# Komputerowe-Projektowanie-Lekow/pmarlo

Measured on AMD Instinct MI355X. Metric: frames/sec featurize->TICA->k-means->T-matrix, 1Mx64 synth; ITS rel-err, higher is better.
Workload: dtype f64; 1 GPU; synthetic 1000000 frames x 64 f32 features per GPU (AR(1) latents), TICA->10, k=500 (10 Lloyd iterations), lag=10, row-normalised T; frames_per_gpu=1000000, features=64, tica_dim=10, k=500, lag=10, kmeans_iters=10, parallelism=shards1

## Files before the change

include/msmhip.h:

```cpp
#ifndef MSMHIP_H
#define MSMHIP_H

#include <stddef.h>
#include <stdint.h>

#ifdef __cplusplus
extern "C" {
#endif

typedef struct msm_ctx msm_ctx;
typedef struct msm_event msm_event;
typedef struct msm_graph msm_graph;

typedef enum {
    MSM_OK = 0,
    MSM_ERR_INVALID = 1,
    MSM_ERR_HIP = 2,
    MSM_ERR_NOMEM = 3,
    MSM_ERR_UNSUPPORTED = 4,
    MSM_ERR_NOCONV = 5
} msm_status;

typedef enum { MSM_F32 = 0, MSM_F64 = 1 } msm_dtype;

// ... 33 lines not shown
                            int64_t ld, int col_off);
msm_status msm_featurize_angles(msm_ctx* ctx, const float* d_xyz, int64_t n, int A,
                                const int32_t* d_triplets, int Tn, float* d_out, int64_t ld, int col_off);
msm_status msm_featurize_dihedrals(msm_ctx* ctx, const float* d_xyz, int64_t n, int A,
                                   const int32_t* d_quads, int Q, int mode, float* d_out, int64_t ld,
                                   int col_off);

msm_status msm_featurize_sasa(msm_ctx* ctx, const float* d_xyz, int64_t n, int A, const float* d_radii,
                              const float* d_points, int P, float* d_out);
msm_status msm_hbond_presence(msm_ctx* ctx, const float* d_xyz, int64_t n, int A, const int32_t* d_triplets,
                              int Tn, float dist_cutoff, float angle_cutoff, uint64_t* d_counts);
msm_status msm_dssp(msm_ctx* ctx, const float* d_xyz, int64_t n, int A, const int32_t* d_backbone,
                    const int32_t* d_chain, const uint8_t* d_proline, int R, uint8_t* d_codes);

#define MSM_SUPERPOSE_TILE_FRAMES 64
#define MSM_SUPERPOSE_TILE_FLOATS 12288
#define MSM_SUPERPOSE_LDS_ATOMS 4096
#define MSM_SUPERPOSE_NARROW_SEL 64
msm_status msm_superpose(msm_ctx* ctx, const float* d_xyz, int64_t n, int A, const int32_t* d_sel, int S,
                         const float* d_ref, float* d_out, float* d_rmsd);


msm_status msm_count_transitions(msm_ctx* ctx, const int32_t* d_labels, int64_t n,
                                 const int64_t* h_seg_start, const int64_t* h_seg_stop,
                                 int n_seg, int lag, int stride, int k,
                                 int64_t* d_counts, int64_t* d_pairs);

msm_status msm_count_transitions_weighted(msm_ctx* ctx, const int32_t* d_labels,
                                          const double* d_weights, int64_t n,
                                          const int64_t* h_seg_start, const int64_t* h_seg_stop,
                                          int n_seg, int lag, int stride, int k,
                                          double* d_counts, int64_t* d_pairs);

msm_status msm_count_transitions_lagscan(msm_ctx* ctx, const int32_t* d_labels, int64_t n,
                                         const int64_t* h_seg_start, const int64_t* h_seg_stop,
                                         int n_seg, const int32_t* h_lags, int n_lag, int k,
                                         int64_t* d_counts, int64_t* d_pairs);

msm_status msm_state_counts(msm_ctx* ctx, const int32_t* d_labels, int64_t n, int k,
                            int64_t* d_visits);

msm_status msm_run_lengths(msm_ctx* ctx, const int32_t* d_labels, int64_t n, int k, int64_t* d_stats,
                           int32_t* d_run_state, int64_t* d_run_len, int64_t capacity, int64_t* d_n_runs);


msm_status msm_column_moments_partial(msm_ctx* ctx, const void* d_x, msm_dtype dtype, int64_t n, int F,
                                      int64_t ld, const double* d_shift, double* d_sums,
                                      double* d_shift_out);
msm_status msm_moments_finalize(msm_ctx* ctx, const double* d_sums, const double* d_shift, int F,
                                int ddof, double* d_mean, double* d_std, double* d_count);
msm_status msm_column_minmax(msm_ctx* ctx, const void* d_x, msm_dtype dtype, int64_t n, int F, int64_t ld,
                             double* d_min, double* d_max, int64_t* d_counts);
msm_status msm_column_moments(msm_ctx* ctx, const void* d_x, msm_dtype dtype, int64_t n, int F,
                              int64_t ld, int ddof, double* d_mean, double* d_std, double* d_count);

msm_status msm_standardise_params(msm_ctx* ctx, const double* d_sums, const double* d_shift, int F,
                                  double n_rows, int with_std, double* d_mean, double* d_scale,
                                  double* d_inv_scale);

msm_status msm_lagged_moments(msm_ctx* ctx, const void* d_x, msm_dtype dtype, int64_t n, int F, int64_t ld,
                              const int64_t* h_seg_start, const int64_t* h_seg_stop, int n_seg, int lag,
                              const double* d_shift, int assume_finite, double* d_moments);

msm_status msm_lagged_moments_reversible(msm_ctx* ctx, const void* d_x, msm_dtype dtype, int64_t n, int F, int64_t ld,
                                         const int64_t* h_seg_start, const int64_t* h_seg_stop, int n_seg, int lag,
                                         const double* d_shift, int assume_finite, double* d_moments);

msm_status msm_lagged_moments_onesided(msm_ctx* ctx, const void* d_x, msm_dtype dtype, int64_t n, int F,
                                       int64_t ld, const int64_t* h_seg_start, const int64_t* h_seg_stop,
                                       int n_seg, int lag, const double* d_shift, int assume_finite,
                                       double* d_moments);

msm_status msm_onesided_tica_eigenvalues(msm_ctx* ctx, const double* d_moments, int F, double clip,
                                         double* d_eigvals);

msm_status msm_moments_from_lagged(msm_ctx* ctx, const void* d_x, msm_dtype dtype, int64_t n, int F, int64_t ld,
                                   const int64_t* h_seg_start, const int64_t* h_seg_stop, int n_seg, int lag,
                                   const double* d_shift, const double* d_moments, double* d_sums);

msm_status msm_tica_solve(msm_ctx* ctx, const double* d_moments, const double* d_scale, int F,
                          double epsilon, int kinetic_map, double* d_eigvals, double* d_coeffs,
                          double* d_mean, int* d_rank);

msm_status msm_project(msm_ctx* ctx, const void* d_x, msm_dtype dtype, int64_t n, int F, int64_t ld,
                       const double* d_mu, const double* d_inv_sigma, const double* d_mean2,
                       const double* d_w, int d, int64_t ldw, double* d_y, int64_t ldy, double* d_absmax);

msm_status msm_project_finite(msm_ctx* ctx, const void* d_x, msm_dtype dtype, int64_t n, int F, int64_t ld,
                              const double* d_mu, const double* d_inv_sigma, const double* d_mean2,
                              const double* d_w, int d, int64_t ldw, double* d_y, int64_t ldy, double* d_absmax);

msm_status msm_eigh(msm_ctx* ctx, const double* d_a, int n, double* d_w, double* d_v, int* d_sweeps);

msm_status msm_autocorr_lagscan(msm_ctx* ctx, const void* d_x, msm_dtype dtype, int64_t n, int F, int64_t ld,
                                const int64_t* h_seg_start, const int64_t* h_seg_stop, int n_seg,
                                const int32_t* h_lags, int n_lag, double var_floor, double* d_value,
                                int32_t* d_nvalid);

msm_status msm_hstack_f64(msm_ctx* ctx, const void* d_a, msm_dtype dtype_a, int pa, int64_t lda, const void* d_b,
                          msm_dtype dtype_b, int pb, int64_t ldb, int64_t n, double* d_out);


msm_status msm_kmeans_assign(msm_ctx* ctx, const void* d_x, msm_dtype dtype, int64_t n, int d,
                             int64_t ld, const double* d_centers, int k,
                             const double* d_mean, const double* d_std,
                             int32_t* d_labels, double* d_mindist);

msm_status msm_kmeans_fit(msm_ctx* ctx, const void* d_x, msm_dtype dtype, int64_t n, int d, int64_t ld,
                          const double* d_mean, const double* d_std, int k, uint64_t seed,
                          int init_centers, int max_iter, double tol2, double* d_centers,
                          double* d_state);
msm_status msm_kmeans_init_plusplus(msm_ctx* ctx, const void* d_x, msm_dtype dtype, int64_t n, int d, int64_t ld,
                                    const double* d_mean, const double* d_std, int k, uint64_t seed, double n_total,
                                    double* d_centers, const double* d_state, int64_t* d_picked);
msm_status msm_kmeans_fit_begin(msm_ctx* ctx, const void* d_x, msm_dtype dtype, int64_t n, int d,
                                int64_t ld, const double* d_mean, const double* d_std, int k,
                                uint64_t seed, int init_centers, double n_total, double tol2,
                                double* d_centers, double* d_state, int absmax_ready);
msm_status msm_kmeans_accumulate(msm_ctx* ctx, const void* d_x, msm_dtype dtype, int64_t n, int d,
                                 int64_t ld, const double* d_centers, int k, const double* d_mean,
                                 const double* d_std, const double* d_state, int64_t* d_sums,
                                 int64_t* d_counts);
msm_status msm_kmeans_update(msm_ctx* ctx, int64_t* d_sums, int64_t* d_counts, int k, int d,
                             double* d_centers, double* d_state, int clear);

msm_status msm_kmeans_image_bytes(int64_t n, int d, size_t* out_bytes);
msm_status msm_kmeans_pack(msm_ctx* ctx, const void* d_x, msm_dtype dtype, int64_t n, int d, int64_t ld,
                           const double* d_mean, const double* d_std, void* d_image);
msm_status msm_kmeans_pack_bounded(msm_ctx* ctx, const void* d_x, msm_dtype dtype, int64_t n, int d, int64_t ld,
                                   const double* d_mean, const double* d_std, const double* d_absmax, void* d_image);
msm_status msm_kmeans_assign_packed(msm_ctx* ctx, const void* d_x, msm_dtype dtype, int64_t n, int d,
                                    int64_t ld, const double* d_centers, int k, const double* d_mean,
                                    const double* d_std, const void* d_image, int32_t* d_labels,
                                    double* d_mindist);
msm_status msm_kmeans_accumulate_packed(msm_ctx* ctx, const void* d_x, msm_dtype dtype, int64_t n, int d,
                                        int64_t ld, const double* d_centers, int k, const double* d_mean,
                                        const double* d_std, const void* d_image, const double* d_state,
                                        int64_t* d_sums, int64_t* d_counts);
msm_status msm_kmeans_accumulate_delta(msm_ctx* ctx, const void* d_x, msm_dtype dtype, int64_t n, int d,
                                       int64_t ld, const double* d_centers, int k, const double* d_mean,
                                       const double* d_std, const void* d_image, const double* d_state,
                                       int32_t* d_prev_labels, int64_t* d_sums, int64_t* d_counts);
msm_status msm_kmeans_lloyd_pass(msm_ctx* ctx, const void* d_x, msm_dtype dtype, int64_t n, int d, int64_t ld,
                                 double* d_centers, int k, const double* d_mean, const double* d_std,
                                 const void* d_image, double* d_state, int32_t* d_prev_labels, int64_t* d_sums,
                                 int64_t* d_counts);
msm_status msm_kmeans_filter_scanned(msm_ctx* ctx, uint64_t* h_out, int reset);
msm_status msm_mfma_bf16_probe(msm_ctx* ctx, const uint16_t* h_a, const uint16_t* h_b, const float* h_c,
                               float* h_d, int n_tiles);
msm_status msm_mfma_f16_probe(msm_ctx* ctx, const uint16_t* h_a, const uint16_t* h_b, const float* h_c,
                              float* h_d, int n_tiles);

msm_status msm_sum_f64(msm_ctx* ctx, const double* d_v, int64_t n, double* d_out);


msm_status msm_transition_matrix(msm_ctx* ctx, const void* d_counts, int counts_are_f64, int k, int mode,
                                 double alpha, double epsilon, double* d_T, int32_t* d_active,
                                 int32_t* d_inv_map, int32_t* d_n_active, double* d_rowsum,
                                 double* d_diag_mass);

msm_status msm_embed_full(msm_ctx* ctx, const double* d_T_active, const double* d_pi_active,
                          const int32_t* d_inv_map, int k, double* d_T_full, double* d_pi_full);

size_t msm_spectrum_workspace_bytes(int n_max, int p, int batch);
msm_status msm_spectrum(msm_ctx* ctx, const double* d_T, int64_t t_stride, int ld, const int32_t* d_n,
                        int n_max, int batch, int p, int n_iter, int init, uint64_t seed, int n_watch,
                        void* d_workspace, double* d_ritz, double* d_pi, int64_t pi_stride,
                        double* d_change, int32_t* d_status, int n_its, const double* d_lags,
                        double* d_its_eig, double* d_its_ts, double freeze_tol, double* d_vecs, int n_vecs);
msm_status msm_matrix_power(msm_ctx* ctx, const double* d_T, int64_t t_stride, int ld, const int32_t* d_n, int n_max,
                            int batch, int n_squarings, double* d_scratch, double* d_out);
msm_status msm_spectrum_powered(msm_ctx* ctx, const double* d_T, const double* d_T_power, int64_t t_stride, int ld,
                                const int32_t* d_n, int n_max, int batch, int p, int n_iter, int init, uint64_t seed,
                                int n_watch, void* d_workspace, double* d_ritz, double* d_pi, int64_t pi_stride,
                                double* d_change, int32_t* d_status, int n_its, const double* d_lags,
                                double* d_its_eig, double* d_its_ts, double freeze_tol, double* d_vecs, int n_vecs);

msm_status msm_reversible_mle(msm_ctx* ctx, const double* d_counts, int n, int ld, double maxerr, int maxiter,
                              double* d_T, int ldt, double* d_pi, int* h_iterations, double* h_err);

msm_status msm_sample_transition_matrices(msm_ctx* ctx, const void* d_counts, int counts_are_f64, int k,
                                          const int32_t* d_active, const int32_t* d_n_active, double alpha,
                                          uint64_t seed, int first_sample, int n_samples, double* d_T,
                                          int64_t t_stride, int ld);

msm_status msm_sample_reversible_transition_matrices(msm_ctx* ctx, const double* d_counts, int n, int ld,
                                                     const double* d_T0, const double* d_pi0, uint64_t seed,
                                                     int first_sample, int n_samples, int n_sweeps, double* d_T,
                                                     int64_t t_stride, int ldt, double* d_pi);

msm_status msm_active_counts(msm_ctx* ctx, const void* d_counts, int counts_are_f64, int k, const int32_t* d_active,
                             const int32_t* d_n_active, double alpha, double* d_out);

msm_status msm_philox4x32(msm_ctx* ctx, uint64_t key, const uint32_t counter[4], uint32_t* d_out);

msm_status msm_gemm_f64(msm_ctx* ctx, int m, int n, int k, const double* d_A, int64_t lda,
                        const double* d_B, int64_t ldb, double* d_C, int64_t ldc);
msm_status msm_ck_test(msm_ctx* ctx, const double* d_T1, int64_t ld1, const double* d_Tk,
                       int64_t tk_stride, int64_t ldk, int n, const int32_t* h_factors, int n_factors,
                       const double* d_rowcounts, int64_t rc_stride, double* d_mse, double* d_noise);

msm_status msm_diff_norms(msm_ctx* ctx, const double* d_P, int64_t ldp, const double* d_Q, int64_t ldq, int n, int m,
                          double* d_out);

msm_status msm_order_statistics(msm_ctx* ctx, const double* d_x, int64_t stride, int64_t n, const int64_t* h_ranks,
                                int n_ranks, double* h_out);

msm_status msm_weighted_stats(msm_ctx* ctx, const double* d_x, int64_t stride, int64_t n,
                              const double* d_w, double* d_out6);
msm_status msm_hist2d(msm_ctx* ctx, const double* d_x, int64_t sx, const double* d_y, int64_t sy,
                      int64_t n, const double* d_w, double w_absmax, const double* d_xedges, int nx,
                      const double* d_yedges, int ny, double* d_hist);
msm_status msm_smooth_sparse_bins(msm_ctx* ctx, const double* d_hist, int nx, int ny,
                                  double min_count, double* d_out, int32_t* d_n_smoothed);
msm_status msm_scale_to_total(msm_ctx* ctx, double* d_v, int n, double total);
msm_status msm_fes_finalize(msm_ctx* ctx, const double* d_hist, int n_cells, double kT,
                            double* d_F, int32_t* d_status);
msm_status msm_kde2d(msm_ctx* ctx, const double* d_x, int64_t sx, const double* d_y, int64_t sy,
                     int64_t n, const double* d_w, double w_scale, const double* d_xcenters, int nx,
                     const double* d_ycenters, int ny, double bw_x, double bw_y, int periodic, double* d_density);

msm_status msm_clip_or_wrap(msm_ctx* ctx, const double* d_x, int64_t stride, int64_t n, double lo, double hi, int mode,
                            double* d_out);

msm_status msm_gather_f64(msm_ctx* ctx, const double* d_table, int m, const int32_t* d_idx, int64_t n, double* d_out);

msm_status msm_solve_f64(msm_ctx* ctx, int n, int nrhs, double* d_A, int64_t lda, double* d_B,
                         int64_t ldb, int32_t* d_info);
msm_status msm_reactive_flux(msm_ctx* ctx, const double* d_T, int64_t ldt, const double* d_pi,
// ... 62 lines not shown
```

pmarlo_amd/_lib.py:

```python

from __future__ import annotations

import ctypes as C
from pathlib import Path

__all__ = ["lib", "load", "LIB_PATH", "check", "MsmError", "DECLARED_SYMBOLS"]

LIB_PATH = Path(__file__).resolve().parent / "csrc" / "libmsmhip.so"

MSM_OK, MSM_ERR_INVALID, MSM_ERR_HIP, MSM_ERR_NOMEM, MSM_ERR_UNSUPPORTED, MSM_ERR_NOCONV = range(6)
MSM_F32, MSM_F64 = 0, 1
SUPERPOSE_TILE_FRAMES, SUPERPOSE_TILE_FLOATS, SUPERPOSE_LDS_ATOMS, SUPERPOSE_NARROW_SEL = 64, 12288, 4096, 64
REP_MAX_D, REP_GROUP_CHUNK, REP_TILE_I, REP_TILE_J = 256, 1024, 128, 64
REP_FLAG_NONFINITE, REP_FLAG_NEGATIVE, REP_FLAG_NONPOSITIVE_SUM = 1, 2, 4
REP_SCORE_CENTROID, REP_SCORE_MEDOID = 0, 1
REP_SELECT_SMALLEST, REP_SELECT_DIVERSE = 0, 1


class MsmError(RuntimeError):
    """A HIP-side failure reported through the C ABI."""


_vp = C.c_void_p
_i32 = C.c_int
_i64 = C.c_int64
_sz = C.c_size_t
_f64 = C.c_double
_pp = C.POINTER(C.c_void_p)

_PROTOTYPES: dict[str, tuple] = {
    "msm_version": (C.c_char_p, []),
    "msm_ctx_create": (_i32, [_i32, _vp, _pp]),
    "msm_ctx_destroy": (None, [_vp]),
    "msm_last_error": (C.c_char_p, [_vp]),
    "msm_device_info": (_i32, [_vp, C.c_char_p, _sz, C.POINTER(_i32), C.POINTER(_sz)]),
    "msm_malloc": (_i32, [_vp, _sz, _pp]),
    "msm_free": (_i32, [_vp, _vp]),
    "msm_memcpy_h2d": (_i32, [_vp, _vp, _vp, _sz]),
    "msm_memcpy_d2h": (_i32, [_vp, _vp, _vp, _sz]),
    "msm_memcpy_d2d": (_i32, [_vp, _vp, _vp, _sz]),
    "msm_memset": (_i32, [_vp, _vp, _i32, _sz]),
    "msm_sync": (_i32, [_vp]),
    "msm_event_create": (_i32, [_vp, _pp]),
    "msm_event_destroy": (None, [_vp]),
    "msm_event_record": (_i32, [_vp, _vp]),
    "msm_event_elapsed_ms": (_i32, [_vp, _vp, C.POINTER(C.c_float)]),
    "msm_graph_begin": (_i32, [_vp]),
    "msm_graph_end": (_i32, [_vp, _pp]),
    "msm_graph_launch": (_i32, [_vp, _vp]),
    "msm_graph_destroy": (None, [_vp]),
    "msm_featurize_distances": (_i32, [_vp, _vp, _i64, _i32, _vp, _i32, _vp, _i64, _i32]),
    "msm_featurize_contacts": (_i32, [_vp, _vp, _i64, _i32, _vp, _i32, C.c_float, _vp, _i64, _i32]),
    "msm_featurize_rg": (_i32, [_vp, _vp, _i64, _i32, _vp, _i64, _i32]),
    "msm_featurize_angles": (_i32, [_vp, _vp, _i64, _i32, _vp, _i32, _vp, _i64, _i32]),
    "msm_featurize_dihedrals": (_i32, [_vp, _vp, _i64, _i32, _vp, _i32, _i32, _vp, _i64, _i32]),
    "msm_featurize_sasa": (_i32, [_vp, _vp, _i64, _i32, _vp, _vp, _i32, _vp]),
    "msm_hbond_presence": (_i32, [_vp, _vp, _i64, _i32, _vp, _i32, C.c_float, C.c_float, _vp]),
    "msm_dssp": (_i32, [_vp, _vp, _i64, _i32, _vp, _vp, _vp, _i32, _vp]),
    "msm_superpose": (_i32, [_vp, _vp, _i64, _i32, _vp, _i32, _vp, _vp, _vp]),
    "msm_count_transitions": (_i32, [_vp, _vp, _i64, _vp, _vp, _i32, _i32, _i32, _i32, _vp, _vp]),
    "msm_count_transitions_weighted": (
        _i32, [_vp, _vp, _vp, _i64, _vp, _vp, _i32, _i32, _i32, _i32, _vp, _vp]),
    "msm_count_transitions_lagscan": (_i32, [_vp, _vp, _i64, _vp, _vp, _i32, _vp, _i32, _i32, _vp, _vp]),
    "msm_state_counts": (_i32, [_vp, _vp, _i64, _i32, _vp]),
    "msm_column_moments_partial": (_i32, [_vp, _vp, _i32, _i64, _i32, _i64, _vp, _vp, _vp]),
    "msm_moments_finalize": (_i32, [_vp, _vp, _vp, _i32, _i32, _vp, _vp, _vp]),
    "msm_column_moments": (_i32, [_vp, _vp, _i32, _i64, _i32, _i64, _i32, _vp, _vp, _vp]),
    "msm_column_minmax": (_i32, [_vp, _vp, _i32, _i64, _i32, _i64, _vp, _vp, _vp]),
    "msm_standardise_params": (_i32, [_vp, _vp, _vp, _i32, _f64, _i32, _vp, _vp, _vp]),
    "msm_lagged_moments": (_i32, [_vp, _vp, _i32, _i64, _i32, _i64, _vp, _vp, _i32, _i32, _vp, _i32, _vp]),
    "msm_tica_solve": (_i32, [_vp, _vp, _vp, _i32, _f64, _i32, _vp, _vp, _vp, _vp]),
    "msm_lagged_moments_reversible": (_i32, [_vp, _vp, _i32, _i64, _i32, _i64, _vp, _vp, _i32, _i32, _vp, _i32, _vp]),
    "msm_lagged_moments_onesided": (_i32, [_vp, _vp, _i32, _i64, _i32, _i64, _vp, _vp, _i32, _i32, _vp, _i32, _vp]),
    "msm_onesided_tica_eigenvalues": (_i32, [_vp, _vp, _i32, _f64, _vp]),
    "msm_moments_from_lagged": (_i32, [_vp, _vp, _i32, _i64, _i32, _i64, _vp, _vp, _i32, _i32, _vp, _vp, _vp]),
    "msm_project": (_i32, [_vp, _vp, _i32, _i64, _i32, _i64, _vp, _vp, _vp, _vp, _i32, _i64, _vp, _i64, _vp]),
    "msm_project_finite": (_i32, [_vp, _vp, _i32, _i64, _i32, _i64, _vp, _vp, _vp, _vp, _i32, _i64, _vp, _i64, _vp]),
    "msm_eigh": (_i32, [_vp, _vp, _i32, _vp, _vp, _vp]),
    "msm_autocorr_lagscan": (_i32, [_vp, _vp, _i32, _i64, _i32, _i64, _vp, _vp, _i32, _vp, _i32, _f64, _vp, _vp]),
    "msm_hstack_f64": (_i32, [_vp, _vp, _i32, _i32, _i64, _vp, _i32, _i32, _i64, _i64, _vp]),
    "msm_kmeans_assign": (_i32, [_vp, _vp, _i32, _i64, _i32, _i64, _vp, _i32, _vp, _vp, _vp, _vp]),
    "msm_kmeans_fit": (_i32, [_vp, _vp, _i32, _i64, _i32, _i64, _vp, _vp, _i32, C.c_uint64, _i32, _i32, _f64, _vp, _vp]),
    "msm_kmeans_fit_begin": (
        _i32, [_vp, _vp, _i32, _i64, _i32, _i64, _vp, _vp, _i32, C.c_uint64, _i32, _f64, _f64, _vp, _vp, _i32]),
    "msm_kmeans_accumulate": (_i32, [_vp, _vp, _i32, _i64, _i32, _i64, _vp, _i32, _vp, _vp, _vp, _vp, _vp]),
    "msm_kmeans_update": (_i32, [_vp, _vp, _vp, _i32, _i32, _vp, _vp, _i32]),
    "msm_comm_unique_id": (_i32, [_vp, _sz]),
    "msm_comm_init": (_i32, [_vp, _i32, _i32, _vp, _sz, _pp]),
    "msm_comm_destroy": (None, [_vp]),
    "msm_comm_info": (_i32, [_vp, C.POINTER(_i32), C.POINTER(_i32), C.POINTER(C.c_uint64)]),
    "msm_allreduce_i64": (_i32, [_vp, _vp, _sz]),
    "msm_allreduce_i64_from": (_i32, [_vp, _vp, _vp, _sz]),
    "msm_allreduce_f64": (_i32, [_vp, _vp, _sz]),
    "msm_allreduce_min_f64": (_i32, [_vp, _vp, _sz]),
    "msm_allreduce_max_f64": (_i32, [_vp, _vp, _sz]),
    "msm_broadcast": (_i32, [_vp, _vp, _sz, _i32]),
    "msm_rcp_f64": (_i32, [_vp, _vp, _sz, _vp]),
    "msm_kmeans_image_bytes": (_i32, [_i64, _i32, C.POINTER(_sz)]),
    "msm_kmeans_pack": (_i32, [_vp, _vp, _i32, _i64, _i32, _i64, _vp, _vp, _vp]),
    "msm_kmeans_pack_bounded": (_i32, [_vp, _vp, _i32, _i64, _i32, _i64, _vp, _vp, _vp, _vp]),
    "msm_kmeans_assign_packed": (_i32, [_vp, _vp, _i32, _i64, _i32, _i64, _vp, _i32, _vp, _vp, _vp, _vp, _vp]),
    "msm_kmeans_accumulate_packed": (_i32, [_vp, _vp, _i32, _i64, _i32, _i64, _vp, _i32, _vp, _vp, _vp, _vp, _vp, _vp]),
    "msm_kmeans_lloyd_pass": (_i32, [_vp, _vp, _i32, _i64, _i32, _i64, _vp, _i32, _vp, _vp, _vp, _vp, _vp, _vp, _vp]),
    "msm_kmeans_accumulate_delta": (_i32, [_vp, _vp, _i32, _i64, _i32, _i64, _vp, _i32, _vp, _vp, _vp, _vp, _vp, _vp,
                                           _vp]),
    "msm_kmeans_filter_scanned": (_i32, [_vp, C.POINTER(C.c_uint64), _i32]),
    "msm_kmeans_init_plusplus": (_i32, [_vp, _vp, _i32, _i64, _i32, _i64, _vp, _vp, _i32, C.c_uint64, _f64, _vp, _vp, _vp]),
    "msm_mfma_bf16_probe": (_i32, [_vp, _vp, _vp, _vp, _vp, _i32]),
    "msm_mfma_f16_probe": (_i32, [_vp, _vp, _vp, _vp, _vp, _i32]),
    "msm_run_lengths": (_i32, [_vp, _vp, _i64, _i32, _vp, _vp, _vp, _i64, _vp]),
    "msm_sum_f64": (_i32, [_vp, _vp, _i64, _vp]),
    "msm_transition_matrix": (_i32, [_vp, _vp, _i32, _i32, _i32, _f64, _f64, _vp, _vp, _vp, _vp, _vp, _vp]),
    "msm_embed_full": (_i32, [_vp, _vp, _vp, _vp, _i32, _vp, _vp]),
    "msm_spectrum_workspace_bytes": (_sz, [_i32, _i32, _i32]),
    "msm_spectrum": (_i32, [_vp, _vp, _i64, _i32, _vp, _i32, _i32, _i32, _i32, _i32, C.c_uint64, _i32, _vp, _vp, _vp,
                            _i64, _vp, _vp, _i32, _vp, _vp, _vp, _f64, _vp, _i32]),
    "msm_matrix_power": (_i32, [_vp, _vp, _i64, _i32, _vp, _i32, _i32, _i32, _vp, _vp]),
    "msm_spectrum_powered": (_i32, [_vp, _vp, _vp, _i64, _i32, _vp, _i32, _i32, _i32, _i32, _i32, C.c_uint64, _i32, _vp, _vp,
                                    _vp, _i64, _vp, _vp, _i32, _vp, _vp, _vp, _f64, _vp, _i32]),
    "msm_sample_transition_matrices": (_i32, [_vp, _vp, _i32, _i32, _vp, _vp, _f64, C.c_uint64, _i32, _i32, _vp, _i64,
                                              _i32]),
    "msm_sample_reversible_transition_matrices": (_i32, [_vp, _vp, _i32, _i32, _vp, _vp, C.c_uint64, _i32, _i32, _i32,
                                                         _vp, _i64, _i32, _vp]),
    "msm_active_counts": (_i32, [_vp, _vp, _i32, _i32, _vp, _vp, _f64, _vp]),
    "msm_reversible_mle": (_i32, [_vp, _vp, _i32, _i32, _f64, _i32, _vp, _i32, _vp, _vp, _vp]),
    "msm_philox4x32": (_i32, [_vp, C.c_uint64, _vp, _vp]),
    "msm_gemm_f64": (_i32, [_vp, _i32, _i32, _i32, _vp, _i64, _vp, _i64, _vp, _i64]),
    "msm_diff_norms": (_i32, [_vp, _vp, _i64, _vp, _i64, _i32, _i32, _vp]),
    "msm_gather_f64": (_i32, [_vp, _vp, _i32, _vp, _i64, _vp]),
    "msm_clip_or_wrap": (_i32, [_vp, _vp, _i64, _i64, _f64, _f64, _i32, _vp]),
    "msm_order_statistics": (_i32, [_vp, _vp, _i64, _i64, _vp, _i32, _vp]),
    "msm_weighted_stats": (_i32, [_vp, _vp, _i64, _i64, _vp, _vp]),
    "msm_hist2d": (_i32, [_vp, _vp, _i64, _vp, _i64, _i64, _vp, _f64, _vp, _i32, _vp, _i32, _vp]),
    "msm_smooth_sparse_bins": (_i32, [_vp, _vp, _i32, _i32, _f64, _vp, _vp]),
    "msm_scale_to_total": (_i32, [_vp, _vp, _i32, _f64]),
    "msm_fes_finalize": (_i32, [_vp, _vp, _i32, _f64, _vp, _vp]),
    "msm_kde2d": (_i32, [_vp, _vp, _i64, _vp, _i64, _i64, _vp, _f64, _vp, _i32, _vp, _i32, _f64, _f64, _i32, _vp]),
    "msm_solve_f64": (_i32, [_vp, _i32, _i32, _vp, _i64, _vp, _i64, _vp]),
    "msm_reactive_flux": (_i32, [_vp, _vp, _i64, _vp, _vp, _i32, _vp, _vp, _vp, _vp, _vp, _vp]),
    "msm_lump_macro": (_i32, [_vp, _vp, _i64, _vp, _vp, _i32, _i32, _vp, _vp]),
    "msm_macro_mfpt": (_i32, [_vp, _vp, _i64, _i32, _vp, _vp]),
    "msm_silhouette": (_i32, [_vp, _vp, _i64, _i32, _i64, _vp, _i32, _vp, _vp]),
    "msm_grid_cells": (_i32, [_vp, _vp, _i32, _i64, _i32, _i64, _vp, _i32, _vp]),
    "msm_first_occurrence": (_i32, [_vp, _vp, _i64, _i32, _vp]),
    "msm_relabel": (_i32, [_vp, _vp, _i64, _vp, _i32, _vp]),
    "msm_ck_test": (_i32, [_vp, _vp, _i64, _vp, _i64, _i64, _i32, _vp, _i32, _vp, _i64, _vp, _vp]),
    "msm_group_by_label": (_i32, [_vp, _vp, _i64, _i32, _vp, _vp]),
    "msm_state_centroids": (_i32, [_vp, _vp, _i64, _i32, _i64, _vp, _vp, _vp, _i32, _vp, _vp, _vp]),
    "msm_state_scores": (_i32, [_vp, _vp, _i64, _i32, _i64, _vp, _vp, _vp, _vp, _i32, _vp, _vp, _i32, _vp, _vp, _i32, _vp]),
    "msm_state_select": (_i32, [_vp, _vp, _i64, _i32, _i64, _vp, _vp, _i32, _vp, _vp, _i32, _vp, _i32, _i32, _vp]),
}

DECLARED_SYMBOLS = tuple(_PROTOTYPES)

_lib = None


def load() -> C.CDLL:
    global _lib
    if _lib is not None:
        return _lib
    if not LIB_PATH.exists():
        raise ImportError(
            f"{LIB_PATH} is missing: build it with `python -m pmarlo_amd.csrc.build` "
            "(hipcc, gfx950).  pmarlo_amd has no CPU fallback."
        )
    handle = C.CDLL(str(LIB_PATH))
    for name, (res, args) in _PROTOTYPES.items():
        fn = getattr(handle, name)
        fn.restype = res
        fn.argtypes = args
    _lib = handle
    return handle


class _LazyLib:
    def __getattr__(self, name):
        return getattr(load(), name)


lib = _LazyLib()

_EXC = {
    MSM_ERR_INVALID: ValueError,
    MSM_ERR_HIP: MsmError,
    MSM_ERR_NOMEM: MemoryError,
# ... 15 lines not shown
```

pmarlo_amd/csrc/cov.hip:

```cpp
#include "common.h"

#include <cstring>

namespace {

typedef double v4f64 __attribute__((ext_vector_type(4)));

constexpr int kThreads = 256;
constexpr int kWaves = kThreads / 64;
constexpr int kUnroll = 1;

struct FrameTab {
    int n;
    int lag;
    int64_t start[MSM_SEG_INLINE];
    int64_t stop[MSM_SEG_INLINE];
    int64_t prefix[MSM_SEG_INLINE + 1];
    int64_t total;
    int64_t pairs;
    double wy_w;
};
constexpr int kGroup = 4 * kUnroll;

template <typename T>
__device__ __forceinline__ double to_f64(T v) { return (double)v; }

template <int NT>
struct CovShape {
    static constexpr int kSym = NT * (NT + 1) / 2;
    static constexpr int kTiles = NT * NT + kSym;
    static constexpr int kSlab = kTiles * 256 + 2 * NT * 16;
};

template <int NT>
__host__ __device__ constexpr int sym_index(int ti, int tj) { return ti * NT - ti * (ti - 1) / 2 + (tj - ti); }

template <int NT>
struct TileSplit {
    static constexpr int kSym = NT * (NT + 1) / 2;
    static constexpr int kTotal = NT * NT + kSym;
    static constexpr int kRows0 = (NT + 1) / 2;
    static constexpr int kSym0 = (kTotal + 1) / 2 - kRows0 * NT;
    template <int HALF> static constexpr bool own_0t(int a) { return HALF < 0 || (HALF == 0) == (a < kRows0); }
    template <int HALF> static constexpr bool own_00(int sidx) { return HALF < 0 || (HALF == 0) == (sidx < kSym0); }
};

template <int NT>
struct TileSplitSym {
    template <int HALF> static constexpr bool own_0t(int) { return HALF <= 0; }
    template <int HALF> static constexpr bool own_00(int) { return HALF != 0; }
};

template <typename T, int NT, bool VEC, int HALF, bool FINITE, bool SYM = false>
__device__ __forceinline__ void cov_wave_body(const T* __restrict__ x, int F, int64_t ld, const FrameTab& ft,
                                              const double* __restrict__ mu, int64_t frames_per_wave,
                                              int frame_wave, int n_frame_waves, double* red, int red_wave,
                                              volatile int* prog = nullptr) {
    using S = CovShape<NT>;
    using TS = std::conditional_t<SYM, TileSplitSym<NT>, TileSplit<NT>>;
    const int lane = threadIdx.x & 63;
    const int fi_ = lane & 15;
    const int kk = lane >> 4;
    const int lag = ft.lag;

    v4f64 acc0t[NT][NT];
    v4f64 acc00[S::kSym];
    double ssum[NT], shift[NT];
    double ssum2[NT];
    double sint[NT];
    bool fok[NT];
#pragma unroll
    for (int a = 0; a < NT; ++a) {
#pragma unroll
        for (int b = 0; b < NT; ++b) acc0t[a][b] = (v4f64){0.0, 0.0, 0.0, 0.0};
        ssum[a] = ssum2[a] = sint[a] = 0.0;
        const int f = NT * fi_ + a;
        fok[a] = f < F;
        shift[a] = fok[a] ? mu[f] : 0.0;
    }
#pragma unroll
    for (int a = 0; a < S::kSym; ++a) acc00[a] = (v4f64){0.0, 0.0, 0.0, 0.0};

    const int64_t gw = (int64_t)blockIdx.x * n_frame_waves + frame_wave;
// ... 566 lines not shown
    }
    ft.total = ft.prefix[ft.n];
    *out = ft;
    return MSM_OK;
}

__global__ __launch_bounds__(256) void symmetrise_m0t_kernel(double* __restrict__ m0t, int F) {
    const int64_t e = (int64_t)blockIdx.x * blockDim.x + threadIdx.x;
    if (e >= (int64_t)F * F) return;
    const int i = (int)(e / F), j = (int)(e % F);
    if (i >= j) return;
    const double h = 0.5 * (m0t[(size_t)i * F + j] + m0t[(size_t)j * F + i]);
    m0t[(size_t)i * F + j] = h;
    m0t[(size_t)j * F + i] = h;
}

template <typename T, int NT>
msm_status launch_cov(msm_ctx* ctx, const T* x, int F, int64_t ld, const FrameTab& ft, const double* mu,
                      bool finite, bool sym, double* d_out) {
    using S = CovShape<NT>;
    int blocks = ctx->n_cu;
    const int64_t groups = ft.total / kGroup;
    const int64_t min_groups_per_wave = 4;
    if ((int64_t)blocks * kWaves * min_groups_per_wave > groups)
        blocks = (int)std::max<int64_t>(1, groups / (kWaves * min_groups_per_wave));
    int64_t fpw = (ft.total + (int64_t)blocks * kWaves - 1) / ((int64_t)blocks * kWaves);
    fpw = (fpw + kGroup - 1) / kGroup * kGroup;
    blocks = (int)((ft.total + fpw * kWaves - 1) / (fpw * kWaves));
    msm_status rs = msm_reserve_scratch(ctx, (size_t)blocks * S::kSlab * sizeof(double));
    if (rs != MSM_OK) return rs;
    const size_t lds = ((size_t)S::kTiles * 256 + (size_t)kWaves * 2 * NT * 64) * sizeof(double);
    const bool vec = (NT != 3) && (F == 16 * NT) && (ld % NT == 0) && (((uintptr_t)x) % (NT * sizeof(T)) == 0) &&
                     (ld * 4 * (int64_t)sizeof(T) < (int64_t(1) << 31));
    constexpr bool kSplit = NT >= 3;
    constexpr bool kHasSym = kSplit;
    auto kern = vec ? (finite ? cov_fused_kernel<T, NT, true, kSplit, true> : cov_fused_kernel<T, NT, true, kSplit, false>)
                    : (finite ? cov_fused_kernel<T, NT, false, kSplit, true> : cov_fused_kernel<T, NT, false, kSplit, false>);
    if constexpr (kHasSym) {
        if (sym)
            kern = vec ? (finite ? cov_fused_kernel<T, NT, true, kSplit, true, true> : cov_fused_kernel<T, NT, true, kSplit, false, true>)
                       : (finite ? cov_fused_kernel<T, NT, false, kSplit, true, true> : cov_fused_kernel<T, NT, false, kSplit, false, true>);
    }
    if (lds > 48 * 1024)
        MSM_HIP(ctx, hipFuncSetAttribute((const void*)kern, hipFuncAttributeMaxDynamicSharedMemorySize, (int)lds));
    hipLaunchKernelGGL(kern, dim3(blocks), dim3(kSplit ? 512 : 256), lds, ctx->stream, x, F, ld, ft, mu, fpw,
                       (double*)ctx->scratch);
    MSM_CHECK_LAUNCH(ctx);
    if (sym && kHasSym) {
        hipLaunchKernelGGL((cov_reduce_kernel<NT, kHasSym>), dim3(msm_ceil_div(S::kSlab, 64)), dim3(1024), 0, ctx->stream,
                           (const double*)ctx->scratch, blocks, F, (double)ft.pairs, d_out);
    } else {
        hipLaunchKernelGGL(cov_reduce_kernel<NT>, dim3(msm_ceil_div(S::kSlab, 64)), dim3(1024), 0, ctx->stream,
                           (const double*)ctx->scratch, blocks, F, (double)ft.pairs, d_out);
        if (sym) {
            MSM_CHECK_LAUNCH(ctx);
            hipLaunchKernelGGL(symmetrise_m0t_kernel, dim3(msm_ceil_div(F * F, 256)), dim3(256), 0, ctx->stream,
                               d_out + (size_t)F * F, F);
        }
    }
    MSM_CHECK_LAUNCH(ctx);
    return MSM_OK;
}

template <typename T>
msm_status dispatch_cov(msm_ctx* ctx, const T* x, int F, int64_t ld, const FrameTab& ft, const double* mu,
                        bool finite, bool sym, double* d_out) {
    if (F <= 16) return launch_cov<T, 1>(ctx, x, F, ld, ft, mu, finite, sym, d_out);
    if (F <= 32) return launch_cov<T, 2>(ctx, x, F, ld, ft, mu, finite, sym, d_out);
    if (F <= 48) return launch_cov<T, 3>(ctx, x, F, ld, ft, mu, finite, sym, d_out);
    if (F <= 64) return launch_cov<T, 4>(ctx, x, F, ld, ft, mu, finite, sym, d_out);
    msm_status rs = launch_cov_blocked<T>(ctx, x, F, ld, ft, mu, finite, d_out);
    if (rs == MSM_OK && sym) {
        hipLaunchKernelGGL(symmetrise_m0t_kernel, dim3(msm_ceil_div((int64_t)F * F, 256)), dim3(256), 0, ctx->stream,
                           d_out + (size_t)F * F, F);
        MSM_CHECK_LAUNCH(ctx);
    }
    return rs;
}

}

namespace {

struct EdgeSegs {
    int n;
    int lag;
    int64_t start[MSM_SEG_INLINE];
    int64_t stop[MSM_SEG_INLINE];
};

template <typename T>
__global__ __launch_bounds__(256) void moments_from_lagged_kernel(const T* __restrict__ x, int F, int64_t ld,
                                                                  EdgeSegs sg, const double* __restrict__ shift,
                                                                  const double* __restrict__ mom,
                                                                  double* __restrict__ sums) {
    double frames = 0.0;
    for (int q = 0; q < sg.n; ++q) frames += (double)(sg.stop[q] - sg.start[q]);
    for (int f = threadIdx.x; f < F; f += blockDim.x) {
        const double sh = shift[f];
        double e1 = 0.0, e2 = 0.0;
        for (int q = 0; q < sg.n; ++q) {
            const int64_t s = sg.start[q], e = sg.stop[q];
            const int64_t head = min<int64_t>(s + sg.lag, e), tail = max<int64_t>(e - sg.lag, s);
            const int n_head = (int)(head - s), n_edge = n_head + (int)(e - tail);
#pragma unroll 8
            for (int q2 = 0; q2 < n_edge; ++q2) {
                const int64_t t = q2 < n_head ? s + q2 : tail + (q2 - n_head);
                const double z = (double)x[t * ld + f] - sh;
                e1 += z;
                e2 = fma(z, z, e2);
            }
        }
        const double sx = mom[(size_t)2 * F * F + f], sy = mom[(size_t)2 * F * F + F + f];
        sums[f] = frames;
        sums[F + f] = 0.5 * (sx + sy + e1);
        sums[2 * F + f] = 0.5 * (mom[(size_t)f * F + f] + e2);
    }
}

}

extern "C" {

static msm_status lagged_moments_impl(msm_ctx* ctx, const void* d_x, msm_dtype dtype, int64_t n, int F, int64_t ld,
                                      const int64_t* h_seg_start, const int64_t* h_seg_stop, int n_seg, int lag,
                                      const double* d_shift, int assume_finite, bool one_sided, bool sym,
                                      double* d_moments) {
    if (!ctx) return MSM_ERR_INVALID;
    MSM_REQUIRE(ctx, n >= 0 && F >= 1 && ld >= F, "msm_lagged_moments: need n >= 0, F >= 1, ld >= F");
    MSM_REQUIRE(ctx, dtype == MSM_F32 || dtype == MSM_F64, "msm_lagged_moments: bad dtype");
    MSM_REQUIRE(ctx, d_shift && d_moments && (d_x || n == 0), "msm_lagged_moments: NULL pointer");
    FrameTab ft;
    msm_status rs = build_frametab(ctx, n, h_seg_start, h_seg_stop, n_seg, lag, one_sided, &ft);
    if (rs != MSM_OK) return rs;
    if (ft.total == 0) {
        MSM_HIP(ctx, hipMemsetAsync(d_moments, 0, ((size_t)2 * F * F + 2 * F + 1) * sizeof(double), ctx->stream));
        return MSM_OK;
    }
    if (dtype == MSM_F32)
        return dispatch_cov<float>(ctx, (const float*)d_x, F, ld, ft, d_shift, assume_finite != 0, sym, d_moments);
    return dispatch_cov<double>(ctx, (const double*)d_x, F, ld, ft, d_shift, assume_finite != 0, sym, d_moments);
}

msm_status msm_lagged_moments(msm_ctx* ctx, const void* d_x, msm_dtype dtype, int64_t n, int F, int64_t ld,
                              const int64_t* h_seg_start, const int64_t* h_seg_stop, int n_seg, int lag,
                              const double* d_shift, int assume_finite, double* d_moments) {
    return lagged_moments_impl(ctx, d_x, dtype, n, F, ld, h_seg_start, h_seg_stop, n_seg, lag, d_shift, assume_finite,
                               false, false, d_moments);
}

msm_status msm_lagged_moments_reversible(msm_ctx* ctx, const void* d_x, msm_dtype dtype, int64_t n, int F, int64_t ld,
                                         const int64_t* h_seg_start, const int64_t* h_seg_stop, int n_seg, int lag,
                                         const double* d_shift, int assume_finite, double* d_moments) {
    return lagged_moments_impl(ctx, d_x, dtype, n, F, ld, h_seg_start, h_seg_stop, n_seg, lag, d_shift, assume_finite,
                               false, true, d_moments);
}

msm_status msm_lagged_moments_onesided(msm_ctx* ctx, const void* d_x, msm_dtype dtype, int64_t n, int F, int64_t ld,
                                       const int64_t* h_seg_start, const int64_t* h_seg_stop, int n_seg, int lag,
                                       const double* d_shift, int assume_finite, double* d_moments) {
    return lagged_moments_impl(ctx, d_x, dtype, n, F, ld, h_seg_start, h_seg_stop, n_seg, lag, d_shift, assume_finite,
                               true, false, d_moments);
}

msm_status msm_moments_from_lagged(msm_ctx* ctx, const void* d_x, msm_dtype dtype, int64_t n, int F, int64_t ld,
                                   const int64_t* h_seg_start, const int64_t* h_seg_stop, int n_seg, int lag,
                                   const double* d_shift, const double* d_moments, double* d_sums) {
    if (!ctx) return MSM_ERR_INVALID;
    MSM_REQUIRE(ctx, n >= 0 && F >= 1 && ld >= F && lag >= 1, "msm_moments_from_lagged: bad shape / lag");
    MSM_REQUIRE(ctx, dtype == MSM_F32 || dtype == MSM_F64, "msm_moments_from_lagged: bad dtype");
    MSM_REQUIRE(ctx, d_shift && d_moments && d_sums && (d_x || n == 0), "msm_moments_from_lagged: NULL pointer");
    MSM_REQUIRE(ctx, n_seg >= 0 && n_seg <= MSM_SEG_INLINE && (n_seg == 0 || (h_seg_start && h_seg_stop)),
                "msm_moments_from_lagged: at most %d segments per call", MSM_SEG_INLINE);
    EdgeSegs sg;
    sg.n = 0;
    sg.lag = lag;
    if (n_seg == 0) {
        if (n > 0) { sg.start[0] = 0; sg.stop[0] = n; sg.n = 1; }
    } else {
        for (int q = 0; q < n_seg; ++q) {
            const int64_t a = std::max<int64_t>(0, h_seg_start[q]), b = std::min<int64_t>(n, h_seg_stop[q]);
            if (b > a) { sg.start[sg.n] = a; sg.stop[sg.n] = b; ++sg.n; }
        }
    }
    if (dtype == MSM_F32)
        hipLaunchKernelGGL(moments_from_lagged_kernel<float>, dim3(1), dim3(256), 0, ctx->stream, (const float*)d_x, F, ld,
                           sg, d_shift, d_moments, d_sums);
    else
        hipLaunchKernelGGL(moments_from_lagged_kernel<double>, dim3(1), dim3(256), 0, ctx->stream, (const double*)d_x, F,
                           ld, sg, d_shift, d_moments, d_sums);
    MSM_CHECK_LAUNCH(ctx);
    return MSM_OK;
}

}
```

pmarlo_amd/csrc/eig.hip:

```cpp
#include "common.h"
#include "wave.h"

#ifdef MSM_JACOBI_STAMPS
__device__ unsigned long long g_jacobi_stamps[8];
#define JSTAMP(i)                                                                          \
    do {                                                                                   \
        unsigned long long t__;                                                            \
        asm volatile("s_memtime %0\n\ts_waitcnt lgkmcnt(0)" : "=s"(t__)::"memory");       \
        acc__[i] += t__ - last__;                                                          \
        last__ = t__;                                                                      \
    } while (0)
#define JSTAMP_INIT unsigned long long acc__[8] = {0, 0, 0, 0, 0, 0, 0, 0}; unsigned long long last__; asm volatile("s_memtime %0\n\ts_waitcnt lgkmcnt(0)" : "=s"(last__)::"memory");
#define JSTAMP_FLUSH if (threadIdx.x == 0) { for (int i__ = 0; i__ < 8; ++i__) g_jacobi_stamps[i__] += acc__[i__]; }
#else
#define JSTAMP(i)
#define JSTAMP_INIT
#define JSTAMP_FLUSH
#endif

namespace {

constexpr int kEigThreads = 1024;
constexpr int kMaxPairs = 128;

struct JacobiShared {
    double2 cs[kMaxPairs];
    int p[kMaxPairs], q[kMaxPairs];
    int colw[kMaxPairs];
    int roww[kMaxPairs];
    double2 cs2[2][32];
    int colw2[2][32], roww2[2][32];
    double red[kEigThreads / 64];
    double bc[4];
    int ibc[4];
};

__device__ __forceinline__ double nr_rcp(double x) {
    double r = __builtin_amdgcn_rcp(x);
    r = fma(r, fma(-x, r, 1.0), r);
    r = fma(r, fma(-x, r, 1.0), r);
    return r;
}
__device__ __forceinline__ double nr_rsqrt(double x) {
    double r = __builtin_amdgcn_rsq(x);
    const double h = 0.5 * x;
    r = r * fma(-h * r, r, 1.5);
    r = r * fma(-h * r, r, 1.5);
    return r;
}

__device__ __forceinline__ void jacobi_rotation(double app, double aqq, double apq, double& c, double& s) {
    c = 1.0; s = 0.0;
    if (apq == 0.0) return;
    const double a = 0.5 * (aqq - app);
    const double h2 = fma(a, a, apq * apq);
    if (!(h2 > 1e-300) || !(h2 < 1e300)) return;
    double rh = __builtin_amdgcn_rsq(h2);
    rh = rh * fma(-0.5 * h2 * rh, rh, 1.5);
    const double h = h2 * rh;
    const double den = fabs(a) + h;
    double rd = __builtin_amdgcn_rcp(den);
    rd = fma(rd, fma(-den, rd, 1.0), rd);
    const double t = (a >= 0.0 ? apq : -apq) * rd;
    c = nr_rsqrt(fma(t, t, 1.0));
    s = t * c;
}

__device__ __forceinline__ void pivot_pair(int round, int i, int npad, int& p, int& q) {
    if (i == 0) { p = round; q = npad - 1; return; }
    p = round + i; if (p >= npad - 1) p -= npad - 1;
    q = round - i; if (q < 0) q += npad - 1;
}

__device__ __forceinline__ int jacobi_eigh_pipelined(double* A, double* V, int n, int ld, JacobiShared* sh,
                                                     int max_sweeps);

__device__ __forceinline__ int jacobi_eigh(double* A, double* V, int n, int ld, JacobiShared* sh, int max_sweeps) {
    const int tid = threadIdx.x, nt = blockDim.x;
    {
        const int mh = n / 2;
        if ((n & 1) == 0 && mh >= 4 && mh <= 32 && mh * mh <= nt && mh * n <= 2 * nt && n * ld < 65536 && nt >= 64)
            return jacobi_eigh_pipelined(A, V, n, ld, sh, max_sweeps);
    }
    for (int i = tid; i < n * n; i += nt) V[(i / n) * ld + (i % n)] = (i / n == i % n) ? 1.0 : 0.0;
// ... 798 lines not shown
            }
#pragma unroll
            for (int u = 0; u < 8; ++u) {
                if (j0 + u + 1 < n && j0 + u >= kk) {
                    z = f[u] * z;
                    Xc[(j0 + u + 1) * ld] = z;
                    nrm2 = fma(z, z, nrm2);
                }
            }
        }
        ts->uq[lane] = nrm2;
    }
    __syncthreads();
    if (tid < n) {
        const double nrm2 = ts->praw[tid] + ts->uq[tid];
        const bool ok = nrm2 > 0.0 && nrm2 < 1e300;
        ts->inv[tid] = nr_rsqrt(ok ? nrm2 : 1.0);
        if (!ok) ts->bad = 1;
    }
    __syncthreads();
    TSTAMP(5);
    {
        double worst = 0.0;
        bool bad = false;
        for (int e0 = tid; e0 < n * n; e0 += nt) {
            const int j = e0 / n, i = e0 - j * n;
            const double x0 = X[j * ld + i];
            const double xm = j > 0 ? ts->e[j - 1] * X[(j - 1) * ld + i] : 0.0;
            const double xp = j + 1 < n ? ts->e[j] * X[(j + 1) * ld + i] : 0.0;
            const double tx = fma(ts->d[j] - ts->lam[i], x0, xm + xp) * ts->inv[i];
            bad = bad || !(fabs(tx) <= 1e-10);
        }
        const int jj = lane & 15, g = lane >> 4;
        const int tiles = (n + 15) >> 4;
        for (int t = wave; t < tiles * tiles; t += nt >> 6) {
            const int a0 = (t / tiles) * 16, b0 = (t - (t / tiles) * tiles) * 16;
            if (b0 > a0) continue;
            const bool aok = a0 + jj < n, bok = b0 + jj < n;
            const int ai = aok ? a0 + jj : 0, bi = bok ? b0 + jj : 0;
            const double sa = ts->inv[ai], sb = ts->inv[bi];
            tri_v4f64 acc = {0.0, 0.0, 0.0, 0.0};
            for (int k0 = 0; k0 < n; k0 += 16) {
                double a[4], b[4];
#pragma unroll
                for (int u = 0; u < 4; ++u) {
                    const bool kok = k0 + 4 * u + g < n;
                    const int k = kok ? k0 + 4 * u + g : 0;
                    a[u] = X[k * ld + ai] * sa;
                    b[u] = X[k * ld + bi] * sb;
                    if (!(aok && kok)) a[u] = 0.0;
                    if (!(bok && kok)) b[u] = 0.0;
                }
#pragma unroll
                for (int u = 0; u < 4; ++u) acc = __builtin_amdgcn_mfma_f64_16x16x4f64(a[u], b[u], acc, 0, 0, 0);
            }
#pragma unroll
            for (int r = 0; r < 4; ++r) {
                const int row = a0 + g + 4 * r, col = b0 + jj;
                if (row < n && col < n) worst = fmax(worst, fabs(acc[r] - (row == col ? 1.0 : 0.0)));
            }
        }
        if (bad) worst = 1e300;
#pragma unroll
        for (int off = 32; off > 0; off >>= 1) worst = fmax(worst, __shfl_xor(worst, off, 64));
        if (lane == 0) ts->red[wave] = worst;
        __syncthreads();
        worst = 0.0;
        for (int w = 0; w < nt / 64; ++w) worst = fmax(worst, ts->red[w]);
        TSTAMP(6);
        if (ts->bad || !(worst <= orth_tol)) return false;
    }
    mfma_mm<true, false>(A, Q, X, n, n, n, ld, ts->inv);
    if (tid < n) ts->lam[tid] /= ts->scale;
    __syncthreads();
    TSTAMP(7);
    return true;
}

struct TicaWork {
    double *A, *V, *B1, *B2, *ev, *mean, *isc;
    int* order;
};

template <int lds_mats>
__global__ __launch_bounds__(kEigThreads) void tica_solve_kernel(
    const double* __restrict__ mom, const double* __restrict__ scale, int n, int ld, double epsilon, int kinetic_map,
    TicaWork wk, double* __restrict__ out_eig, double* __restrict__ out_W, double* __restrict__ out_mean,
    int* __restrict__ out_rank) {
    extern __shared__ __attribute__((aligned(16))) unsigned char smem_raw[];
    __shared__ JacobiShared sh;
    __shared__ TriShared ts;
    const int tid = threadIdx.x, nt = blockDim.x;
    double* lds = reinterpret_cast<double*>(smem_raw);
    const size_t mat = (size_t)n * ld;
    double *A, *V, *B1, *B2;
    if constexpr (lds_mats >= 2) { A = lds; V = lds + mat; } else { A = wk.A; V = wk.V; }
    if constexpr (lds_mats >= 4) { B1 = lds + 2 * mat; B2 = lds + 3 * mat; } else { B1 = wk.B1; B2 = wk.B2; }

    const double* M00 = mom;
    const double* M0t = mom + (size_t)n * n;
    const double* sx = M0t + (size_t)n * n;
    const double* sy = sx + n;
    const double T = sy[n];
    const double w = 2.0 * T;
    KSTAMP_INIT
    if (!(T > 0.0)) {
        if (tid == 0) *out_rank = 0;
        for (int i = tid; i < n; i += nt) { out_eig[i] = 0.0; out_mean[i] = 0.0; }
        for (int i = tid; i < n * n; i += nt) out_W[i] = 0.0;
        return;
    }
    double* iscp = (lds_mats == 4 && n <= kTriMax) ? ts.lam : wk.isc;
    double* meanp = (lds_mats == 4 && n <= kTriMax) ? ts.inv : wk.mean;
    for (int i = tid; i < n; i += nt) {
        const double is = scale ? 1.0 / scale[i] : 1.0;
        iscp[i] = is;
        const double m = (sx[i] + sy[i]) / w * is;
        meanp[i] = m;
        out_mean[i] = m;
    }
    __syncthreads();
    auto build_cov = [&]() {
        for (int e = tid; e < n * n; e += nt) {
            const int i = e / n, j = e - i * n;
            const double ss = iscp[i] * iscp[j];
            const double mm = meanp[i] * meanp[j];
            A[i * ld + j] = 0.5 * (M00[e] + M00[j * n + i]) / w * ss - mm;
            B1[i * ld + j] = (M0t[e] + M0t[j * n + i]) / w * ss - mm;
        }
        __syncthreads();
    };
    build_cov();
    KSTAMP(8);

    constexpr bool kFused = lds_mats == 4;
    bool full_rank;
    if (kFused && n <= kTriMax) {
        full_rank = ldl_whiten_registers(A, B2, n, epsilon, &ts, 1);
        if (full_rank) {
            double s = 0.0;
            for (int e = tid; e < n * n; e += nt) {
                const double wv = B2[(e / n) * ld + (e % n)];
                s = fma(wv, wv, s);
            }
            s = block_sum_bcast(s, sh.red, sh.bc);
            if (!(s * epsilon * (1.0 + 1e-9) <= 1.0)) full_rank = ldl_whiten_registers(A, nullptr, n, epsilon, &ts, 2);
        }
    } else {
        for (int e = tid; e < n * n; e += nt) {
            const int i = e / n, j = e - i * n;
            B2[i * ld + j] = A[i * ld + j] - (i == j ? epsilon : 0.0);
            V[i * ld + j] = A[i * ld + j];
        }
        __syncthreads();
        full_rank = cholesky_lower_pair(B2, V, n, ld, &sh);
        if (full_rank) {
            lower_inverse(V, A, n, ld);
            for (int e = tid; e < n * n; e += nt) {
                const int i = e / n, j = e - i * n;
                B2[i * ld + j] = j >= i ? A[j * ld + i] : 0.0;
            }
            __syncthreads();
        } else {
            __syncthreads();
            build_cov();
        }
    }
    KSTAMP(9);
    int rank;
    if (full_rank) {
        rank = n;
        if (tid == 0) *out_rank = n;
    } else {
        jacobi_eigh(A, V, n, ld, &sh, 40);
        for (int i = tid; i < n; i += nt) wk.ev[i] = A[i * ld + i];
        __syncthreads();
        sort_desc_abs(wk.ev, n, wk.order);
        if (tid == 0) {
            double evmin = wk.ev[0];
            for (int i = 1; i < n; ++i) evmin = fmin(evmin, wk.ev[i]);
            double eps = epsilon;
            if (evmin < 0.0) eps = fmax(eps, -evmin + 1e-16);
            int rank = 0;
            for (int i = 0; i < n; ++i) rank += fabs(wk.ev[i]) >= eps;
            sh.ibc[0] = rank;
            *out_rank = rank;
        }
        __syncthreads();
        rank = sh.ibc[0];
        if (rank == 0) {
            for (int i = tid; i < n; i += nt) out_eig[i] = 0.0;
            for (int i = tid; i < n * n; i += nt) out_W[i] = 0.0;
            return;
        }
        for (int e = tid; e < n * rank; e += nt) {
            const int i = e / rank, j = e - i * rank;
            B2[i * ld + j] = V[i * ld + wk.order[j]];
        }
        __syncthreads();
// ... 174 lines not shown
    __syncthreads();
    auto eigh = [&](const double*& vec) {
        bool fast = false;
        if (use_lds && n <= kTriMax) {
            for (int e = tid; e < n * n; e += nt) gbak[e] = P0[(e / n) * ld + (e % n)];
            __syncthreads();
            fast = tridiag_eigh(P0, P2, P3, n, ld, &ts, 1e-12);
            if (fast) {
                for (int i = tid; i < n; i += nt) gw[i] = ts.lam[i];
                vec = P0;
            } else {
                __syncthreads();
                for (int e = tid; e < n * n; e += nt) P0[(e / n) * ld + (e % n)] = gbak[e];
            }
            __syncthreads();
        }
        if (!fast) {
            jacobi_eigh(P0, P2, n, ld, &sh, 40);
            for (int i = tid; i < n; i += nt) gw[i] = P0[i * ld + i];
            vec = P2;
            __syncthreads();
        }
    };
    const double* vec = nullptr;
    eigh(vec);
    for (int e = tid; e < n * n; e += nt) {
        const int i = e / n, j = e - i * n;
        const double wj = gw[j] > clip ? gw[j] : clip;
        P3[i * ld + j] = vec[i * ld + j] / sqrt(sqrt(wj));
    }
    __syncthreads();
    mfma_mm<false, true>(P0, P3, P3, n, n, n, ld);
    mfma_mm<false, false>(P2, P0, P1, n, n, n, ld);
    mfma_mm<false, false>(P3, P2, P0, n, n, n, ld);
    for (int e = tid; e < n * n; e += nt) {
        const int i = e / n, j = e - i * n;
        P0[i * ld + j] = 0.5 * (P3[i * ld + j] + P3[j * ld + i]);
    }
    __syncthreads();
    eigh(vec);
    for (int i = tid; i < n; i += nt) {
        const double a = gw[i];
        int rank = 0;
        for (int j = 0; j < n; ++j) {
            const double b = gw[j];
            rank += (b > a) || (b == a && j < i);
        }
        order[rank] = i;
    }
    __syncthreads();
    for (int j = tid; j < n; j += nt) out_eig[j] = gw[order[j]];
}

size_t jacobi_lds_bytes(int n, int ld) { return (size_t)(n <= kTriMax ? 3 : 2) * n * ld * sizeof(double); }

}

extern "C" {

msm_status msm_tica_solve(msm_ctx* ctx, const double* d_moments, const double* d_scale, int F, double epsilon,
                          int kinetic_map, double* d_eigvals, double* d_coeffs, double* d_mean, int* d_rank) {
    if (!ctx) return MSM_ERR_INVALID;
    MSM_REQUIRE(ctx, F >= 1 && F <= 2 * kMaxPairs, "msm_tica_solve: need 1 <= F <= %d (got %d)", 2 * kMaxPairs, F);
    MSM_REQUIRE(ctx, epsilon >= 0.0, "msm_tica_solve: epsilon must be >= 0");
    MSM_REQUIRE(ctx, d_moments && d_eigvals && d_coeffs && d_mean && d_rank, "msm_tica_solve: NULL pointer");
    const int ld = F <= kTriMax ? kTriLd : (F | 1);
    const size_t mat = (size_t)F * ld;
    const size_t need = (4 * mat + 3 * F) * sizeof(double) + (size_t)F * sizeof(int) + 64;
    msm_status rs = msm_reserve_scratch(ctx, need);
    if (rs != MSM_OK) return rs;
    double* base = (double*)ctx->scratch;
    TicaWork wk;
    wk.A = base; wk.V = base + mat; wk.B1 = base + 2 * mat; wk.B2 = base + 3 * mat;
    wk.ev = base + 4 * mat; wk.mean = wk.ev + F; wk.isc = wk.mean + F; wk.order = (int*)(wk.isc + F);
    const size_t lds_budget = 150 * 1024;
    int lds_mats = 0;
    if (4 * mat * sizeof(double) <= lds_budget) lds_mats = 4;
    else if (2 * mat * sizeof(double) <= lds_budget) lds_mats = 2;
    const size_t lds = (size_t)lds_mats * mat * sizeof(double);
    auto kern = lds_mats == 4 ? tica_solve_kernel<4> : (lds_mats == 2 ? tica_solve_kernel<2> : tica_solve_kernel<0>);
    if (lds > 48 * 1024)
        MSM_HIP(ctx, hipFuncSetAttribute((const void*)kern, hipFuncAttributeMaxDynamicSharedMemorySize, (int)lds));
    hipLaunchKernelGGL(kern, dim3(1), dim3(kEigThreads), lds, ctx->stream, d_moments, d_scale, F, ld, epsilon,
                       kinetic_map, wk, d_eigvals, d_coeffs, d_mean, d_rank);
    MSM_CHECK_LAUNCH(ctx);
    return MSM_OK;
}

msm_status msm_onesided_tica_eigenvalues(msm_ctx* ctx, const double* d_moments, int F, double clip, double* d_eigvals) {
    if (!ctx) return MSM_ERR_INVALID;
    MSM_REQUIRE(ctx, F >= 1 && F <= 2 * kMaxPairs, "msm_onesided_tica_eigenvalues: need 1 <= F <= %d (got %d)",
                2 * kMaxPairs, F);
    MSM_REQUIRE(ctx, d_moments && d_eigvals && clip > 0.0, "msm_onesided_tica_eigenvalues: bad arguments");
    const int ld = F <= kTriMax ? kTriLd : (F | 1);
    const size_t mat = (size_t)F * ld;
    const size_t lds = 4 * mat * sizeof(double);
    const bool use_lds = lds <= 140 * 1024;
    msm_status rs = msm_reserve_scratch(ctx, ((use_lds ? 0 : 4 * mat) + (size_t)F * F + F) * sizeof(double) +
                                                 (size_t)F * sizeof(int) + 64);
    if (rs != MSM_OK) return rs;
    double* gP = (double*)ctx->scratch;
    double* gbak = gP + (use_lds ? 0 : 4 * mat);
    double* gw = gbak + (size_t)F * F;
    int* order = (int*)(gw + F);
    auto kern = use_lds ? onesided_eig_kernel<true> : onesided_eig_kernel<false>;
    if (use_lds && lds > 48 * 1024)
        MSM_HIP(ctx, hipFuncSetAttribute((const void*)kern, hipFuncAttributeMaxDynamicSharedMemorySize, (int)lds));
    hipLaunchKernelGGL(kern, dim3(1), dim3(kEigThreads), use_lds ? lds : 0, ctx->stream, d_moments, F, ld, clip, gP, gbak,
                       gw, order, d_eigvals);
    MSM_CHECK_LAUNCH(ctx);
    return MSM_OK;
}

msm_status msm_eigh(msm_ctx* ctx, const double* d_a, int n, double* d_w, double* d_v, int* d_sweeps) {
    if (!ctx) return MSM_ERR_INVALID;
    MSM_REQUIRE(ctx, n >= 1 && n <= 2 * kMaxPairs, "msm_eigh: need 1 <= n <= %d (got %d)", 2 * kMaxPairs, n);
    MSM_REQUIRE(ctx, d_a && d_w, "msm_eigh: NULL pointer");
    const int ld = n <= kTriMax ? kTriLd : (n | 1);
    const size_t mat = (size_t)n * ld;
    msm_status rs = msm_reserve_scratch(ctx, 2 * mat * sizeof(double) + (size_t)n * sizeof(int) + 64);
    if (rs != MSM_OK) return rs;
    double* gA = (double*)ctx->scratch;
    double* gV = gA + mat;
    int* order = (int*)(gV + mat);
    const size_t lds = jacobi_lds_bytes(n, ld);
    const int use_lds = lds <= 140 * 1024;
    auto kern = use_lds ? eigh_kernel<true> : eigh_kernel<false>;
    if (use_lds && lds > 48 * 1024)
        MSM_HIP(ctx, hipFuncSetAttribute((const void*)kern, hipFuncAttributeMaxDynamicSharedMemorySize, (int)lds));
    hipLaunchKernelGGL(kern, dim3(1), dim3(kEigThreads), use_lds ? lds : 0, ctx->stream, d_a, n, ld, gA, gV, order,
                       d_w, d_v, d_sweeps);
    MSM_CHECK_LAUNCH(ctx);
    return MSM_OK;
}

}
```

pmarlo_amd/csrc/kmeans.hip:

```cpp
#include "common.h"
#include "wave.h"

#include <algorithm>
#include <cstdlib>

namespace {

constexpr int kThreads = 256;

template <typename T>
__device__ __forceinline__ double load_as_f64(const T* p) { return (double)(*p); }

struct FitState {
    double scale;
    double inv_scale;
    double absmax;
    double shift2;
    double tol2;
    double done;
    double n_iter;
    double inertia;
};

__device__ __forceinline__ long long to_fixed(double v, double scale) { return __double2ll_rn(v * scale); }

template <typename T>
__global__ __launch_bounds__(kThreads) void absmax_kernel(const T* __restrict__ x, int64_t n, int d, int64_t ld,
                                                         const double* __restrict__ mean,
                                                         const double* __restrict__ stdv,
                                                         unsigned long long* __restrict__ out_bits) {
    double m = 0.0;
    const int64_t total = n * d;
    const int64_t step = (int64_t)gridDim.x * kThreads;
    if (ld == d && !mean) {
        constexpr int V = 16 / (int)sizeof(T);
        struct alignas(16) Pack { T v[V]; };
        const bool aligned = (reinterpret_cast<uintptr_t>(x) & 15) == 0;
        const int64_t npack = aligned ? total / V : 0;
        const Pack* xp = reinterpret_cast<const Pack*>(x);
        int64_t i = (int64_t)blockIdx.x * kThreads + threadIdx.x;
        for (; i + 3 * step < npack; i += 4 * step) {
            Pack q[4];
#pragma unroll
            for (int u = 0; u < 4; ++u) q[u] = xp[i + u * step];
#pragma unroll
            for (int u = 0; u < 4; ++u)
#pragma unroll
                for (int j = 0; j < V; ++j) m = fmax(m, fabs((double)q[u].v[j]));
        }
        for (; i < npack; i += step) {
            const Pack q = xp[i];
#pragma unroll
            for (int j = 0; j < V; ++j) m = fmax(m, fabs((double)q.v[j]));
        }
        for (int64_t e = npack * V + (int64_t)blockIdx.x * kThreads + threadIdx.x; e < total; e += step)
            m = fmax(m, fabs((double)x[e]));
    } else {
        for (int64_t i = (int64_t)blockIdx.x * kThreads + threadIdx.x; i < total; i += step) {
            const int64_t r = i / d;
            const int f = (int)(i - r * d);
            double v = (double)x[r * ld + f];
            if (mean) v = (v - mean[f]) / stdv[f];
            m = fmax(m, fabs(v));
        }
    }
    m = wave_max_down(m);
    __shared__ double wave_max[kThreads / 64];
    if ((threadIdx.x & 63) == 0) wave_max[threadIdx.x >> 6] = m;
    __syncthreads();
    if (threadIdx.x == 0) {
        for (int w = 1; w < kThreads / 64; ++w) m = fmax(m, wave_max[w]);
        const unsigned long long bits = (unsigned long long)__double_as_longlong(m);
        if (bits > __atomic_load_n(out_bits, __ATOMIC_RELAXED)) atomicMax(out_bits, bits);
    }
}

__device__ __forceinline__ void fit_scale_body(const unsigned long long* __restrict__ absmax_bits, double n_total,
                                               double tol2, FitState* __restrict__ st) {
    double amax = __longlong_as_double((long long)*absmax_bits);
    if (!(amax > 0.0)) amax = 1.0;
    int e = 61 - (int)ceil(log2(n_total * amax));
    if (e > 60) e = 60;
    if (e < -900) e = -900;
    st->scale = ldexp(1.0, e);
    st->inv_scale = ldexp(1.0, -e);
    st->absmax = amax;
    st->shift2 = 0.0;
    st->tol2 = tol2;
    st->done = 0.0;
    st->n_iter = 0.0;
    st->inertia = 0.0;
}

__global__ void fit_scale_kernel(const unsigned long long* __restrict__ absmax_bits, double n_total, double tol2,
                                 FitState* __restrict__ st) {
    if (threadIdx.x != 0 || blockIdx.x != 0) return;
    fit_scale_body(absmax_bits, n_total, tol2, st);
}

template <typename T>
__global__ void init_centers_kernel(const T* __restrict__ x, int64_t n, int d, int64_t ld,
                                    const double* __restrict__ mean, const double* __restrict__ stdv, int k,
                                    unsigned long long seed, double* __restrict__ centers,
                                    const unsigned long long* __restrict__ absmax_bits, double n_total, double tol2,
                                    FitState* __restrict__ st) {
    const int i = blockIdx.x * blockDim.x + threadIdx.x;
    if (i == 0 && st) fit_scale_body(absmax_bits, n_total, tol2, st);
    if (i >= k * d) return;
    const int j = i / d, f = i - j * d;
    unsigned long long h = seed + 0x9E3779B97F4A7C15ull * (unsigned long long)(j + 1);
    h = (h ^ (h >> 30)) * 0xBF58476D1CE4E5B9ull;
    h = (h ^ (h >> 27)) * 0x94D049BB133111EBull;
    h ^= h >> 31;
    const double u = (double)(h >> 11) * (1.0 / 9007199254740992.0);
    int64_t t = (int64_t)(((double)j + u) * ((double)n / (double)k));
    if (t >= n) t = n - 1;
    double v = (double)x[t * ld + f];
    if (mean) v = (v - mean[f]) / stdv[f];
    centers[i] = v;
}

__global__ __launch_bounds__(1024) void kmeans_update_kernel(unsigned long long* __restrict__ sums,
                                                            unsigned long long* __restrict__ counts, int k, int d,
                                                            double* __restrict__ centers, FitState* __restrict__ st,
                                                            int clear) {
    __shared__ double red[16];
    if (st->done != 0.0) return;
    const double inv_scale = st->inv_scale;
    double acc = 0.0;
    constexpr int CH = 4;
    for (int i0 = threadIdx.x; i0 < k * d; i0 += 1024 * CH) {
        long long cnt[CH], sm[CH];
        double old[CH];
#pragma unroll
        for (int c = 0; c < CH; ++c) {
            const int i = i0 + c * 1024;
            cnt[c] = 0;
            if (i < k * d) {
                cnt[c] = (long long)counts[i / d];
                sm[c] = (long long)sums[i];
                old[c] = centers[i];
            }
        }
#pragma unroll
        for (int c = 0; c < CH; ++c)
            if (cnt[c] > 0) {
                const double c_new = (double)sm[c] * inv_scale / (double)cnt[c];
                const double dlt = c_new - old[c];
                acc = fma(dlt, dlt, acc);
                centers[i0 + c * 1024] = c_new;
            }
    }
    acc = wave_sum_down(acc);
    if ((threadIdx.x & 63) == 0) red[threadIdx.x >> 6] = acc;
    __syncthreads();
    if (clear) {
        for (int i = threadIdx.x; i < k * d; i += blockDim.x) sums[i] = 0ull;
        for (int i = threadIdx.x; i < k; i += blockDim.x) counts[i] = 0ull;
    }
    if (threadIdx.x == 0) {
        double t = 0.0;
        for (int i = 0; i < (int)(blockDim.x >> 6); ++i) t += red[i];
        st->shift2 = t;
        st->n_iter += 1.0;
        if (t <= st->tol2) st->done = 1.0;
    }
}

constexpr int kUpdateWide = 16384;
__global__ __launch_bounds__(1024) void kmeans_update_wide_kernel(unsigned long long* __restrict__ sums,
                                                                 unsigned long long* __restrict__ counts, int k, int d,
                                                                 int centres_per_block, double* __restrict__ centers,
                                                                 const FitState* __restrict__ st, int clear,
                                                                 double* __restrict__ partial) {
    __shared__ double red[16];
    if (st->done != 0.0) return;
    const double inv_scale = st->inv_scale;
    const int j0 = blockIdx.x * centres_per_block, j1 = min(k, j0 + centres_per_block);
    const int64_t e0 = (int64_t)j0 * d, e1 = (int64_t)j1 * d;
    double acc = 0.0;
    for (int64_t i = e0 + threadIdx.x; i < e1; i += blockDim.x) {
        const int j = (int)(i / d);
        const long long cnt = (long long)counts[j];
        if (cnt > 0) {
            const double c_new = (double)(long long)sums[i] * inv_scale / (double)cnt;
            const double dlt = c_new - centers[i];
            acc = fma(dlt, dlt, acc);
            centers[i] = c_new;
        }
    }
// ... 572 lines not shown
    D += (size_t)blockIdx.x * 256;
    v8bf a, b;
    for (int j = 0; j < 8; ++j) {
        a[j] = __builtin_bit_cast(__bf16, A[i * 32 + 8 * q + j]);
        b[j] = __builtin_bit_cast(__bf16, B[(8 * q + j) * 16 + i]);
    }
    v4f32 c;
    for (int r = 0; r < 4; ++r) c[r] = C[(4 * q + r) * 16 + i];
    c = __builtin_amdgcn_mfma_f32_16x16x32_bf16(a, b, c, 0, 0, 0);
    for (int r = 0; r < 4; ++r) D[(4 * q + r) * 16 + i] = c[r];
}

__global__ void mfma_f16_probe_kernel(const uint16_t* __restrict__ A, const uint16_t* __restrict__ B,
                                      const float* __restrict__ C, float* __restrict__ D) {
    const int l = threadIdx.x, i = l & 15, q = l >> 4;
    A += (size_t)blockIdx.x * 512;
    B += (size_t)blockIdx.x * 512;
    C += (size_t)blockIdx.x * 256;
    D += (size_t)blockIdx.x * 256;
    v8h a, b;
    for (int j = 0; j < 8; ++j) {
        a[j] = __builtin_bit_cast(_Float16, A[i * 32 + 8 * q + j]);
        b[j] = __builtin_bit_cast(_Float16, B[(8 * q + j) * 16 + i]);
    }
    v4f32 c;
    for (int r = 0; r < 4; ++r) c[r] = C[(4 * q + r) * 16 + i];
    c = __builtin_amdgcn_mfma_f32_16x16x32_f16(a, b, c, 0, 0, 0);
    for (int r = 0; r < 4; ++r) D[(4 * q + r) * 16 + i] = c[r];
}

bool filter_enabled() {
    static const bool on = [] {
        const char* e = getenv("MSM_KMEANS_FILTER");
        return !(e && e[0] == '0');
    }();
    return on;
}

size_t filter_image_bytes(int64_t n, int) { return (size_t)((n + 63) & ~(int64_t)63) * 16 * kFilterRowQ + 16; }

template <typename T>
msm_status launch_pack(msm_ctx* ctx, const T* x, int64_t n, int d, int64_t ld, const double* mean, const double* stdv,
                       const double* absmax, uint4* image) {
    const unsigned grid = (unsigned)((n + 255) / 256);
    if (!absmax) {
        uint4* tail = image + (size_t)((n + 63) & ~(int64_t)63) * kFilterRowQ;
        MSM_HIP(ctx, hipMemsetAsync(tail, 0, 8, ctx->stream));
        const int g = (int)std::min<int64_t>((n * d + 256 * 8 - 1) / (256 * 8), (int64_t)ctx->n_cu * 8);
        hipLaunchKernelGGL(filter_absmax_kernel<T>, dim3(g), dim3(256), 0, ctx->stream, x, n, d, ld, mean, stdv,
                           (unsigned long long*)tail);
        MSM_CHECK_LAUNCH(ctx);
        absmax = (const double*)tail;
    }
    const int dense = ld == d && ((uintptr_t)x & 15) == 0;
#define MSM_PACK_CASE(D)                                                                                              \
    case D:                                                                                                           \
        hipLaunchKernelGGL((kmeans_pack_kernel<T, D>), dim3(grid), dim3(256), 0, ctx->stream, x, n, ld, mean, stdv, absmax, \
                           image, dense);                                                                             \
        break
    switch (d) {
        MSM_PACK_CASE(1); MSM_PACK_CASE(2); MSM_PACK_CASE(3); MSM_PACK_CASE(4); MSM_PACK_CASE(5);
        MSM_PACK_CASE(6); MSM_PACK_CASE(7); MSM_PACK_CASE(8); MSM_PACK_CASE(9); MSM_PACK_CASE(10);
        default: return msm_fail(ctx, MSM_ERR_UNSUPPORTED, "k-means frame images need d <= %d (got %d)", kFilterMaxD, d);
    }
#undef MSM_PACK_CASE
    MSM_CHECK_LAUNCH(ctx);
    return MSM_OK;
}

msm_status filter_stats_buffer(msm_ctx* ctx, unsigned long long** out) {
    static_assert(sizeof(unsigned long long) == 8, "");
    if (!ctx->km_stats) {
        if (ctx->capturing) { *out = nullptr; return MSM_OK; }
        MSM_HIP(ctx, hipMalloc(&ctx->km_stats, 16));
        MSM_HIP(ctx, hipMemsetAsync(ctx->km_stats, 0, 16, ctx->stream));
    }
    *out = (unsigned long long*)ctx->km_stats;
    return MSM_OK;
}

template <typename T, int DP, bool ACCUM>
msm_status launch_filter_dp(msm_ctx* ctx, const T* x, int64_t n, int d, int64_t ld, const double* centers, int k,
                            const double* mean, const double* stdv, const uint4* image, int32_t* labels, double* mindist,
                            const FitState* st, unsigned long long* sums, unsigned long long* counts, double* upd_centers) {
    constexpr int NF = 4;
    const size_t lds = filter_lds_bytes(k, d, ACCUM);
    msm_status rs;
    const int64_t n_units = (n + 16 * NF - 1) / (16 * NF);
    const int kWaves = filter_waves(DP, ACCUM);
    const int grid = (int)std::min<int64_t>((n_units + kWaves - 1) / kWaves, (int64_t)ctx->n_cu);
    unsigned long long* stats = nullptr;
    rs = filter_stats_buffer(ctx, &stats);
    if (rs != MSM_OK) return rs;
    auto kern = mean ? kmeans_filter_kernel<T, DP, NF, ACCUM, true> : kmeans_filter_kernel<T, DP, NF, ACCUM, false>;
    if (lds > 48 * 1024)
        MSM_HIP(ctx, hipFuncSetAttribute((const void*)kern, hipFuncAttributeMaxDynamicSharedMemorySize, (int)lds));
    hipLaunchKernelGGL(kern, dim3(grid), dim3(64 * kWaves), lds, ctx->stream, x, n, d, ld, k, mean, stdv, image, centers,
                       labels, mindist, st, sums, counts, stats, stats ? upd_centers : nullptr,
                       stats ? (unsigned int*)(stats + 1) : nullptr);
    MSM_CHECK_LAUNCH(ctx);
    return MSM_OK;
}

template <typename T, bool ACCUM>
msm_status launch_filter(msm_ctx* ctx, const T* x, int64_t n, int d, int64_t ld, const double* centers, int k,
                         const double* mean, const double* stdv, const uint4* image, int32_t* labels, double* mindist,
                         const FitState* st, unsigned long long* sums, unsigned long long* counts, double* upd_centers) {
    if (filter_dp(d) == 4)
        return launch_filter_dp<T, 4, ACCUM>(ctx, x, n, d, ld, centers, k, mean, stdv, image, labels, mindist, st, sums,
                                             counts, upd_centers);
    return launch_filter_dp<T, 10, ACCUM>(ctx, x, n, d, ld, centers, k, mean, stdv, image, labels, mindist, st, sums, counts,
                                          upd_centers);
}

bool filter_fits(int k, int d, bool accum) { return filter_enabled() && d <= kFilterMaxD && filter_lds_bytes(k, d, accum) != 0; }

template <typename T, bool ACCUM>
msm_status dispatch_mfma(msm_ctx* ctx, const T* x, int64_t n, int d, int64_t ld, const double* centers, int k,
                         const double* mean, const double* stdv, int32_t* labels, double* mindist, const FitState* st,
                         unsigned long long* sums, unsigned long long* counts, const void* image = nullptr,
                         double* upd_centers = nullptr, bool* folded = nullptr) {
    if (folded) *folded = false;
    if (filter_fits(k, d, ACCUM)) {
        if (getenv("MSM_KMEANS_DEBUG"))
            fprintf(stderr, "msm_kmeans: filter T=%s n=%lld d=%d k=%d ACCUM=%d\n", sizeof(T) == 4 ? "f32" : "f64", (long long)n,
                    d, k, (int)ACCUM);
        if (!image) {
            msm_status rs = msm_reserve_km_image(ctx, filter_image_bytes(n, d));
            if (rs != MSM_OK) return rs;
            rs = launch_pack<T>(ctx, x, n, d, ld, mean, stdv, nullptr, (uint4*)ctx->km_image);
            if (rs != MSM_OK) return rs;
            image = ctx->km_image;
        }
        if (upd_centers && !(ACCUM && (int64_t)k * d <= kUpdateWide && (ctx->km_stats || !ctx->capturing))) upd_centers = nullptr;
        if (folded) *folded = upd_centers != nullptr;
        return launch_filter<T, ACCUM>(ctx, x, n, d, ld, centers, k, mean, stdv, (const uint4*)image, labels, mindist, st,
                                       sums, counts, upd_centers);
    }
#define MSM_MFMA_CASE(KSV) \
    if (d <= 4 * KSV)      \
        return launch_mfma<T, KSV, ACCUM>(ctx, x, n, d, ld, centers, k, mean, stdv, labels, mindist, st, sums, counts)
    MSM_MFMA_CASE(1);
    MSM_MFMA_CASE(2);
    MSM_MFMA_CASE(3);
    MSM_MFMA_CASE(4);
    MSM_MFMA_CASE(6);
    MSM_MFMA_CASE(8);
    MSM_MFMA_CASE(12);
    MSM_MFMA_CASE(16);
    MSM_MFMA_CASE(24);
    MSM_MFMA_CASE(32);
    MSM_MFMA_CASE(48);
    MSM_MFMA_CASE(64);
#undef MSM_MFMA_CASE
    return msm_fail(ctx, MSM_ERR_UNSUPPORTED, "k-means: d=%d > 256 not supported", d);
}

msm_status mfma_probe(msm_ctx* ctx, bool f16, const uint16_t* h_a, const uint16_t* h_b, const float* h_c, float* h_d,
                      int n_tiles) {
    if (!ctx) return MSM_ERR_INVALID;
    MSM_REQUIRE(ctx, n_tiles >= 1 && h_a && h_b && h_c && h_d, "msm_mfma_probe: bad arguments");
    const size_t na = (size_t)n_tiles * 512 * sizeof(uint16_t), nc = (size_t)n_tiles * 256 * sizeof(float);
    msm_status rs = msm_reserve_scratch(ctx, 2 * na + 2 * nc);
    if (rs != MSM_OK) return rs;
    unsigned char* base = (unsigned char*)ctx->scratch;
    uint16_t* d_a = (uint16_t*)base;
    uint16_t* d_b = (uint16_t*)(base + na);
    float* d_c = (float*)(base + 2 * na);
    float* d_d = (float*)(base + 2 * na + nc);
    MSM_HIP(ctx, hipMemcpyAsync(d_a, h_a, na, hipMemcpyHostToDevice, ctx->stream));
    MSM_HIP(ctx, hipMemcpyAsync(d_b, h_b, na, hipMemcpyHostToDevice, ctx->stream));
    MSM_HIP(ctx, hipMemcpyAsync(d_c, h_c, nc, hipMemcpyHostToDevice, ctx->stream));
    if (f16)
        hipLaunchKernelGGL(mfma_f16_probe_kernel, dim3((unsigned)n_tiles), dim3(64), 0, ctx->stream, d_a, d_b, d_c, d_d);
    else
        hipLaunchKernelGGL(mfma_bf16_probe_kernel, dim3((unsigned)n_tiles), dim3(64), 0, ctx->stream, d_a, d_b, d_c, d_d);
    MSM_CHECK_LAUNCH(ctx);
    MSM_HIP(ctx, hipMemcpyAsync(h_d, d_d, nc, hipMemcpyDeviceToHost, ctx->stream));
    MSM_HIP(ctx, hipStreamSynchronize(ctx->stream));
    return MSM_OK;
}

}

extern "C" {

static msm_status kmeans_assign_impl(msm_ctx* ctx, const void* d_x, msm_dtype dtype, int64_t n, int d, int64_t ld,
                                     const double* d_centers, int k, const double* d_mean, const double* d_std,
                                     const void* d_image, int32_t* d_labels, double* d_mindist) {
    if (!ctx) return MSM_ERR_INVALID;
    MSM_REQUIRE(ctx, n >= 0 && d >= 1 && k >= 1, "msm_kmeans_assign: need n >= 0, d >= 1, k >= 1");
    MSM_REQUIRE(ctx, ld >= d, "msm_kmeans_assign: ld (%lld) < d (%d)", (long long)ld, d);
    MSM_REQUIRE(ctx, (d_mean == nullptr) == (d_std == nullptr),
                "msm_kmeans_assign: mean and std must both be given or both be NULL");
    MSM_REQUIRE(ctx, dtype == MSM_F32 || dtype == MSM_F64, "msm_kmeans_assign: bad dtype");
    if (n == 0) return MSM_OK;
    MSM_REQUIRE(ctx, d_x && d_centers && d_labels, "msm_kmeans_assign: NULL pointer");
    if (dtype == MSM_F32)
        return dispatch_mfma<float, false>(ctx, (const float*)d_x, n, d, ld, d_centers, k, d_mean, d_std, d_labels,
                                           d_mindist, nullptr, nullptr, nullptr, d_image);
    return dispatch_mfma<double, false>(ctx, (const double*)d_x, n, d, ld, d_centers, k, d_mean, d_std, d_labels,
                                        d_mindist, nullptr, nullptr, nullptr, d_image);
}

msm_status msm_kmeans_assign(msm_ctx* ctx, const void* d_x, msm_dtype dtype, int64_t n, int d, int64_t ld,
                             const double* d_centers, int k, const double* d_mean, const double* d_std,
                             int32_t* d_labels, double* d_mindist) {
    return kmeans_assign_impl(ctx, d_x, dtype, n, d, ld, d_centers, k, d_mean, d_std, nullptr, d_labels, d_mindist);
}

msm_status msm_kmeans_assign_packed(msm_ctx* ctx, const void* d_x, msm_dtype dtype, int64_t n, int d, int64_t ld,
                                    const double* d_centers, int k, const double* d_mean, const double* d_std,
                                    const void* d_image, int32_t* d_labels, double* d_mindist) {
    return kmeans_assign_impl(ctx, d_x, dtype, n, d, ld, d_centers, k, d_mean, d_std, d_image, d_labels, d_mindist);
}

msm_status msm_kmeans_image_bytes(int64_t n, int d, size_t* out_bytes) {
    if (!out_bytes || n < 0 || d < 1) return MSM_ERR_INVALID;
    *out_bytes = d <= kFilterMaxD ? filter_image_bytes(n, d) : 0;
    return MSM_OK;
}

msm_status msm_kmeans_pack(msm_ctx* ctx, const void* d_x, msm_dtype dtype, int64_t n, int d, int64_t ld,
                           const double* d_mean, const double* d_std, void* d_image) {
    return msm_kmeans_pack_bounded(ctx, d_x, dtype, n, d, ld, d_mean, d_std, nullptr, d_image);
}

msm_status msm_kmeans_pack_bounded(msm_ctx* ctx, const void* d_x, msm_dtype dtype, int64_t n, int d, int64_t ld,
                                   const double* d_mean, const double* d_std, const double* d_absmax, void* d_image) {
    if (!ctx) return MSM_ERR_INVALID;
    MSM_REQUIRE(ctx, n >= 0 && d >= 1 && d <= kFilterMaxD && ld >= d, "msm_kmeans_pack: need 1 <= d <= %d, ld >= d",
                kFilterMaxD);
    MSM_REQUIRE(ctx, (d_mean == nullptr) == (d_std == nullptr), "msm_kmeans_pack: mean/std must come together");
    MSM_REQUIRE(ctx, dtype == MSM_F32 || dtype == MSM_F64, "msm_kmeans_pack: bad dtype");
    if (n == 0) return MSM_OK;
    MSM_REQUIRE(ctx, d_x && d_image, "msm_kmeans_pack: NULL pointer");
    MSM_REQUIRE(ctx, ((uintptr_t)d_image & 15) == 0, "msm_kmeans_pack: the image must be 16-byte aligned");
    if (dtype == MSM_F32)
        return launch_pack<float>(ctx, (const float*)d_x, n, d, ld, d_mean, d_std, d_absmax, (uint4*)d_image);
    return launch_pack<double>(ctx, (const double*)d_x, n, d, ld, d_mean, d_std, d_absmax, (uint4*)d_image);
}

msm_status msm_kmeans_filter_scanned(msm_ctx* ctx, uint64_t* h_out, int reset) {
    if (!ctx || !h_out) return MSM_ERR_INVALID;
    *h_out = 0;
    if (!ctx->km_stats) return MSM_OK;
    MSM_HIP(ctx, hipStreamSynchronize(ctx->stream));
    MSM_HIP(ctx, hipMemcpy(h_out, ctx->km_stats, 8, hipMemcpyDeviceToHost));
    if (reset) MSM_HIP(ctx, hipMemset(ctx->km_stats, 0, 8));
    return MSM_OK;
}

msm_status msm_mfma_bf16_probe(msm_ctx* ctx, const uint16_t* h_a, const uint16_t* h_b, const float* h_c, float* h_d,
                               int n_tiles) {
    return mfma_probe(ctx, false, h_a, h_b, h_c, h_d, n_tiles);
}

msm_status msm_mfma_f16_probe(msm_ctx* ctx, const uint16_t* h_a, const uint16_t* h_b, const float* h_c, float* h_d,
                              int n_tiles) {
    return mfma_probe(ctx, true, h_a, h_b, h_c, h_d, n_tiles);
}

msm_status msm_kmeans_fit_begin(msm_ctx* ctx, const void* d_x, msm_dtype dtype, int64_t n, int d, int64_t ld,
                                const double* d_mean, const double* d_std, int k, uint64_t seed, int init_centers,
                                double n_total, double tol2, double* d_centers, double* d_state, int absmax_ready) {
    if (!ctx) return MSM_ERR_INVALID;
    MSM_REQUIRE(ctx, n >= 1 && d >= 1 && d <= 256 && k >= 1 && ld >= d, "msm_kmeans_fit_begin: bad shape");
    MSM_REQUIRE(ctx, !absmax_ready || !d_mean, "msm_kmeans_fit_begin: a precomputed max |x| excludes whitening");
    MSM_REQUIRE(ctx, !init_centers || n >= k, "msm_kmeans_fit_begin: fewer frames (%lld) than centres (%d)",
                (long long)n, k);
    MSM_REQUIRE(ctx, (d_mean == nullptr) == (d_std == nullptr), "msm_kmeans_fit_begin: mean/std must come together");
    MSM_REQUIRE(ctx, d_x && d_centers && d_state, "msm_kmeans_fit_begin: NULL pointer");
    MSM_REQUIRE(ctx, dtype == MSM_F32 || dtype == MSM_F64, "msm_kmeans_fit_begin: bad dtype");
    MSM_REQUIRE(ctx, n_total >= (double)n && tol2 >= 0.0, "msm_kmeans_fit_begin: bad n_total / tol2");
    unsigned long long* bits = (unsigned long long*)(d_state + 2);
    if (!absmax_ready) {
        MSM_HIP(ctx, hipMemsetAsync(bits, 0, sizeof(unsigned long long), ctx->stream));
        const int grid = (int)std::min<int64_t>((n * d + kThreads * 8 - 1) / (kThreads * 8), (int64_t)ctx->n_cu * 8);
        if (dtype == MSM_F32)
            hipLaunchKernelGGL(absmax_kernel<float>, dim3(grid), dim3(kThreads), 0, ctx->stream, (const float*)d_x, n, d,
                               ld, d_mean, d_std, bits);
        else
            hipLaunchKernelGGL(absmax_kernel<double>, dim3(grid), dim3(kThreads), 0, ctx->stream, (const double*)d_x, n,
                               d, ld, d_mean, d_std, bits);
        MSM_CHECK_LAUNCH(ctx);
    }
    if (!init_centers) {
        hipLaunchKernelGGL(fit_scale_kernel, dim3(1), dim3(64), 0, ctx->stream, bits, n_total, tol2, (FitState*)d_state);
        MSM_CHECK_LAUNCH(ctx);
    }
    if (init_centers) {
        const int g2 = msm_ceil_div((int64_t)k * d, 256);
        if (dtype == MSM_F32)
            hipLaunchKernelGGL(init_centers_kernel<float>, dim3(g2), dim3(256), 0, ctx->stream, (const float*)d_x, n, d,
                               ld, d_mean, d_std, k, (unsigned long long)seed, d_centers, bits, n_total, tol2,
                               (FitState*)d_state);
        else
            hipLaunchKernelGGL(init_centers_kernel<double>, dim3(g2), dim3(256), 0, ctx->stream, (const double*)d_x, n,
                               d, ld, d_mean, d_std, k, (unsigned long long)seed, d_centers, bits, n_total, tol2,
                               (FitState*)d_state);
        MSM_CHECK_LAUNCH(ctx);
    }
    return MSM_OK;
}

static msm_status kmeans_accumulate_impl(msm_ctx* ctx, const void* d_x, msm_dtype dtype, int64_t n, int d, int64_t ld,
                                         const double* d_centers, int k, const double* d_mean, const double* d_std,
                                         const void* d_image, const double* d_state, int64_t* d_sums, int64_t* d_counts,
                                         int32_t* d_prev_labels = nullptr, double* d_update_centers = nullptr,
                                         bool* folded = nullptr) {
    if (folded) *folded = false;
    if (!ctx) return MSM_ERR_INVALID;
    MSM_REQUIRE(ctx, n >= 0 && d >= 1 && k >= 1 && ld >= d, "msm_kmeans_accumulate: bad shape");
    MSM_REQUIRE(ctx, (d_mean == nullptr) == (d_std == nullptr), "msm_kmeans_accumulate: mean/std must come together");
    MSM_REQUIRE(ctx, dtype == MSM_F32 || dtype == MSM_F64, "msm_kmeans_accumulate: bad dtype");
    if (n == 0) return MSM_OK;
    MSM_REQUIRE(ctx, d_x && d_centers && d_state && d_sums && d_counts, "msm_kmeans_accumulate: NULL pointer");
    if (dtype == MSM_F32)
        return dispatch_mfma<float, true>(ctx, (const float*)d_x, n, d, ld, d_centers, k, d_mean, d_std, d_prev_labels,
                                          nullptr, (const FitState*)d_state, (unsigned long long*)d_sums,
                                          (unsigned long long*)d_counts, d_image, d_update_centers, folded);
    return dispatch_mfma<double, true>(ctx, (const double*)d_x, n, d, ld, d_centers, k, d_mean, d_std, d_prev_labels,
                                       nullptr, (const FitState*)d_state, (unsigned long long*)d_sums,
                                       (unsigned long long*)d_counts, d_image, d_update_centers, folded);
}

msm_status msm_kmeans_lloyd_pass(msm_ctx* ctx, const void* d_x, msm_dtype dtype, int64_t n, int d, int64_t ld,
                                 double* d_centers, int k, const double* d_mean, const double* d_std, const void* d_image,
                                 double* d_state, int32_t* d_prev_labels, int64_t* d_sums, int64_t* d_counts) {
    bool folded = false;
    msm_status rs = kmeans_accumulate_impl(ctx, d_x, dtype, n, d, ld, d_centers, k, d_mean, d_std, d_image, d_state, d_sums,
                                           d_counts, d_prev_labels, d_centers, &folded);
    if (rs != MSM_OK || folded) return rs;
    return msm_kmeans_update(ctx, d_sums, d_counts, k, d, d_centers, d_state, 0);
}

msm_status msm_kmeans_accumulate_delta(msm_ctx* ctx, const void* d_x, msm_dtype dtype, int64_t n, int d, int64_t ld,
                                       const double* d_centers, int k, const double* d_mean, const double* d_std,
                                       const void* d_image, const double* d_state, int32_t* d_prev_labels,
                                       int64_t* d_sums, int64_t* d_counts) {
    if (!ctx) return MSM_ERR_INVALID;
    MSM_REQUIRE(ctx, d_prev_labels || n == 0, "msm_kmeans_accumulate_delta: NULL label buffer");
    return kmeans_accumulate_impl(ctx, d_x, dtype, n, d, ld, d_centers, k, d_mean, d_std, d_image, d_state, d_sums,
                                  d_counts, d_prev_labels);
}

msm_status msm_kmeans_accumulate(msm_ctx* ctx, const void* d_x, msm_dtype dtype, int64_t n, int d, int64_t ld,
                                 const double* d_centers, int k, const double* d_mean, const double* d_std,
                                 const double* d_state, int64_t* d_sums, int64_t* d_counts) {
    return kmeans_accumulate_impl(ctx, d_x, dtype, n, d, ld, d_centers, k, d_mean, d_std, nullptr, d_state, d_sums,
                                  d_counts);
}

msm_status msm_kmeans_accumulate_packed(msm_ctx* ctx, const void* d_x, msm_dtype dtype, int64_t n, int d, int64_t ld,
                                        const double* d_centers, int k, const double* d_mean, const double* d_std,
                                        const void* d_image, const double* d_state, int64_t* d_sums,
                                        int64_t* d_counts) {
    return kmeans_accumulate_impl(ctx, d_x, dtype, n, d, ld, d_centers, k, d_mean, d_std, d_image, d_state, d_sums,
                                  d_counts);
}

msm_status msm_kmeans_update(msm_ctx* ctx, int64_t* d_sums, int64_t* d_counts, int k, int d, double* d_centers,
                             double* d_state, int clear) {
    if (!ctx) return MSM_ERR_INVALID;
    MSM_REQUIRE(ctx, k >= 1 && d >= 1, "msm_kmeans_update: bad shape");
    MSM_REQUIRE(ctx, d_sums && d_counts && d_centers && d_state, "msm_kmeans_update: NULL pointer");
    if ((int64_t)k * d > kUpdateWide) {
        const int nb = std::min(k, ctx->n_cu);
        const int cpb = (k + nb - 1) / nb;
        const int nblocks = (k + cpb - 1) / cpb;
        msm_status rs = msm_reserve_aux(ctx, (size_t)nblocks * sizeof(double));
        if (rs != MSM_OK) return rs;
        hipLaunchKernelGGL(kmeans_update_wide_kernel, dim3(nblocks), dim3(1024), 0, ctx->stream, (unsigned long long*)d_sums,
                           (unsigned long long*)d_counts, k, d, cpb, d_centers, (const FitState*)d_state, clear,
                           (double*)ctx->aux);
        MSM_CHECK_LAUNCH(ctx);
        hipLaunchKernelGGL(kmeans_update_finish_kernel, dim3(1), dim3(64), 0, ctx->stream, (const double*)ctx->aux, nblocks,
                           (FitState*)d_state);
        MSM_CHECK_LAUNCH(ctx);
        return MSM_OK;
    }
    hipLaunchKernelGGL(kmeans_update_kernel, dim3(1), dim3(1024), 0, ctx->stream, (unsigned long long*)d_sums,
                       (unsigned long long*)d_counts, k, d, d_centers, (FitState*)d_state, clear);
    MSM_CHECK_LAUNCH(ctx);
    return MSM_OK;
}

msm_status msm_kmeans_fit(msm_ctx* ctx, const void* d_x, msm_dtype dtype, int64_t n, int d, int64_t ld,
                          const double* d_mean, const double* d_std, int k, uint64_t seed, int init_centers,
                          int max_iter, double tol2, double* d_centers, double* d_state) {
    if (!ctx) return MSM_ERR_INVALID;
    MSM_REQUIRE(ctx, max_iter >= 0, "msm_kmeans_fit: max_iter must be >= 0");
    msm_status rs = msm_kmeans_fit_begin(ctx, d_x, dtype, n, d, ld, d_mean, d_std, k, seed, init_centers, (double)n,
                                         tol2, d_centers, d_state, 0);
    if (rs != MSM_OK) return rs;
    const size_t acc_bytes = ((size_t)k * (d + 1) * sizeof(unsigned long long) + 15) & ~(size_t)15;
    rs = msm_reserve_scratch(ctx, acc_bytes + (size_t)n * sizeof(int32_t));
    if (rs != MSM_OK) return rs;
    int64_t* sums = (int64_t*)ctx->scratch;
    int64_t* counts = sums + (size_t)k * d;
    int32_t* prev = (int32_t*)((char*)ctx->scratch + acc_bytes);
    MSM_HIP(ctx, hipMemsetAsync(sums, 0, acc_bytes, ctx->stream));
    MSM_HIP(ctx, hipMemsetAsync(prev, 0xFF, (size_t)n * sizeof(int32_t), ctx->stream));
    const void* image = nullptr;
    if (max_iter > 0 && filter_fits(k, d, true)) {
        rs = msm_reserve_km_image(ctx, filter_image_bytes(n, d));
        if (rs != MSM_OK) return rs;
        rs = msm_kmeans_pack(ctx, d_x, dtype, n, d, ld, d_mean, d_std, ctx->km_image);
        if (rs != MSM_OK) return rs;
        image = ctx->km_image;
    }
    for (int it = 0; it < max_iter; ++it) {
        rs = msm_kmeans_lloyd_pass(ctx, d_x, dtype, n, d, ld, d_centers, k, d_mean, d_std, image, d_state, prev, sums, counts);
        if (rs != MSM_OK) return rs;
    }
    return MSM_OK;
}
// ... 16 lines not shown
```

pmarlo_amd/csrc/kmeans_filter.h:

```cpp
#pragma once

typedef __bf16 v8bf __attribute__((ext_vector_type(8)));
typedef _Float16 v8h __attribute__((ext_vector_type(8)));
typedef float v4f32 __attribute__((ext_vector_type(4)));

#ifdef MSM_KMF_WAVES
__host__ __device__ constexpr int filter_waves(int, bool) { return MSM_KMF_WAVES; }
#else
__host__ __device__ constexpr int filter_waves(int dp, bool heavy) { return dp == 10 && heavy ? 12 : 16; }
#endif
constexpr int kFilterMaxD = 10;
constexpr int kFilterRowQ = 3;
constexpr double kFilterHi = 1e18;
constexpr double kFilterScaledHi = 16384.0;
constexpr double kF16MinNormal = 6.103515625e-05;
constexpr int kFilterScaleTop = 13;
constexpr double kFilterKappa = 52.0 * 5.9604644775390625e-08;
constexpr float kPickEps = 20.0f * 5.9604644775390625e-08f;
constexpr float kPickFloor = 1e-30f;
constexpr float kUp20 = 1.0f + 9.5367431640625e-07f;
constexpr double kUp20d = 1.0 + 9.5367431640625e-07;

__host__ __device__ inline int filter_scale_exp(double amax) {
    if (!(amax > 0.0) || !(amax <= 1.7976931348623157e308)) return 0;
// ... 241 lines not shown
__device__ __forceinline__ void filter_load_frame(const T* __restrict__ x, int64_t ld, int d, bool vec_rows,
                                                  const double* __restrict__ mean, const double* __restrict__ stdv,
                                                  int64_t t, double (&z)[DP]) {
    const T* row = x + t * ld;
    if (vec_rows) {
        const double2* r2 = reinterpret_cast<const double2*>(row);
#pragma unroll
        for (int f2 = 0; f2 < DP / 2; ++f2) {
            const double2 v = r2[f2];
            z[2 * f2] = v.x;
            z[2 * f2 + 1] = v.y;
        }
    } else {
#pragma unroll
        for (int f = 0; f < DP; ++f) {
            const double v = load_as_f64(row + (f < d ? f : d - 1));
            z[f] = f < d ? v : 0.0;
        }
    }
    if constexpr (WHITEN) {
#pragma unroll
        for (int f = 0; f < DP; ++f) {
            const int fc = f < d ? f : d - 1;
            const double w = (z[f] - mean[fc]) / stdv[fc];
            z[f] = f < d ? w : 0.0;
        }
    }
}

template <int MT>
__device__ __forceinline__ void filter_close_iteration(const unsigned long long* sums, const unsigned long long* counts, int k,
                                                       int d, double* centers, FitState* st) {
    __shared__ double red[16];
    const int tid = threadIdx.x;
    const double inv_scale = st->inv_scale;
    for (int v0 = 0; v0 < 1024; v0 += MT) {
        const int v = v0 + tid;
        if (v < 1024) {
            double acc = 0.0;
            constexpr int CH = 4;
            for (int i0 = v; i0 < k * d; i0 += 1024 * CH) {
                long long cnt[CH], sm[CH];
                double old[CH];
#pragma unroll
                for (int c = 0; c < CH; ++c) {
                    const int i = i0 + c * 1024;
                    cnt[c] = 0;
                    if (i < k * d) {
                        cnt[c] = (long long)__hip_atomic_load(&counts[i / d], __ATOMIC_RELAXED, __HIP_MEMORY_SCOPE_AGENT);
                        sm[c] = (long long)__hip_atomic_load(&sums[i], __ATOMIC_RELAXED, __HIP_MEMORY_SCOPE_AGENT);
                        old[c] = centers[i];
                    }
                }
#pragma unroll
                for (int c = 0; c < CH; ++c)
                    if (cnt[c] > 0) {
                        const double c_new = (double)sm[c] * inv_scale / (double)cnt[c];
                        const double dlt = c_new - old[c];
                        acc = fma(dlt, dlt, acc);
                        centers[i0 + c * 1024] = c_new;
                    }
            }
            for (int off = 32; off > 0; off >>= 1) acc += __shfl_down(acc, off, 64);
            if ((v & 63) == 0) red[v >> 6] = acc;
        }
    }
    __syncthreads();
    if (tid == 0) {
        double t = 0.0;
        for (int i = 0; i < 16; ++i) t += red[i];
        st->shift2 = t;
        st->n_iter += 1.0;
        if (t <= st->tol2) st->done = 1.0;
    }
}

template <typename T, int DP, int NF, bool ACCUM, bool WHITEN>
__global__ __launch_bounds__(64 * filter_waves(DP, ACCUM)) void kmeans_filter_kernel(
    const T* __restrict__ x, int64_t n, int d, int64_t ld, int k, const double* __restrict__ mean,
    const double* __restrict__ stdv, const uint4* __restrict__ image, const double* __restrict__ centers,
    int32_t* __restrict__ labels,
    double* __restrict__ mindist, const FitState* __restrict__ st, unsigned long long* __restrict__ sums,
    unsigned long long* __restrict__ counts, unsigned long long* __restrict__ n_scanned, double* upd_centers,
    unsigned int* __restrict__ ticket) {
    using S = FilterShape<DP>;
    constexpr int kFilterWaves = filter_waves(DP, ACCUM);
    constexpr int kMT = 64 * kFilterWaves, RF = S::RF, RQ = kFilterRowQ;
    static_assert(NF == 4, "one frame group per lane quarter: a unit is 64 frames, one per lane in the candidate pick");
    extern __shared__ __attribute__((aligned(16))) unsigned char smem_raw[];
    if constexpr (ACCUM) {
        if (st->done != 0.0) return;
    }
    const int k16 = (k + 15) & ~15;
    const int n_tiles = ((k16 / 16) + 1) & ~1;
    uint4* img = reinterpret_cast<uint4*>(smem_raw);
    float* tab = reinterpret_cast<float*>(img + (size_t)n_tiles * 64);
    float* cz = tab + (size_t)n_tiles * 16 * RF;
    double* hs = reinterpret_cast<double*>(cz + (size_t)n_tiles * 16);
    unsigned long long* lsum = reinterpret_cast<unsigned long long*>(hs + (size_t)n_tiles * 16);
    unsigned long long* lcnt = lsum + (ACCUM ? (size_t)k * d : 0);
    __shared__ int unit_ctr;
    __shared__ int any_bad;
    __shared__ unsigned long long cmax_bits;
    const int tid = threadIdx.x, lane = tid & 63, wave = __builtin_amdgcn_readfirstlane(tid >> 6);
    const int j16 = lane & 15, q = lane >> 4;
    const double scale = ACCUM ? st->scale : 0.0;
    if (tid == 0) {
        unit_ctr = kFilterWaves;
        any_bad = 0;
        cmax_bits = 0ull;
    }
    KSTAMP_INIT
    if constexpr (ACCUM) {
        for (int i = tid; i < k * (d + 1); i += kMT) lsum[i] = 0ull;
    }
    __syncthreads();
    constexpr int kUnit = 16 * NF;
    const int64_t n_units = (n + kUnit - 1) / kUnit;
    const int64_t units_per_block = (n_units + gridDim.x - 1) / gridDim.x;
    const int64_t u_begin = (int64_t)blockIdx.x * units_per_block;
    const int64_t u_end = min(n_units, u_begin + units_per_block);
    const int voff = j16 * RQ + filter_piece(q);
    const int ex = reinterpret_cast<const int*>(image + (size_t)((n + 63) & ~(int64_t)63) * RQ)[2];

    int64_t unit = u_begin + wave;
    v8h b[NF];
    auto load_images = [&](int64_t un) {
        const uint4* ub = image + un * (kUnit * RQ);
#pragma unroll
        for (int u = 0; u < NF; ++u) b[u] = __builtin_bit_cast(v8h, ub[voff + u * 16 * RQ]);
    };
    if (unit < u_end) load_images(unit);

    {
        double cm = 0.0;
        for (int i = tid; i < k * d; i += kMT) cm = fmax(cm, fabs(centers[i]));
        cm = wave_max_f64(cm);
        if (lane == 0 && cm > 0.0) atomicMax(&cmax_bits, (unsigned long long)__double_as_longlong(cm));
    }
    __syncthreads();
    const int ec = __builtin_amdgcn_readfirstlane(filter_scale_exp(__longlong_as_double((long long)cmax_bits)));
    const int exc = ex + ec;
    for (int t = wave; t < n_tiles; t += 2 * kFilterWaves) {
        const int t2 = t + kFilterWaves;
        double c0[kStageRegs], c1[kStageRegs], r0[DP], r1[DP];
        filter_stage_fetch<DP>(t, lane, centers, k, d, c0, r0);
        if (t2 < n_tiles) filter_stage_fetch<DP>(t2, lane, centers, k, d, c1, r1);
        filter_stage_build<DP>(t, lane, reinterpret_cast<unsigned short*>(img + (size_t)t * 64), c0, r0, k, d, ec, exc, tab, cz,
                               hs, &any_bad);
        if (t2 < n_tiles)
            filter_stage_build<DP>(t2, lane, reinterpret_cast<unsigned short*>(img + (size_t)t2 * 64), c1, r1, k, d, ec, exc, tab,
                                   cz, hs, &any_bad);
    }
    __syncthreads();
    const float inv_scale_u = __int_as_float((127 - exc) << 23);
    const bool all_scan = __builtin_amdgcn_readfirstlane(any_bad) != 0;
    KSTAMP(0);

    unsigned long long my_scans = 0;
    const bool vec_rows = sizeof(T) == 8 && d == DP && ((ld * sizeof(T)) & 15) == 0 && (((uintptr_t)x) & 15) == 0;
    const int iters = n_tiles / 2;
    constexpr int kNone = 0x7fffffff;

    auto load_frame = [&](int64_t t, double (&z)[DP]) { filter_load_frame<T, DP, WHITEN>(x, ld, d, vec_rows, mean, stdv, t, z); };
    auto score64 = [&](const double* crow, int c, const double (&z)[DP]) {
        double a = 0.0;
#pragma unroll
        for (int f = 0; f < DP; ++f)
            if (f < d) a = fma(crow[f], z[f], a);
        return a - hs[c];
    };
    auto write_label = [&](int64_t t, int bidx, double bm, const double (&z)[DP]) {
        labels[t] = bidx;
        if (mindist) {
            double zsq = 0.0;
#pragma unroll
            for (int f = 0; f < DP; ++f) zsq = fma(z[f], z[f], zsq);
            const double md = -2.0 * bm + zsq;
            mindist[t] = md > 0.0 ? md : 0.0;
        }
    };
    auto commit_scan = [&](int64_t t, int sbi, double sbest, const double (&zz)[DP], int old_s) {
        if constexpr (ACCUM) {
            if (!labels || old_s != sbi) {
#pragma unroll
                for (int f = 0; f < DP; ++f) {
                    if (f < d && lane == f) {
                        const unsigned long long fx = (unsigned long long)to_fixed(zz[f], scale);
                        atomicAdd(&lsum[(size_t)sbi * d + f], fx);
                        if (old_s >= 0) atomicAdd(&lsum[(size_t)old_s * d + f], 0ull - fx);
                    }
                }
                if (lane == 0) {
                    atomicAdd(&lcnt[sbi], 1ull);
                    if (old_s >= 0) atomicAdd(&lcnt[old_s], ~0ull);
                    if (labels) labels[t] = sbi;
                }
            }
        } else {
            if (lane == 0) write_label(t, sbi, sbest, zz);
        }
    };
    auto scan_frame = [&](int64_t t) {
        double zz[DP];
        load_frame(t, zz);
        double sbest = -__builtin_inf();
        int sbi = kNone;
        for (int c = lane; c < k; c += 64) {
            const double sc = score64(centers + (size_t)c * d, c, zz);
            if (sc > sbest) { sbest = sc; sbi = c; }
        }
#pragma unroll
        for (int off = 1; off < 64; off <<= 1) {
            const double ob = __shfl_xor(sbest, off, 64);
            const int oi = __shfl_xor(sbi, off, 64);
            if (ob > sbest || (ob == sbest && oi < sbi)) { sbest = ob; sbi = oi; }
        }
        if (sbi >= k) { sbi = 0; sbest = -__builtin_inf(); }
        int old_s = -1;
        if constexpr (ACCUM) {
            if (labels) old_s = labels[t];
        }
        commit_scan(t, sbi, sbest, zz, old_s);
#ifdef MSM_KMF_DIAG_COUNT
        if (MSM_KMF_DIAG_COUNT == 1) ++my_scans;
#else
        ++my_scans;
#endif
    };

    while (unit < u_end) {
        int nt = 0;
        if (lane == 0) nt = atomicAdd(&unit_ctr, 1);
        const int64_t nxt = u_begin + __builtin_amdgcn_readfirstlane(nt);
        KSTAMP_VM(1);
        float b1[NF], b2[NF];
        int bp[NF];
#pragma unroll
        for (int u = 0; u < NF; ++u) { b1[u] = -__builtin_inff(); b2[u] = -__builtin_inff(); bp[u] = 0; }
#ifdef MSM_KMF_DIAG_NOTILE
        for (int it = 0; it < (iters < 9 ? iters : 9); ++it) {
#else
        for (int it = 0; it < iters; ++it) {
#endif
            const int jt = 2 * it;
            const v8h aa = __builtin_bit_cast(v8h, img[(jt + 0) * 64 + lane]);
            const v8h ab = __builtin_bit_cast(v8h, img[(jt + 1) * 64 + lane]);
            const v4f32 ca = *reinterpret_cast<const v4f32*>(cz + (jt + 0) * 16 + 4 * q);
            const v4f32 cb = *reinterpret_cast<const v4f32*>(cz + (jt + 1) * 16 + 4 * q);
            v4f32 acca[NF], accb[NF];
#pragma unroll
            for (int u = 0; u < NF; ++u) {
                acca[u] = __builtin_amdgcn_mfma_f32_16x16x32_f16(aa, b[u], ca, 0, 0, 0);
                accb[u] = __builtin_amdgcn_mfma_f32_16x16x32_f16(ab, b[u], cb, 0, 0, 0);
            }
#pragma unroll
            for (int u = 0; u < NF; ++u) {
                float m = max3_f32(b2[u], acca[u][0], acca[u][1]);
                m = max3_f32(m, acca[u][2], acca[u][3]);
                m = max3_f32(m, accb[u][0], accb[u][1]);
                m = max3_f32(m, accb[u][2], accb[u][3]);
                const bool better = m > b1[u];
                b2[u] = med3_f32(b1[u], b2[u], m);
                b1[u] = hw_max_f32(b1[u], m);
                bp[u] = better ? jt : bp[u];
            }
        }
        KSTAMP(2);
        bool guard[NF];
#pragma unroll
        for (int u = 0; u < NF; ++u) guard[u] = q == 3 && __builtin_bit_cast(unsigned short, b[u][7]) == 0x7C00;
        if (nxt < u_end) load_images(nxt);
        const int64_t f0 = unit * kUnit + lane;
        const bool fok = f0 < n;
        const int64_t fr = fok ? f0 : n - 1;
        int old = -1;
        if constexpr (ACCUM) {
            if (labels) old = labels[fr];
        }
        double z[DP];
        load_frame(fr, z);
        int cd = kNone;
        float Ru = __builtin_inff();
#ifdef MSM_KMF_DIAG_NOCROSS
        cd = bp[0] | (q << 16);
        Ru = b2[0] + b1[1] + b1[2] + b1[3] + b2[1] + b2[2] + b2[3] + (guard[0] | guard[1] | guard[2] | guard[3] ? 1.f : 0.f) + (float)(bp[1] + bp[2] + bp[3]);
#else
#pragma unroll
        for (int u = 0; u < NF; ++u) {
            const float M1 = xrow_max_f32(b1[u]);
            const int code_u = xrow_min_i32(b1[u] == M1 ? ((q << 16) | bp[u]) : kNone);
            const int gs = code_u >> 16;
            float r = q == gs ? b2[u] : b1[u];
            if (guard[u]) r = __builtin_inff();
            const float R_u = xrow_max_f32(r);
            cd = q == u ? code_u : cd;
            Ru = q == u ? R_u : Ru;
        }
#endif
        Ru = __builtin_fmaf(Ru, inv_scale_u, 1.40129846e-45f);
        KSTAMP(3);
        const int gs = cd >> 16, pstar = cd & 0xffff;
        const int base = min(pstar * 16 + 4 * gs, n_tiles * 16 - 20);
        float pz[DP];
        float qz = 0.f;
#pragma unroll
        for (int f = 0; f < DP; ++f) {
            pz[f] = (float)z[f];
            qz = __builtin_fmaf(pz[f], pz[f], qz);
        }
        const bool z_bad = !(qz < __builtin_inff());
        const float zn = hw_max_f32(__builtin_amdgcn_sqrtf(qz) * kUp20, 1.0f);
        float s1 = -__builtin_inff(), s2 = -__builtin_inff(), sbmax = 0.f;
        int i1 = 0;
#ifndef MSM_KMF_DIAG_NOPICK
        const float* p_row = tab + (size_t)base * RF;
#pragma unroll
        for (int c = 0; c < 8; ++c) {
            const float4* r4 = reinterpret_cast<const float4*>(p_row + ((c & 3) + 16 * (c >> 2)) * RF);
            float a = 0.f, h, cn;
            if constexpr (DP == 4) {
                const float4 r0 = r4[0], r1 = r4[1];
                a = __builtin_fmaf(r0.x, pz[0], a);
                a = __builtin_fmaf(r0.y, pz[1], a);
                a = __builtin_fmaf(r0.z, pz[2], a);
                a = __builtin_fmaf(r0.w, pz[3], a);
                h = r1.x;
                cn = r1.y;
            } else {
                const float4 r0 = r4[0], r1 = r4[1], r2 = r4[2];
                a = __builtin_fmaf(r0.x, pz[0], a);
                a = __builtin_fmaf(r0.y, pz[1], a);
                a = __builtin_fmaf(r0.z, pz[2], a);
                a = __builtin_fmaf(r0.w, pz[3], a);
                a = __builtin_fmaf(r1.x, pz[4], a);
                a = __builtin_fmaf(r1.y, pz[5], a);
                a = __builtin_fmaf(r1.z, pz[6], a);
                a = __builtin_fmaf(r1.w, pz[7], a);
                a = __builtin_fmaf(r2.x, pz[8], a);
                a = __builtin_fmaf(r2.y, pz[9], a);
                h = r2.z;
                cn = r2.w;
            }
            const float s = a - h;
            sbmax = hw_max_f32(sbmax, __builtin_fmaf(zn, cn, h));
            const bool better = s > s1;
            s2 = med3_f32(s1, s2, s);
            s1 = hw_max_f32(s1, s);
            i1 = better ? c : i1;
        }
#endif
        const float e = __builtin_fmaf(kPickEps, sbmax, kPickFloor);
        const int jw = base + (i1 & 3) + 16 * (i1 >> 2);
        const bool certified = !all_scan && !z_bad && cd != kNone && jw < k && s1 - s2 > 2.0f * e && s1 - e > Ru;
        const int lab = jw;
#if defined(MSM_KMF_DIAG_NOSCAN) || defined(MSM_KMF_DIAG_NOQUEUE)
        unsigned long long todo = 0;
#else
        unsigned long long todo = __ballot(fok && !certified);
#endif
        KSTAMP(4);
// ... 168 lines not shown
```

pmarlo_amd/csrc/moments.hip:

```cpp
#include "common.h"
#include "wave.h"

namespace {

constexpr int kThreads = 256;

template <typename T>
__device__ __forceinline__ double ld_f64(const T* p) { return (double)(*p); }

template <typename T>
__global__ __launch_bounds__(kThreads) void moments_partial_kernel(
    const T* __restrict__ x, int64_t n, int F, int64_t ld, const double* __restrict__ shift_in,
    int tf, int64_t rows_per_block, double* __restrict__ partial) {
    extern __shared__ __attribute__((aligned(16))) unsigned char smem_raw[];
    double* red = reinterpret_cast<double*>(smem_raw);
    const int tid = threadIdx.x;
    const int fx = tid % tf;
    const int ry = tid / tf;
    const int rp = kThreads / tf;
    const int64_t r0 = (int64_t)blockIdx.x * rows_per_block;
    const int64_t r1 = min(r0 + rows_per_block, n);
    double* out = partial + (size_t)blockIdx.x * 3 * F;
    for (int f0 = 0; f0 < F; f0 += tf) {
        const int f = f0 + fx;
        double cnt = 0.0, s1 = 0.0, s2 = 0.0;
        if (f < F) {
            double sh;
            if (shift_in) sh = shift_in[f];
            else { sh = ld_f64(x + f); if (sh != sh) sh = 0.0; }
            int64_t r = r0 + ry;
            for (; r + 3 * rp < r1; r += 4 * rp) {
                double v[4];
#pragma unroll
                for (int u = 0; u < 4; ++u) v[u] = ld_f64(x + (r + (int64_t)u * rp) * ld + f);
#pragma unroll
                for (int u = 0; u < 4; ++u) {
                    if (v[u] == v[u]) { const double dlt = v[u] - sh; cnt += 1.0; s1 += dlt; s2 = fma(dlt, dlt, s2); }
                }
            }
            for (; r < r1; r += rp) {
                const double v = ld_f64(x + r * ld + f);
                if (v == v) { const double dlt = v - sh; cnt += 1.0; s1 += dlt; s2 = fma(dlt, dlt, s2); }
            }
        }
        red[tid] = cnt; red[kThreads + tid] = s1; red[2 * kThreads + tid] = s2;
        __syncthreads();
        if (ry == 0 && f < F) {
            for (int y = 1; y < rp; ++y) {
                cnt += red[y * tf + fx]; s1 += red[kThreads + y * tf + fx]; s2 += red[2 * kThreads + y * tf + fx];
            }
            out[f] = cnt; out[F + f] = s1; out[2 * F + f] = s2;
        }
        __syncthreads();
    }
}

template <typename T>
__global__ __launch_bounds__(1024) void moments_reduce_kernel(const double* __restrict__ partial, int n_blocks, int F,
                                                             const T* __restrict__ x,
                                                             const double* __restrict__ shift_in,
                                                             double* __restrict__ sums, double* __restrict__ shift_out) {
    __shared__ double red[16][64];
    const int io = threadIdx.x & 63, g = threadIdx.x >> 6;
    const int i = blockIdx.x * 64 + io;
    double acc = 0.0;
    if (i < 3 * F)
        for (int b = g; b < n_blocks; b += 16) acc += partial[(size_t)b * 3 * F + i];
    red[g][io] = acc;
    __syncthreads();
    if (g == 0 && i < 3 * F) {
        double t = 0.0;
        for (int k = 0; k < 16; ++k) t += red[k][io];
        sums[i] = t;
    }
    if (g == 1 && i < F && shift_out) {
        double sh;
        if (shift_in) sh = shift_in[i];
        else { sh = ld_f64(x + i); if (sh != sh) sh = 0.0; }
        shift_out[i] = sh;
    }
}

__global__ void moments_finalize_kernel(const double* __restrict__ sums, const double* __restrict__ shift, int F,
                                        int ddof, double* __restrict__ mean, double* __restrict__ stdv,
                                        double* __restrict__ count) {
    const int f = blockIdx.x * blockDim.x + threadIdx.x;
    if (f >= F) return;
    const double cnt = sums[f], s1 = sums[F + f], s2 = sums[2 * F + f];
    double m = 0.0, sd = 0.0;
    if (cnt > 0.0) {
        m = shift[f] + s1 / cnt;
        const double denom = cnt - (double)ddof;
        if (denom > 0.0) {
            double var = (s2 - s1 * s1 / cnt) / denom;
            sd = var > 0.0 ? sqrt(var) : 0.0;
        } else {
            sd = __builtin_nan("");
        }
    }
    mean[f] = m;
    stdv[f] = sd;
    if (count) count[f] = cnt;
}

__global__ void standardise_params_kernel(const double* __restrict__ sums, const double* __restrict__ shift, int F,
                                          double n_rows, int with_std, double* __restrict__ mean,
                                          double* __restrict__ scale, double* __restrict__ inv_scale) {
    const int f = blockIdx.x * blockDim.x + threadIdx.x;
    if (f >= F) return;
    const double cnt = sums[f], s1 = sums[F + f], s2 = sums[2 * F + f];
    double m = 0.0, sd = 1.0;
    if (cnt > 0.0) {
        m = shift[f] + s1 / cnt;
        if (with_std) {
            const double var = (s2 - s1 * s1 / cnt) / n_rows;
            sd = var > 0.0 ? sqrt(var) : 0.0;
            if (sd < 10.0 * 2.220446049250313e-16) sd = 1.0;
        }
    }
    mean[f] = m;
    scale[f] = sd;
    inv_scale[f] = 1.0 / sd;
}

constexpr int kProjFrames = 64;
constexpr int kProjFT = 64;

__device__ __forceinline__ void publish_absmax(double m, unsigned long long* __restrict__ bits, double* red) {
    if (!bits) return;
    m = wave_max_down(m);
    __syncthreads();
    if ((threadIdx.x & 63) == 0) red[threadIdx.x >> 6] = m;
    __syncthreads();
    if (threadIdx.x == 0) {
        for (int w = 1; w < kThreads / 64; ++w) m = fmax(m, red[w]);
        const unsigned long long b = (unsigned long long)__double_as_longlong(m);
        if (b > *bits) atomicMax(bits, b);
    }
}

template <typename T>
__global__ __launch_bounds__(kThreads) void project_kernel(
    const T* __restrict__ x, int64_t n, int F, int64_t ld, const double* __restrict__ mu,
    const double* __restrict__ inv_sigma, const double* __restrict__ m2, const double* __restrict__ W, int d,
    int64_t ldw, double* __restrict__ y, int64_t ldy, unsigned long long* __restrict__ absmax_bits) {
    extern __shared__ __attribute__((aligned(16))) unsigned char smem_raw[];
    double amax = 0.0;
    double* zs = reinterpret_cast<double*>(smem_raw);
    double* ws = zs + kProjFrames * (kProjFT + 1);
    const int tid = threadIdx.x;
    const int r = tid & 63;
    const int cg = tid >> 6;
    const int64_t n_tiles = (n + kProjFrames - 1) / kProjFrames;
    constexpr int kMaxCols = 16;
    for (int64_t tile = blockIdx.x; tile < n_tiles; tile += gridDim.x) {
        const int64_t t0 = tile * kProjFrames;
        const int rows = (int)min<int64_t>(kProjFrames, n - t0);
        double acc[kMaxCols];
#pragma unroll
        for (int c = 0; c < kMaxCols; ++c) acc[c] = 0.0;
        for (int f0 = 0; f0 < F; f0 += kProjFT) {
            const int fc = min(kProjFT, F - f0);
            __syncthreads();
            for (int i = tid; i < rows * fc; i += kThreads) {
                const int rr = i / fc, ff = i - rr * fc;
                double v = ld_f64(x + (t0 + rr) * ld + f0 + ff);
                double z = (v - mu[f0 + ff]) * inv_sigma[f0 + ff];
                if (v != v) z = 0.0;
                if (m2) z -= m2[f0 + ff];
                zs[rr * (kProjFT + 1) + ff] = z;
            }
            for (int i = tid; i < fc * d; i += kThreads) {
                const int ff = i / d, c = i - ff * d;
                ws[i] = W[(size_t)(f0 + ff) * ldw + c];
            }
            __syncthreads();
            if (r < rows) {
                const double* zr = zs + r * (kProjFT + 1);
#pragma unroll
                for (int ci = 0; ci < kMaxCols; ++ci) {
                    const int c = cg + 4 * ci;
                    if (c < d) {
                        double a = acc[ci];
                        for (int ff = 0; ff < fc; ++ff) a = fma(zr[ff], ws[ff * d + c], a);
                        acc[ci] = a;
                    }
                }
            }
        }
        if (r < rows) {
#pragma unroll
            for (int ci = 0; ci < kMaxCols; ++ci) {
                const int c = cg + 4 * ci;
                if (c < d) {
                    y[(t0 + r) * ldy + c] = acc[ci];
                    amax = fmax(amax, fabs(acc[ci]));
                }
            }
        }
    }
    publish_absmax(amax, absmax_bits, zs);
}
// ... 225 lines not shown

extern "C" {

msm_status msm_column_moments_partial(msm_ctx* ctx, const void* d_x, msm_dtype dtype, int64_t n, int F,
                                      int64_t ld, const double* d_shift, double* d_sums, double* d_shift_out) {
    if (!ctx) return MSM_ERR_INVALID;
    MSM_REQUIRE(ctx, n >= 1 && F >= 1 && ld >= F, "msm_column_moments_partial: need n >= 1, F >= 1, ld >= F");
    MSM_REQUIRE(ctx, d_x && d_sums, "msm_column_moments_partial: NULL pointer");
    MSM_REQUIRE(ctx, dtype == MSM_F32 || dtype == MSM_F64, "msm_column_moments_partial: bad dtype");
    if (dtype == MSM_F32)
        return moments_partial_impl<float>(ctx, (const float*)d_x, n, F, ld, d_shift, d_sums, d_shift_out);
    return moments_partial_impl<double>(ctx, (const double*)d_x, n, F, ld, d_shift, d_sums, d_shift_out);
}

msm_status msm_moments_finalize(msm_ctx* ctx, const double* d_sums, const double* d_shift, int F, int ddof,
                                double* d_mean, double* d_std, double* d_count) {
    if (!ctx) return MSM_ERR_INVALID;
    MSM_REQUIRE(ctx, F >= 1 && ddof >= 0, "msm_moments_finalize: need F >= 1, ddof >= 0");
    MSM_REQUIRE(ctx, d_sums && d_shift && d_mean && d_std, "msm_moments_finalize: NULL pointer");
    hipLaunchKernelGGL(moments_finalize_kernel, dim3(msm_ceil_div(F, 256)), dim3(256), 0, ctx->stream, d_sums, d_shift,
                       F, ddof, d_mean, d_std, d_count);
    MSM_CHECK_LAUNCH(ctx);
    return MSM_OK;
}

msm_status msm_standardise_params(msm_ctx* ctx, const double* d_sums, const double* d_shift, int F, double n_rows,
                                  int with_std, double* d_mean, double* d_scale, double* d_inv_scale) {
    if (!ctx) return MSM_ERR_INVALID;
    MSM_REQUIRE(ctx, F >= 1 && n_rows >= 1.0, "msm_standardise_params: need F >= 1, n_rows >= 1");
    MSM_REQUIRE(ctx, d_sums && d_shift && d_mean && d_scale && d_inv_scale, "msm_standardise_params: NULL pointer");
    hipLaunchKernelGGL(standardise_params_kernel, dim3(msm_ceil_div(F, 256)), dim3(256), 0, ctx->stream, d_sums, d_shift,
                       F, n_rows, with_std, d_mean, d_scale, d_inv_scale);
    MSM_CHECK_LAUNCH(ctx);
    return MSM_OK;
}

msm_status msm_column_minmax(msm_ctx* ctx, const void* d_x, msm_dtype dtype, int64_t n, int F, int64_t ld, double* d_min,
                             double* d_max, int64_t* d_counts) {
    if (!ctx) return MSM_ERR_INVALID;
    MSM_REQUIRE(ctx, n >= 0 && F >= 1 && ld >= F, "msm_column_minmax: bad shape");
    MSM_REQUIRE(ctx, F <= 4096, "msm_column_minmax: at most 4096 columns per call (F = %d)", F);
    MSM_REQUIRE(ctx, dtype == MSM_F32 || dtype == MSM_F64, "msm_column_minmax: bad dtype");
    MSM_REQUIRE(ctx, d_min && d_max && d_counts && (d_x || n == 0), "msm_column_minmax: NULL pointer");
    msm_status rs = msm_reserve_scratch(ctx, (size_t)2 * F * sizeof(unsigned long long));
    if (rs != MSM_OK) return rs;
    unsigned long long* gmin = (unsigned long long*)ctx->scratch;
    unsigned long long* gmax = gmin + F;
    MSM_HIP(ctx, hipMemsetAsync(gmin, 0xFF, (size_t)F * sizeof(unsigned long long), ctx->stream));
    MSM_HIP(ctx, hipMemsetAsync(gmax, 0, (size_t)F * sizeof(unsigned long long), ctx->stream));
    MSM_HIP(ctx, hipMemsetAsync(d_counts, 0, 2 * sizeof(int64_t), ctx->stream));
    if (n > 0) {
        const int grid = (int)std::min<int64_t>((n + 255) / 256, (int64_t)ctx->n_cu * 8);
        const size_t lds = (size_t)2 * F * sizeof(unsigned long long);
        if (dtype == MSM_F32)
            hipLaunchKernelGGL(column_minmax_kernel<float>, dim3(grid), dim3(256), lds, ctx->stream, (const float*)d_x, n, F, ld,
                               gmin, gmax, (unsigned long long*)d_counts);
        else
            hipLaunchKernelGGL(column_minmax_kernel<double>, dim3(grid), dim3(256), lds, ctx->stream, (const double*)d_x, n, F, ld,
                               gmin, gmax, (unsigned long long*)d_counts);
        MSM_CHECK_LAUNCH(ctx);
    }
    hipLaunchKernelGGL(column_minmax_finish_kernel, dim3((F + 63) / 64), dim3(64), 0, ctx->stream, gmin, gmax, F, d_min, d_max);
    MSM_CHECK_LAUNCH(ctx);
    return MSM_OK;
}

msm_status msm_column_moments(msm_ctx* ctx, const void* d_x, msm_dtype dtype, int64_t n, int F, int64_t ld, int ddof,
                              double* d_mean, double* d_std, double* d_count) {
    if (!ctx) return MSM_ERR_INVALID;
    MSM_REQUIRE(ctx, F >= 1, "msm_column_moments: F must be >= 1");
    const size_t tail = (size_t)4 * F * sizeof(double);
    const size_t head = (size_t)ctx->n_cu * 8 * 3 * F * sizeof(double);
    msm_status rs = msm_reserve_scratch(ctx, head + tail);
    if (rs != MSM_OK) return rs;
    double* sums = (double*)((char*)ctx->scratch + head);
    double* shift = sums + 3 * F;
    rs = msm_column_moments_partial(ctx, d_x, dtype, n, F, ld, nullptr, sums, shift);
    if (rs != MSM_OK) return rs;
    return msm_moments_finalize(ctx, sums, shift, F, ddof, d_mean, d_std, d_count);
}

static msm_status project_impl(msm_ctx* ctx, const void* d_x, msm_dtype dtype, int64_t n, int F, int64_t ld,
                               const double* d_mu, const double* d_inv_sigma, const double* d_mean2, const double* d_w, int d,
                               int64_t ldw, double* d_y, int64_t ldy, double* d_absmax, bool finite) {
    if (!ctx) return MSM_ERR_INVALID;
    MSM_REQUIRE(ctx, n >= 0 && F >= 1 && d >= 1 && d <= 64, "msm_project: need n >= 0, F >= 1, 1 <= d <= 64");
    unsigned long long* bits = reinterpret_cast<unsigned long long*>(d_absmax);
    if (bits) MSM_HIP(ctx, hipMemsetAsync(bits, 0, sizeof(unsigned long long), ctx->stream));
    MSM_REQUIRE(ctx, ld >= F && ldw >= d && ldy >= d, "msm_project: bad leading dimension");
    MSM_REQUIRE(ctx, dtype == MSM_F32 || dtype == MSM_F64, "msm_project: bad dtype");
    if (n == 0) return MSM_OK;
    MSM_REQUIRE(ctx, d_x && d_mu && d_inv_sigma && d_w && d_y, "msm_project: NULL pointer");
    if (d <= 16 && ((size_t)((F + 15) & ~15) * 17 + 16) * sizeof(double) <= 48 * 1024) {
        const int64_t n_groups = (n + 15) / 16;
        const size_t esz = dtype == MSM_F32 ? 4 : 8;
        const int F16 = (F + 15) & ~15;
        const size_t plds = ((size_t)F16 * 17 + 16) * sizeof(double);
        const bool vec = (F % 16 == 0) && (ld % 4 == 0) && (((uintptr_t)d_x) % (4 * esz) == 0);
#define MSM_PROJ(T, V, FIN)                                                                                    \
        do {                                                                                                   \
            int per_cu = 0;                                                                                    \
            MSM_HIP(ctx, hipOccupancyMaxActiveBlocksPerMultiprocessor(&per_cu, project_mfma_kernel<T, V, FIN>, kThreads, plds)); \
            const int grid = (int)std::min<int64_t>((n_groups + 3) / 4, (int64_t)ctx->n_cu * std::max(per_cu, 1)); \
            hipLaunchKernelGGL((project_mfma_kernel<T, V, FIN>), dim3(grid), dim3(kThreads), plds, ctx->stream, (const T*)d_x, n, \
                               F, ld, d_mu, d_inv_sigma, d_mean2, d_w, d, ldw, d_y, ldy, bits);                \
        } while (0)
        if (dtype == MSM_F32) { if (vec && finite) MSM_PROJ(float, true, true); else if (vec) MSM_PROJ(float, true, false); else MSM_PROJ(float, false, false); }
        else { if (vec && finite) MSM_PROJ(double, true, true); else if (vec) MSM_PROJ(double, true, false); else MSM_PROJ(double, false, false); }
#undef MSM_PROJ
        MSM_CHECK_LAUNCH(ctx);
        return MSM_OK;
    }
    const size_t lds = ((size_t)kProjFrames * (kProjFT + 1) + (size_t)kProjFT * d) * sizeof(double);
    const int64_t n_tiles = (n + kProjFrames - 1) / kProjFrames;
    const int grid = (int)std::min<int64_t>(n_tiles, (int64_t)ctx->n_cu * 8);
    if (lds > 48 * 1024) {
        MSM_HIP(ctx, hipFuncSetAttribute((const void*)project_kernel<float>,
                                         hipFuncAttributeMaxDynamicSharedMemorySize, (int)lds));
        MSM_HIP(ctx, hipFuncSetAttribute((const void*)project_kernel<double>,
                                         hipFuncAttributeMaxDynamicSharedMemorySize, (int)lds));
    }
    if (dtype == MSM_F32)
        hipLaunchKernelGGL(project_kernel<float>, dim3(grid), dim3(kThreads), lds, ctx->stream, (const float*)d_x, n, F,
                           ld, d_mu, d_inv_sigma, d_mean2, d_w, d, ldw, d_y, ldy, bits);
    else
        hipLaunchKernelGGL(project_kernel<double>, dim3(grid), dim3(kThreads), lds, ctx->stream, (const double*)d_x, n,
                           F, ld, d_mu, d_inv_sigma, d_mean2, d_w, d, ldw, d_y, ldy, bits);
    MSM_CHECK_LAUNCH(ctx);
    return MSM_OK;
}

msm_status msm_project(msm_ctx* ctx, const void* d_x, msm_dtype dtype, int64_t n, int F, int64_t ld,
                       const double* d_mu, const double* d_inv_sigma, const double* d_mean2, const double* d_w, int d,
                       int64_t ldw, double* d_y, int64_t ldy, double* d_absmax) {
    return project_impl(ctx, d_x, dtype, n, F, ld, d_mu, d_inv_sigma, d_mean2, d_w, d, ldw, d_y, ldy, d_absmax, false);
}

msm_status msm_project_finite(msm_ctx* ctx, const void* d_x, msm_dtype dtype, int64_t n, int F, int64_t ld,
                              const double* d_mu, const double* d_inv_sigma, const double* d_mean2, const double* d_w,
                              int d, int64_t ldw, double* d_y, int64_t ldy, double* d_absmax) {
    return project_impl(ctx, d_x, dtype, n, F, ld, d_mu, d_inv_sigma, d_mean2, d_w, d, ldw, d_y, ldy, d_absmax, true);
}

}
```

pmarlo_amd/device.py:

```python

from __future__ import annotations

import ctypes as C
import os
import sys
from typing import Iterable, Sequence

import numpy as np

from . import _lib
from ._lib import check, lib

__all__ = ["Engine", "DeviceArray", "get_engine", "segments_to_bounds"]


def _dtype_code(dtype: np.dtype) -> int:
    dtype = np.dtype(dtype)
    if dtype == np.float32:
        return _lib.MSM_F32
    if dtype == np.float64:
        return _lib.MSM_F64
    raise TypeError(f"feature matrices must be float32 or float64, got {dtype}")


# ... 432 lines not shown
                                       cnt.ptr), self.handle)
        return mean, std, cnt

    def standardise_params(self, sums: DeviceArray, shift: DeviceArray, F: int, n_rows: float, with_std: bool = True,
                           out=None):
        mean, scale, inv = out if out is not None else tuple(self.empty((F,), np.float64) for _ in range(3))
        check(lib.msm_standardise_params(self.handle, sums.ptr, shift.ptr, F, float(n_rows), int(bool(with_std)),
                                         mean.ptr, scale.ptr, inv.ptr), self.handle)
        return mean, scale, inv

    def lagged_moments(self, x: DeviceArray, lag: int, shift: DeviceArray, *, starts=None, stops=None,
                       assume_finite: bool = False, out: DeviceArray | None = None,
                       one_sided: bool = False, symmetric: bool = False, ld: int | None = None) -> DeviceArray:
        if one_sided and symmetric:
            raise ValueError("one_sided and symmetric moments exclude each other")
        n, F = x.shape
        if starts is None:
            starts, stops = segments_to_bounds(None, n)
        starts, stops = self._seg_ptrs(starts, stops)
        out = out if out is not None else self.empty((2 * F * F + 2 * F + 1,), np.float64)
        fn = (lib.msm_lagged_moments_onesided if one_sided
              else lib.msm_lagged_moments_reversible if symmetric else lib.msm_lagged_moments)
        check(fn(self.handle, x.ptr, _dtype_code(x.dtype), n, F, int(F if ld is None else ld), starts.ctypes.data,
                 stops.ctypes.data, len(starts), int(lag), shift.ptr, int(bool(assume_finite)), out.ptr), self.handle)
        return out

    def autocorr_lagscan(self, x: DeviceArray, lags: Sequence[int], *, starts=None, stops=None,
                         var_floor: float = 1e-8, ld: int | None = None):
        n, F = x.shape
        lags_arr = np.ascontiguousarray(lags, np.int64).reshape(-1)
        if lags_arr.size and (lags_arr.min() < 1 or lags_arr.max() > np.iinfo(np.int32).max):
            raise ValueError("lags must be integers in [1, 2^31)")
        lags_arr = lags_arr.astype(np.int32)
        if starts is None:
            starts, stops = segments_to_bounds(None, n)
        starts, stops = self._seg_ptrs(starts, stops)
        value = self.empty((len(starts), len(lags_arr)), np.float64)
        nvalid = self.empty((len(starts),), np.int32)
        check(lib.msm_autocorr_lagscan(self.handle, x.ptr, _dtype_code(x.dtype), n, F, int(F if ld is None else ld),
                                       starts.ctypes.data, stops.ctypes.data, len(starts), lags_arr.ctypes.data,
                                       len(lags_arr), float(var_floor), value.ptr, nvalid.ptr), self.handle)
        return value, nvalid

    def hstack(self, a: DeviceArray, b: DeviceArray) -> DeviceArray:
        (n, pa), (nb, pb) = a.shape, b.shape
        if n != nb:
            raise ValueError(f"hstack: row counts differ ({n} vs {nb})")
        out = self.empty((n, pa + pb), np.float64)
        check(lib.msm_hstack_f64(self.handle, a.ptr, _dtype_code(a.dtype), pa, pa, b.ptr, _dtype_code(b.dtype), pb, pb,
                                 n, out.ptr), self.handle)
        return out

    def onesided_tica_eigenvalues(self, moments: DeviceArray, F: int, clip: float = 1e-12) -> DeviceArray:
        out = self.empty((F,), np.float64)
        check(lib.msm_onesided_tica_eigenvalues(self.handle, moments.ptr, int(F), float(clip), out.ptr), self.handle)
        return out

    def moments_from_lagged(self, x: DeviceArray, lag: int, shift: DeviceArray, moments: DeviceArray, *, starts=None,
                            stops=None, out: DeviceArray | None = None, ld: int | None = None) -> DeviceArray:
        n, F = x.shape
        if starts is None:
            starts, stops = segments_to_bounds(None, n)
        starts, stops = self._seg_ptrs(starts, stops)
        out = out if out is not None else self.empty((3 * F,), np.float64)
        check(lib.msm_moments_from_lagged(self.handle, x.ptr, _dtype_code(x.dtype), n, F, int(F if ld is None else ld),
                                          starts.ctypes.data, stops.ctypes.data, len(starts), int(lag), shift.ptr,
                                          moments.ptr, out.ptr), self.handle)
        return out

    def tica_solve(self, moments: DeviceArray, F: int, *, scale: DeviceArray | None = None,
                   epsilon: float = 1e-6, kinetic_map: bool = True, out=None):
        if out is not None:
            eig, W, mean, rank = out
        else:
            eig = self.empty((F,), np.float64)
            W = self.empty((F, F), np.float64)
            mean = self.empty((F,), np.float64)
            rank = self.empty((1,), np.int32)
        check(lib.msm_tica_solve(self.handle, moments.ptr, scale.ptr if scale is not None else None, F,
                                 float(epsilon), int(bool(kinetic_map)), eig.ptr, W.ptr, mean.ptr, rank.ptr),
              self.handle)
        return eig, W, mean, rank

    def project(self, x: DeviceArray, mu: DeviceArray, inv_sigma: DeviceArray, W: DeviceArray, d: int, *,
                mean2: DeviceArray | None = None, out: DeviceArray | None = None,
                absmax: DeviceArray | None = None, assume_finite: bool = False, ld: int | None = None) -> DeviceArray:
        n, F = x.shape
        ldw = W.shape[1]
        out = out if out is not None else self.empty((n, d), np.float64)
        fn = lib.msm_project_finite if assume_finite else lib.msm_project
        check(fn(self.handle, x.ptr, _dtype_code(x.dtype), n, F, int(F if ld is None else ld), mu.ptr, inv_sigma.ptr,
                 mean2.ptr if mean2 is not None else None, W.ptr, int(d), ldw, out.ptr,
                 out.shape[1], absmax.ptr if absmax is not None else None), self.handle)
        return out

    def eigh(self, a: DeviceArray, want_vectors: bool = True):
        n = a.shape[0]
        w = self.empty((n,), np.float64)
        v = self.empty((n, n), np.float64) if want_vectors else None
        sweeps = self.empty((1,), np.int32)
        check(lib.msm_eigh(self.handle, a.ptr, n, w.ptr, v.ptr if v is not None else None, sweeps.ptr),
              self.handle)
        return w, v, sweeps

    def kmeans_assign(self, x: DeviceArray, centers: DeviceArray, *, mean: DeviceArray | None = None,
                      std: DeviceArray | None = None, labels: DeviceArray | None = None,
                      mindist: DeviceArray | None = None, image: DeviceArray | None = None) -> DeviceArray:
        n, d = x.shape
        k, dc = centers.shape
        if dc != d:
            raise ValueError(f"centres have {dc} features, data has {d}")
        if centers.dtype != np.float64:
            raise TypeError("centres must be float64")
        labels = labels if labels is not None else self.empty((n,), np.int32)
        check(lib.msm_kmeans_assign_packed(self.handle, x.ptr, _dtype_code(x.dtype), n, d, d, centers.ptr, k,
                                           mean.ptr if mean is not None else None,
                                           std.ptr if std is not None else None,
                                           image.ptr if image is not None else None, labels.ptr,
                                           mindist.ptr if mindist is not None else None), self.handle)
        return labels


    FIT_STATE_FIELDS = ("scale", "inv_scale", "absmax", "shift2", "tol2", "done", "n_iter", "inertia")

    def kmeans_fit(self, x: DeviceArray, k: int, *, seed: int = 0, max_iter: int = 50, tol2: float = 0.0,
                   mean: DeviceArray | None = None, std: DeviceArray | None = None,
                   centers: DeviceArray | None = None) -> tuple[DeviceArray, DeviceArray]:
        n, d = x.shape
        init = centers is None
        centers = centers if centers is not None else self.empty((k, d), np.float64)
        state = self.zeros((8,), np.float64)
        check(lib.msm_kmeans_fit(self.handle, x.ptr, _dtype_code(x.dtype), n, d, d,
                                 mean.ptr if mean is not None else None, std.ptr if std is not None else None,
                                 int(k), int(seed) & (2**64 - 1), int(init), int(max_iter), float(tol2), centers.ptr,
                                 state.ptr), self.handle)
        return centers, state

    def kmeans_init_plusplus(self, x: DeviceArray, k: int, *, seed: int = 0, mean: DeviceArray | None = None,
                             std: DeviceArray | None = None, n_total: int | None = None,
                             centers: DeviceArray | None = None, return_picked: bool = False):
        n, d = x.shape
        n_total = n if n_total is None else int(n_total)
        centers, state = self.kmeans_fit_begin(x, k, seed=seed, n_total=n_total, tol2=0.0, mean=mean, std=std,
                                               centers=centers, init_centers=False)
        picked = self.empty((k,), np.int64) if return_picked else None
        check(lib.msm_kmeans_init_plusplus(self.handle, x.ptr, _dtype_code(x.dtype), n, d, d,
                                           mean.ptr if mean is not None else None, std.ptr if std is not None else None,
                                           int(k), int(seed) & (2**64 - 1), float(n_total), centers.ptr, state.ptr,
                                           picked.ptr if picked is not None else None), self.handle)
        return (centers, picked) if return_picked else centers

    def kmeans_fit_minibatch(self, x: DeviceArray, k: int, *, seed: int = 0, batch_size: int = 100, max_iter: int = 5,
                             init: str = "kmeans++", centers: DeviceArray | None = None,
                             max_batches: int = 4096) -> tuple[DeviceArray, DeviceArray]:
        n, d = x.shape
        if batch_size < 1 or max_iter < 0:
            raise ValueError("batch_size must be >= 1 and max_iter >= 0")
        given = centers is not None
        n_terms = n * max(1, int(max_iter))
        centers, state = self.kmeans_fit_begin(x, k, seed=seed, n_total=n_terms, tol2=0.0, centers=centers,
                                               init_centers=not given and init != "kmeans++")
        if not given and init == "kmeans++":
            check(lib.msm_kmeans_init_plusplus(self.handle, x.ptr, _dtype_code(x.dtype), n, d, d, None, None, int(k),
                                               int(seed) & (2**64 - 1), float(n_terms), centers.ptr, state.ptr, None),
                  self.handle)
        nb = max(1, min(int(max_batches), -(-n // int(batch_size))))
        sums, counts = self.zeros((k * d,), np.int64), self.zeros((k,), np.int64)
        item = x.dtype.itemsize
        for _ in range(int(max_iter)):
            for b in range(nb):
                rows = (n - b + nb - 1) // nb
                if rows <= 0:
                    continue
                check(lib.msm_kmeans_accumulate(self.handle, x.ptr + b * d * item, _dtype_code(x.dtype), rows, d, nb * d,
                                                centers.ptr, k, None, None, state.ptr, sums.ptr, counts.ptr), self.handle)
                check(lib.msm_kmeans_update(self.handle, sums.ptr, counts.ptr, k, d, centers.ptr, state.ptr, 0), self.handle)
        return centers, state

    def kmeans_fit_begin(self, x: DeviceArray, k: int, *, seed: int, n_total: int, tol2: float,
                         mean: DeviceArray | None = None, std: DeviceArray | None = None,
                         centers: DeviceArray | None = None, init_centers: bool = True,
                         state: DeviceArray | None = None, absmax_ready: bool = False):
        n, d = x.shape
        centers = centers if centers is not None else self.empty((k, d), np.float64)
        state = state if state is not None else self.zeros((8,), np.float64)
        check(lib.msm_kmeans_fit_begin(self.handle, x.ptr, _dtype_code(x.dtype), n, d, d,
                                       mean.ptr if mean is not None else None,
                                       std.ptr if std is not None else None, int(k), int(seed) & (2**64 - 1),
                                       int(bool(init_centers)), float(n_total), float(tol2), centers.ptr, state.ptr,
                                       int(bool(absmax_ready))), self.handle)
        return centers, state

    def kmeans_accumulate(self, x: DeviceArray, centers: DeviceArray, state: DeviceArray, sums: DeviceArray,
                          counts: DeviceArray, *, mean: DeviceArray | None = None, std: DeviceArray | None = None,
                          image: DeviceArray | None = None, prev_labels: DeviceArray | None = None):
        n, d = x.shape
        k = centers.shape[0]
        if prev_labels is not None:
            check(lib.msm_kmeans_accumulate_delta(self.handle, x.ptr, _dtype_code(x.dtype), n, d, d, centers.ptr, k,
                                                  mean.ptr if mean is not None else None,
                                                  std.ptr if std is not None else None,
                                                  image.ptr if image is not None else None, state.ptr,
                                                  prev_labels.ptr, sums.ptr, counts.ptr), self.handle)
            return
        check(lib.msm_kmeans_accumulate_packed(self.handle, x.ptr, _dtype_code(x.dtype), n, d, d, centers.ptr, k,
                                               mean.ptr if mean is not None else None,
                                               std.ptr if std is not None else None,
                                               image.ptr if image is not None else None, state.ptr, sums.ptr,
                                               counts.ptr), self.handle)

    def kmeans_image_bytes(self, n: int, d: int) -> int:
        out = C.c_size_t(0)
        check(lib.msm_kmeans_image_bytes(int(n), int(d), C.byref(out)), self.handle)
        return int(out.value)

    def kmeans_pack(self, x: DeviceArray, *, mean: DeviceArray | None = None, std: DeviceArray | None = None,
                    image: DeviceArray | None = None, absmax: DeviceArray | None = None) -> DeviceArray | None:
        n, d = x.shape
        nbytes = self.kmeans_image_bytes(n, d)
        if nbytes == 0:
            return None
        image = image if image is not None else self.empty((nbytes,), np.uint8)
        if image.nbytes < nbytes:
            raise ValueError(f"image buffer holds {image.nbytes} bytes, {nbytes} needed")
        check(lib.msm_kmeans_pack_bounded(self.handle, x.ptr, _dtype_code(x.dtype), n, d, d,
                                          mean.ptr if mean is not None else None, std.ptr if std is not None else None,
                                          absmax.ptr if absmax is not None else None, image.ptr), self.handle)
        return image

    def kmeans_filter_scanned(self, reset: bool = False) -> int:
        out = C.c_uint64(0)
        check(lib.msm_kmeans_filter_scanned(self.handle, C.byref(out), int(reset)), self.handle)
        return int(out.value)

    def mfma_bf16_probe(self, a_bits: np.ndarray, b_bits: np.ndarray, c: np.ndarray) -> np.ndarray:
        return self._mfma_probe(lib.msm_mfma_bf16_probe, a_bits, b_bits, c)

    def mfma_f16_probe(self, a_bits: np.ndarray, b_bits: np.ndarray, c: np.ndarray) -> np.ndarray:
        return self._mfma_probe(lib.msm_mfma_f16_probe, a_bits, b_bits, c)

    def _mfma_probe(self, fn, a_bits: np.ndarray, b_bits: np.ndarray, c: np.ndarray) -> np.ndarray:
        a = np.ascontiguousarray(a_bits, np.uint16)
        b = np.ascontiguousarray(b_bits, np.uint16)
        cc = np.ascontiguousarray(c, np.float32)
        t = a.shape[0]
        if a.shape != (t, 16, 32) or b.shape != (t, 32, 16) or cc.shape != (t, 16, 16):
            raise ValueError("mfma probe: shapes must be [t,16,32], [t,32,16], [t,16,16]")
        out = np.empty((t, 16, 16), np.float32)
        check(fn(self.handle, a.ctypes.data, b.ctypes.data, cc.ctypes.data, out.ctypes.data, t), self.handle)
        return out

    def kmeans_lloyd_pass(self, x: DeviceArray, centers: DeviceArray, state: DeviceArray, sums: DeviceArray,
                          counts: DeviceArray, *, mean: DeviceArray | None = None, std: DeviceArray | None = None,
                          image: DeviceArray | None = None, prev_labels: DeviceArray | None = None):
        n, d = x.shape
        k = centers.shape[0]
        check(lib.msm_kmeans_lloyd_pass(self.handle, x.ptr, _dtype_code(x.dtype), n, d, d, centers.ptr, k,
                                        mean.ptr if mean is not None else None, std.ptr if std is not None else None,
                                        image.ptr if image is not None else None, state.ptr,
                                        prev_labels.ptr if prev_labels is not None else None, sums.ptr, counts.ptr),
              self.handle)

    def kmeans_update(self, sums: DeviceArray, counts: DeviceArray, centers: DeviceArray, state: DeviceArray,
                      clear: bool = True):
        k, d = centers.shape
        check(lib.msm_kmeans_update(self.handle, sums.ptr, counts.ptr, k, d, centers.ptr, state.ptr, int(clear)),
              self.handle)

    def sum_f64(self, v: DeviceArray, out: DeviceArray | None = None) -> DeviceArray:
        out = out if out is not None else self.empty((1,), np.float64)
        check(lib.msm_sum_f64(self.handle, v.ptr, v.size, out.ptr), self.handle)
        return out


    def transition_matrix(self, counts: DeviceArray, *, mode: int = 0, alpha: float = 1e-3,
                          epsilon: float = 1e-12) -> dict:
        k = counts.shape[0]
        if counts.dtype not in (np.dtype(np.int64), np.dtype(np.float64)):
            raise TypeError("counts must be int64 or float64")
        T = self.empty((k, k), np.float64)
        rowsum = self.empty((k,), np.float64)
        out = {"T": T, "rowsum": rowsum}
        if mode == 0:
            dm = self.empty((1,), np.float64)
            check(lib.msm_transition_matrix(self.handle, counts.ptr, int(counts.dtype == np.float64), k, 0, 0.0, 0.0,
                                            T.ptr, None, None, None, rowsum.ptr, dm.ptr), self.handle)
            out["diag_mass"] = dm
        else:
            active, inv = self.empty((k,), np.int32), self.empty((k,), np.int32)
            na = self.empty((1,), np.int32)
            check(lib.msm_transition_matrix(self.handle, counts.ptr, int(counts.dtype == np.float64), k, 1,
                                            float(alpha), float(epsilon), T.ptr, active.ptr, inv.ptr, na.ptr,
                                            rowsum.ptr, None), self.handle)
            out.update(active=active, inv_map=inv, n_active=na)
        return out

    def row_normalise_into(self, counts: DeviceArray, T: DeviceArray, rowsum: DeviceArray, diag_mass: DeviceArray):
        k = counts.shape[0]
        check(lib.msm_transition_matrix(self.handle, counts.ptr, int(counts.dtype == np.float64), k, 0, 0.0, 0.0,
                                        T.ptr, None, None, None, rowsum.ptr, diag_mass.ptr), self.handle)

    def rcp(self, src: DeviceArray, dst: DeviceArray) -> None:
        check(lib.msm_rcp_f64(self.handle, src.ptr, src.size, dst.ptr), self.handle)

    def embed_full(self, T_active: DeviceArray, inv_map: DeviceArray, pi_active: DeviceArray | None = None):
        k = T_active.shape[0]
        T_full = self.empty((k, k), np.float64)
        pi_full = self.empty((k,), np.float64)
        check(lib.msm_embed_full(self.handle, T_active.ptr, pi_active.ptr if pi_active is not None else None,
                                 inv_map.ptr, k, T_full.ptr, pi_full.ptr), self.handle)
        return T_full, pi_full

    def silhouette(self, x_sorted: DeviceArray, offsets) -> tuple[float, DeviceArray]:
        n, d = x_sorted.shape
        off = np.ascontiguousarray(offsets, np.int64)
        samples = self.empty((n,), np.float64)
        score = self.empty((1,), np.float64)
        check(lib.msm_silhouette(self.handle, x_sorted.ptr, n, d, d, off.ctypes.data, len(off) - 1, samples.ptr, score.ptr),
              self.handle)
        return float(score.to_host()[0]), samples

    def group_by_label(self, labels: DeviceArray, k: int) -> tuple[DeviceArray, DeviceArray]:
        n = labels.size
        offsets = self.empty((int(k) + 1,), np.int64)
        members = self.empty((n,), np.int32)
        check(lib.msm_group_by_label(self.handle, labels.ptr, n, int(k), offsets.ptr, members.ptr), self.handle)
        return offsets, members

    def state_centroids(self, x: DeviceArray, offsets: DeviceArray, members: DeviceArray,
                        weights: DeviceArray | None = None) -> tuple[DeviceArray, DeviceArray, DeviceArray]:
        n, d = x.shape
        k = offsets.size - 1
        cen, wsum, flags = self.empty((k, d), np.float64), self.empty((k,), np.float64), self.empty((k,), np.int32)
        check(lib.msm_state_centroids(self.handle, x.ptr, n, d, d, weights.ptr if weights is not None else None, offsets.ptr,
                                      members.ptr, k, cen.ptr, wsum.ptr, flags.ptr), self.handle)
        return cen, wsum, flags

    def state_scores(self, x: DeviceArray, labels: DeviceArray, offsets: DeviceArray, members: DeviceArray,
                     h_offsets: np.ndarray, *, centroid: DeviceArray | None = None, wsum: DeviceArray | None = None,
                     weights: DeviceArray | None = None, states=None) -> DeviceArray:
        n, d = x.shape
        k = offsets.size - 1
        ho = np.ascontiguousarray(h_offsets, np.int64)
        scores = self.empty((n,), np.float64)
# ... 381 lines not shown
```

pmarlo_amd/dist.py:

```python

from __future__ import annotations

import ctypes as C
import os
import time
from dataclasses import dataclass
from pathlib import Path

import numpy as np

from .device import DeviceArray, Engine

__all__ = ["Comm", "NativeComm", "TorchComm", "ShardedMSM", "ShardConfig", "exchange_shapes", "exchange_aliases",
           "torch_exchange_buffers", "bootstrap_id"]


class Comm:

    world = 1
    rank = 0

    def allreduce_sum(self, name: str) -> None: ...
    def allreduce_sum_from(self, name: str, src) -> None: ...
    def allreduce_min(self, name: str) -> None: ...
# ... 246 lines not shown
    L = 2 * F * F + 2 * F + 1
    return {"lagged": ("moments", 0, L), "mom_sums": ("moments", L, 3 * F),
            "fit_scale": ("fit_state", 0, 1), "fit_inv_scale": ("fit_state", 1, 1),
            "centers": ("start", 0, k * d), "start_scale": ("start", k * d, 1)}


class ShardedMSM:

    def __init__(self, engine: Engine, cfg: ShardConfig, x: DeviceArray, comm: Comm | None = None,
                 shared: dict[str, DeviceArray] | None = None, always_exchange: bool = False):
        self.eng, self.cfg = engine, cfg
        self.comm = comm
        self.always_exchange = bool(always_exchange) and comm is not None
        self.world = comm.world if comm else 1
        self.n_total = cfg.n_total if cfg.n_total is not None else cfg.n_frames * self.world
        eng = engine
        F, d, k, n = cfg.n_features, cfg.cluster_dim, cfg.k, cfg.n_frames
        self.buf = shared if shared is not None else {
            nm: eng.zeros(shape, np.dtype(dt)) for nm, (shape, dt) in exchange_shapes(cfg).items()}
        b = self.buf
        for name, (parent, first, length) in exchange_aliases(cfg).items():
            if name not in b:
                b[name] = b[parent].view((length,), offset_elems=first)
        b["centers"] = b["start"].view((k, d))
        if cfg.n_atoms > 0:
            if cfg.pairs is None or len(cfg.pairs) != F:
                raise ValueError("ShardConfig.pairs must list n_features atom pairs")
            self.xyz = x
            self.pairs_d = eng.to_device(np.ascontiguousarray(cfg.pairs, np.int32).reshape(F, 2))
            self.x = eng.empty((n, F), np.float32)
            eng.featurize_distances_into(self.xyz, self.pairs_d, self.x)
        else:
            self.xyz = None
            self.x = x
        if cfg.tica_dim > 0:
            self.mean, self.scale, self.inv_scale = (eng.empty((F,), np.float64) for _ in range(3))
            self.eig = eng.empty((F,), np.float64)
            self.W = eng.empty((F, F), np.float64)
            self.m2 = eng.empty((F,), np.float64)
            self.rank_d = eng.empty((1,), np.int32)
            self.Y = eng.empty((n, d), np.float64)
        else:
            self.Y = self.x
        self.labels = eng.empty((n,), np.int32)
        self.T = eng.empty((k, k), np.float64)
        self.rowsum = eng.empty((k,), np.float64)
        self.diag = eng.empty((1,), np.float64)
        self.km_sums = b["km_acc"].view((k * d,), np.int64)
        self.km_counts = b["km_acc"].view((k,), np.int64, offset_elems=k * d)
        multi_shard = self.comm is not None and (self.comm.world > 1 or self.always_exchange)
        self.km_local = eng.empty((k * d + k,), np.int64) if multi_shard else None
        nbytes = eng.kmeans_image_bytes(n, d)
        self.km_image = eng.empty((nbytes,), np.uint8) if nbytes else None
        self.accum_events: list = []
        self.stage_events: dict = {}
        self.time_accum = False
        self.time_stages = False
        if cfg.tica_dim > 0:
            _, first = eng.column_moments_partial(self.x)
            b["shift"].copy_from_host(first.to_host())
            if comm and (comm.world > 1 or self.always_exchange):
                comm.broadcast("shift", 0)

    @property
    def collectives_per_step(self) -> int:
        return (3 if self.cfg.tica_dim > 0 else 2) + self.cfg.kmeans_iters

    def _stamp(self, name: str):
        if self.time_stages:
            ev = self.eng.event()
            ev.record()
            self.stage_events.setdefault(name, []).append(ev)

    def step(self) -> None:
        eng, cfg, b, comm = self.eng, self.cfg, self.buf, self.comm
        multi = comm is not None and (comm.world > 1 or self.always_exchange)
        F, d, k = cfg.n_features, cfg.cluster_dim, cfg.k
        self._stamp("begin")
        if self.xyz is not None:
            eng.featurize_distances_into(self.xyz, self.pairs_d, self.x)
            self._stamp("featurize")
        if cfg.tica_dim > 0:
            eng.lagged_moments(self.x, cfg.lag, b["shift"], assume_finite=True, out=b["lagged"], symmetric=True)
            eng.moments_from_lagged(self.x, cfg.lag, b["shift"], b["lagged"], out=b["mom_sums"])
            if multi:
                comm.allreduce_sum("moments")
            eng.standardise_params(b["mom_sums"], b["shift"], F, float(self.n_total), True,
                                   out=(self.mean, self.scale, self.inv_scale))
            self._stamp("moments")
            eng.tica_solve(b["lagged"], F, scale=self.scale, epsilon=1e-6, kinetic_map=True,
                           out=(self.eig, self.W, self.m2, self.rank_d))
            self._stamp("tica_solve")
            eng.project(self.x, b["shift"], self.inv_scale, self.W, d, mean2=self.m2, out=self.Y,
                        absmax=b["fit_state"].view((1,), offset_elems=2), assume_finite=True)
            self._stamp("project")
        eng.kmeans_fit_begin(self.Y, k, seed=cfg.seed, n_total=self.n_total, tol2=0.0, centers=b["centers"],
                             state=b["fit_state"], absmax_ready=cfg.tica_dim > 0)
        if multi:
            if comm.rank != 0:
                b["centers"].fill_bytes_(0x7F)
            b["start_scale"].copy_from(b["fit_scale"])
            comm.allreduce_min("start")
            b["fit_scale"].copy_from(b["start_scale"])
            comm.reciprocal("fit_inv_scale", "fit_scale")
        acc = self.km_local if self.km_local is not None else b["km_acc"]
        acc.zero_()
        acc_sums, acc_counts = acc.view((k * d,), np.int64), acc.view((k,), np.int64, offset_elems=k * d)
        self.labels.fill_bytes_(0xFF)
        if self.km_image is not None:
            eng.kmeans_pack(self.Y, image=self.km_image, absmax=b["fit_state"].view((1,), offset_elems=2))
        for _ in range(cfg.kmeans_iters):
            if self.time_accum:
                e0, e1 = eng.event(), eng.event()
                e0.record()
            if not multi:
                eng.kmeans_lloyd_pass(self.Y, b["centers"], b["fit_state"], acc_sums, acc_counts,
                                      image=self.km_image, prev_labels=self.labels)
            else:
                eng.kmeans_accumulate(self.Y, b["centers"], b["fit_state"], acc_sums, acc_counts,
                                      image=self.km_image, prev_labels=self.labels)
            if self.time_accum:
                e1.record()
                self.accum_events.append((e0, e1))
            if multi:
                comm.allreduce_sum_from("km_acc", self.km_local)
                eng.kmeans_update(self.km_sums, self.km_counts, b["centers"], b["fit_state"], clear=False)
        eng.kmeans_assign(self.Y, b["centers"], labels=self.labels, image=self.km_image)
        self._stamp("kmeans")
        if cfg.lags:
            L = len(cfg.lags)
            eng.count_transitions_lagscan(self.labels, k, cfg.lags, out=b["counts"].view((L, k, k)),
                                          pairs=b["counts"].view((L,), offset_elems=L * k * k))
            if multi:
                comm.allreduce_sum("counts")
            li = list(cfg.lags).index(cfg.lag) if cfg.lag in cfg.lags else 0
            eng.row_normalise_into(b["counts"].view((k, k), offset_elems=li * k * k), self.T, self.rowsum, self.diag)
        else:
            eng.count_transitions(self.labels, k, cfg.lag, out=b["counts"].view((k, k)),
                                  pairs=b["counts"].view((1,), offset_elems=k * k))
            if multi:
                comm.allreduce_sum("counts")
            eng.row_normalise_into(b["counts"].view((k, k)), self.T, self.rowsum, self.diag)
        self._stamp("counts")

    def lagscan_counts(self) -> np.ndarray:
        L, k = len(self.cfg.lags), self.cfg.k
        return self.buf["counts"].view((L, k, k)).to_host()


def torch_exchange_buffers(engine: Engine, cfg: ShardConfig, device) -> tuple[dict, dict]:
    import torch

    tensors, views = {}, {}
    for name, (shape, dt) in exchange_shapes(cfg).items():
        t = torch.zeros(shape, dtype=getattr(torch, dt), device=device)
        tensors[name] = t
        views[name] = engine.wrap(t.data_ptr(), shape, np.dtype(dt))
    for name, (parent, first, length) in exchange_aliases(cfg).items():
        tensors[name] = tensors[parent][first:first + length]
        views[name] = views[parent].view((length,), offset_elems=first)
    return tensors, views
```

Before: 701.0 million frames/s.

## Fuse edge-moment and standardise prologue into TICA solve; drop memsets

On the single-GPU path, the edge-moment sums and feature standardisation now run as a prologue inside the single-block TICA eigen-solver kernel, which also zeroes the absmax word. This replaces the separate moments_from_lagged and standardise_params launches and the absmax memset. The k-means accumulator zeroing and labels fill are folded into fit_begin, and a dedicated first Lloyd pass removes the need for the 0xFF labels sentinel. The intent is to cut small kernel launches and memsets on the critical path, at the cost of running the serial prologue inside a one-block kernel and adding more specialised code paths.

```diff
diff --git a/include/msmhip.h b/include/msmhip.h
--- a/include/msmhip.h
+++ b/include/msmhip.h
@@ -139,6 +139,13 @@
                           double epsilon, int kinetic_map, double* d_eigvals, double* d_coeffs,
                           double* d_mean, int* d_rank);
 
+msm_status msm_tica_solve_from_lagged(msm_ctx* ctx, const void* d_x, msm_dtype dtype, int64_t n, int F, int64_t ld,
+                                      const int64_t* h_seg_start, const int64_t* h_seg_stop, int n_seg, int lag,
+                                      const double* d_shift, const double* d_moments, double n_rows, int with_std,
+                                      double epsilon, int kinetic_map, double* d_sums, double* d_mean, double* d_scale,
+                                      double* d_inv_scale, double* d_eigvals, double* d_coeffs, double* d_mean2,
+                                      int* d_rank, double* d_clear_word);
+
 msm_status msm_project(msm_ctx* ctx, const void* d_x, msm_dtype dtype, int64_t n, int F, int64_t ld,
                        const double* d_mu, const double* d_inv_sigma, const double* d_mean2,
                        const double* d_w, int d, int64_t ldw, double* d_y, int64_t ldy, double* d_absmax);
@@ -146,6 +153,11 @@
 msm_status msm_project_finite(msm_ctx* ctx, const void* d_x, msm_dtype dtype, int64_t n, int F, int64_t ld,
                               const double* d_mu, const double* d_inv_sigma, const double* d_mean2,
                               const double* d_w, int d, int64_t ldw, double* d_y, int64_t ldy, double* d_absmax);
+
+msm_status msm_project_cleared(msm_ctx* ctx, const void* d_x, msm_dtype dtype, int64_t n, int F, int64_t ld,
+                               const double* d_mu, const double* d_inv_sigma, const double* d_mean2,
+                               const double* d_w, int d, int64_t ldw, double* d_y, int64_t ldy, double* d_absmax,
+                               int assume_finite);
 
 msm_status msm_eigh(msm_ctx* ctx, const double* d_a, int n, double* d_w, double* d_v, int* d_sweeps);
 
@@ -174,6 +186,11 @@
                                 int64_t ld, const double* d_mean, const double* d_std, int k,
                                 uint64_t seed, int init_centers, double n_total, double tol2,
                                 double* d_centers, double* d_state, int absmax_ready);
+msm_status msm_kmeans_fit_begin_clear(msm_ctx* ctx, const void* d_x, msm_dtype dtype, int64_t n, int d,
+                                      int64_t ld, const double* d_mean, const double* d_std, int k,
+                                      uint64_t seed, int init_centers, double n_total, double tol2,
+                                      double* d_centers, double* d_state, int absmax_ready, int64_t* d_clear,
+                                      int64_t n_clear);
 msm_status msm_kmeans_accumulate(msm_ctx* ctx, const void* d_x, msm_dtype dtype, int64_t n, int d,
                                  int64_t ld, const double* d_centers, int k, const double* d_mean,
                                  const double* d_std, const double* d_state, int64_t* d_sums,
@@ -202,6 +219,10 @@
                                  double* d_centers, int k, const double* d_mean, const double* d_std,
                                  const void* d_image, double* d_state, int32_t* d_prev_labels, int64_t* d_sums,
                                  int64_t* d_counts);
+msm_status msm_kmeans_lloyd_first_pass(msm_ctx* ctx, const void* d_x, msm_dtype dtype, int64_t n, int d, int64_t ld,
+                                       double* d_centers, int k, const double* d_mean, const double* d_std,
+                                       const void* d_image, double* d_state, int32_t* d_prev_labels, int64_t* d_sums,
+                                       int64_t* d_counts);
 msm_status msm_kmeans_filter_scanned(msm_ctx* ctx, uint64_t* h_out, int reset);
 msm_status msm_mfma_bf16_probe(msm_ctx* ctx, const uint16_t* h_a, const uint16_t* h_b, const float* h_c,
                                float* h_d, int n_tiles);
diff --git a/pmarlo_amd/_lib.py b/pmarlo_amd/_lib.py
--- a/pmarlo_amd/_lib.py
+++ b/pmarlo_amd/_lib.py
@@ -75,6 +75,9 @@
     "msm_onesided_tica_eigenvalues": (_i32, [_vp, _vp, _i32, _f64, _vp]),
     "msm_moments_from_lagged": (_i32, [_vp, _vp, _i32, _i64, _i32, _i64, _vp, _vp, _i32, _i32, _vp, _vp, _vp]),
     "msm_project": (_i32, [_vp, _vp, _i32, _i64, _i32, _i64, _vp, _vp, _vp, _vp, _i32, _i64, _vp, _i64, _vp]),
+    "msm_tica_solve_from_lagged": (_i32, [_vp, _vp, _i32, _i64, _i32, _i64, _vp, _vp, _i32, _i32, _vp, _vp, _f64, _i32, _f64,
+                                          _i32, _vp, _vp, _vp, _vp, _vp, _vp, _vp, _vp, _vp]),
+    "msm_project_cleared": (_i32, [_vp, _vp, _i32, _i64, _i32, _i64, _vp, _vp, _vp, _vp, _i32, _i64, _vp, _i64, _vp, _i32]),
     "msm_project_finite": (_i32, [_vp, _vp, _i32, _i64, _i32, _i64, _vp, _vp, _vp, _vp, _i32, _i64, _vp, _i64, _vp]),
     "msm_eigh": (_i32, [_vp, _vp, _i32, _vp, _vp, _vp]),
     "msm_autocorr_lagscan": (_i32, [_vp, _vp, _i32, _i64, _i32, _i64, _vp, _vp, _i32, _vp, _i32, _f64, _vp, _vp]),
@@ -83,6 +86,8 @@
     "msm_kmeans_fit": (_i32, [_vp, _vp, _i32, _i64, _i32, _i64, _vp, _vp, _i32, C.c_uint64, _i32, _i32, _f64, _vp, _vp]),
     "msm_kmeans_fit_begin": (
         _i32, [_vp, _vp, _i32, _i64, _i32, _i64, _vp, _vp, _i32, C.c_uint64, _i32, _f64, _f64, _vp, _vp, _i32]),
+    "msm_kmeans_fit_begin_clear": (
+        _i32, [_vp, _vp, _i32, _i64, _i32, _i64, _vp, _vp, _i32, C.c_uint64, _i32, _f64, _f64, _vp, _vp, _i32, _vp, _i64]),
     "msm_kmeans_accumulate": (_i32, [_vp, _vp, _i32, _i64, _i32, _i64, _vp, _i32, _vp, _vp, _vp, _vp, _vp]),
     "msm_kmeans_update": (_i32, [_vp, _vp, _vp, _i32, _i32, _vp, _vp, _i32]),
     "msm_comm_unique_id": (_i32, [_vp, _sz]),
@@ -102,6 +107,7 @@
     "msm_kmeans_assign_packed": (_i32, [_vp, _vp, _i32, _i64, _i32, _i64, _vp, _i32, _vp, _vp, _vp, _vp, _vp]),
     "msm_kmeans_accumulate_packed": (_i32, [_vp, _vp, _i32, _i64, _i32, _i64, _vp, _i32, _vp, _vp, _vp, _vp, _vp, _vp]),
     "msm_kmeans_lloyd_pass": (_i32, [_vp, _vp, _i32, _i64, _i32, _i64, _vp, _i32, _vp, _vp, _vp, _vp, _vp, _vp, _vp]),
+    "msm_kmeans_lloyd_first_pass": (_i32, [_vp, _vp, _i32, _i64, _i32, _i64, _vp, _i32, _vp, _vp, _vp, _vp, _vp, _vp, _vp]),
     "msm_kmeans_accumulate_delta": (_i32, [_vp, _vp, _i32, _i64, _i32, _i64, _vp, _i32, _vp, _vp, _vp, _vp, _vp, _vp,
                                            _vp]),
     "msm_kmeans_filter_scanned": (_i32, [_vp, C.POINTER(C.c_uint64), _i32]),
diff --git a/pmarlo_amd/csrc/cov.hip b/pmarlo_amd/csrc/cov.hip
--- a/pmarlo_amd/csrc/cov.hip
+++ b/pmarlo_amd/csrc/cov.hip
@@ -1,4 +1,5 @@
 #include "common.h"
+#include "standardise.h"
 
 #include <cstring>
 
@@ -731,39 +732,18 @@
 
 namespace {
 
-struct EdgeSegs {
-    int n;
-    int lag;
-    int64_t start[MSM_SEG_INLINE];
-    int64_t stop[MSM_SEG_INLINE];
-};
-
 template <typename T>
 __global__ __launch_bounds__(256) void moments_from_lagged_kernel(const T* __restrict__ x, int F, int64_t ld,
                                                                   EdgeSegs sg, const double* __restrict__ shift,
                                                                   const double* __restrict__ mom,
                                                                   double* __restrict__ sums) {
-    double frames = 0.0;
-    for (int q = 0; q < sg.n; ++q) frames += (double)(sg.stop[q] - sg.start[q]);
+    const double frames = edge_frames(sg);
     for (int f = threadIdx.x; f < F; f += blockDim.x) {
-        const double sh = shift[f];
-        double e1 = 0.0, e2 = 0.0;
-        for (int q = 0; q < sg.n; ++q) {
-            const int64_t s = sg.start[q], e = sg.stop[q];
-            const int64_t head = min<int64_t>(s + sg.lag, e), tail = max<int64_t>(e - sg.lag, s);
-            const int n_head = (int)(head - s), n_edge = n_head + (int)(e - tail);
-#pragma unroll 8
-            for (int q2 = 0; q2 < n_edge; ++q2) {
-                const int64_t t = q2 < n_head ? s + q2 : tail + (q2 - n_head);
-                const double z = (double)x[t * ld + f] - sh;
-                e1 += z;
-                e2 = fma(z, z, e2);
-            }
-        }
-        const double sx = mom[(size_t)2 * F * F + f], sy = mom[(size_t)2 * F * F + F + f];
+        double s1, s2;
+        edge_moment_sums(x, F, ld, sg, shift, mom, f, &s1, &s2);
         sums[f] = frames;
-        sums[F + f] = 0.5 * (sx + sy + e1);
-        sums[2 * F + f] = 0.5 * (mom[(size_t)f * F + f] + e2);
+        sums[F + f] = s1;
+        sums[2 * F + f] = s2;
     }
 }
 
@@ -821,17 +801,7 @@
     MSM_REQUIRE(ctx, d_shift && d_moments && d_sums && (d_x || n == 0), "msm_moments_from_lagged: NULL pointer");
     MSM_REQUIRE(ctx, n_seg >= 0 && n_seg <= MSM_SEG_INLINE && (n_seg == 0 || (h_seg_start && h_seg_stop)),
                 "msm_moments_from_lagged: at most %d segments per call", MSM_SEG_INLINE);
-    EdgeSegs sg;
-    sg.n = 0;
-    sg.lag = lag;
-    if (n_seg == 0) {
-        if (n > 0) { sg.start[0] = 0; sg.stop[0] = n; sg.n = 1; }
-    } else {
-        for (int q = 0; q < n_seg; ++q) {
-            const int64_t a = std::max<int64_t>(0, h_seg_start[q]), b = std::min<int64_t>(n, h_seg_stop[q]);
-            if (b > a) { sg.start[sg.n] = a; sg.stop[sg.n] = b; ++sg.n; }
-        }
-    }
+    const EdgeSegs sg = make_edge_segs(n, h_seg_start, h_seg_stop, n_seg, lag);
     if (dtype == MSM_F32)
         hipLaunchKernelGGL(moments_from_lagged_kernel<float>, dim3(1), dim3(256), 0, ctx->stream, (const float*)d_x, F, ld,
                            sg, d_shift, d_moments, d_sums);
diff --git a/pmarlo_amd/csrc/eig.hip b/pmarlo_amd/csrc/eig.hip
--- a/pmarlo_amd/csrc/eig.hip
+++ b/pmarlo_amd/csrc/eig.hip
@@ -1,5 +1,8 @@
 #include "common.h"
+#include "standardise.h"
 #include "wave.h"
+
+#include <type_traits>
 
 #ifdef MSM_JACOBI_STAMPS
 __device__ unsigned long long g_jacobi_stamps[8];
@@ -964,11 +967,27 @@
     int* order;
 };
 
-template <int lds_mats>
+template <typename TX>
+struct TicaPre {
+    const TX* x;
+    int64_t ld;
+    EdgeSegs sg;
+    const double* shift;
+    double n_rows;
+    int with_std;
+    double *sums, *mean, *scale, *inv_scale;
+    unsigned long long* clear_word;
+};
+template <>
+struct TicaPre<void> {};
+
+template <int lds_mats, typename TX = void>
 __global__ __launch_bounds__(kEigThreads) void tica_solve_kernel(
     const double* __restrict__ mom, const double* __restrict__ scale, int n, int ld, double epsilon, int kinetic_map,
     TicaWork wk, double* __restrict__ out_eig, double* __restrict__ out_W, double* __restrict__ out_mean,
-    int* __restrict__ out_rank) {
+    int* __restrict__ out_rank, TicaPre<TX> pre) {
+    constexpr bool kPre = !std::is_void<TX>::value;
+    static_assert(!kPre || lds_mats == 4, "the prologue keeps 1 / scale in the solver's LDS arrays");
     extern __shared__ __attribute__((aligned(16))) unsigned char smem_raw[];
     __shared__ JacobiShared sh;
     __shared__ TriShared ts;
@@ -986,6 +1005,23 @@
     const double T = sy[n];
     const double w = 2.0 * T;
     KSTAMP_INIT
+    if constexpr (kPre) {
+        const double frames = edge_frames(pre.sg);
+        for (int f = tid; f < n; f += nt) {
+            double s1, s2, m, sd;
+            edge_moment_sums(pre.x, n, pre.ld, pre.sg, pre.shift, mom, f, &s1, &s2);
+            pre.sums[f] = frames;
+            pre.sums[n + f] = s1;
+            pre.sums[2 * n + f] = s2;
+            standardise_feature(frames, s1, s2, pre.shift[f], pre.n_rows, pre.with_std, &m, &sd);
+            pre.mean[f] = m;
+            pre.scale[f] = sd;
+            const double is = 1.0 / sd;
+            pre.inv_scale[f] = is;
+            ts.lam[f] = is;
+        }
+        if (tid == 0 && pre.clear_word) *pre.clear_word = 0ull;
+    }
     if (!(T > 0.0)) {
         if (tid == 0) *out_rank = 0;
         for (int i = tid; i < n; i += nt) { out_eig[i] = 0.0; out_mean[i] = 0.0; }
@@ -995,8 +1031,13 @@
     double* iscp = (lds_mats == 4 && n <= kTriMax) ? ts.lam : wk.isc;
     double* meanp = (lds_mats == 4 && n <= kTriMax) ? ts.inv : wk.mean;
     for (int i = tid; i < n; i += nt) {
-        const double is = scale ? 1.0 / scale[i] : 1.0;
-        iscp[i] = is;
+        double is;
+        if constexpr (kPre) {
+            is = iscp[i];
+        } else {
+            is = scale ? 1.0 / scale[i] : 1.0;
+            iscp[i] = is;
+        }
         const double m = (sx[i] + sy[i]) / w * is;
         meanp[i] = m;
         out_mean[i] = m;
@@ -1337,7 +1378,57 @@
     if (lds > 48 * 1024)
         MSM_HIP(ctx, hipFuncSetAttribute((const void*)kern, hipFuncAttributeMaxDynamicSharedMemorySize, (int)lds));
     hipLaunchKernelGGL(kern, dim3(1), dim3(kEigThreads), lds, ctx->stream, d_moments, d_scale, F, ld, epsilon,
-                       kinetic_map, wk, d_eigvals, d_coeffs, d_mean, d_rank);
+                       kinetic_map, wk, d_eigvals, d_coeffs, d_mean, d_rank, TicaPre<void>{});
+    MSM_CHECK_LAUNCH(ctx);
+    return MSM_OK;
+}
+
+msm_status msm_tica_solve_from_lagged(msm_ctx* ctx, const void* d_x, msm_dtype dtype, int64_t n, int F, int64_t ld,
+                                      const int64_t* h_seg_start, const int64_t* h_seg_stop, int n_seg, int lag,
+                                      const double* d_shift, const double* d_moments, double n_rows, int with_std,
+                                      double epsilon, int kinetic_map, double* d_sums, double* d_mean, double* d_scale,
+                                      double* d_inv_scale, double* d_eigvals, double* d_coeffs, double* d_mean2,
+                                      int* d_rank, double* d_clear_word) {
+    if (!ctx) return MSM_ERR_INVALID;
+    if (F > kTriMax) {
+        msm_status rs = msm_moments_from_lagged(ctx, d_x, dtype, n, F, ld, h_seg_start, h_seg_stop, n_seg, lag, d_shift,
+                                                d_moments, d_sums);
+        if (rs != MSM_OK) return rs;
+        rs = msm_standardise_params(ctx, d_sums, d_shift, F, n_rows, with_std, d_mean, d_scale, d_inv_scale);
+        if (rs != MSM_OK) return rs;
+        if (d_clear_word) MSM_HIP(ctx, hipMemsetAsync(d_clear_word, 0, sizeof(unsigned long long), ctx->stream));
+        return msm_tica_solve(ctx, d_moments, d_scale, F, epsilon, kinetic_map, d_eigvals, d_coeffs, d_mean2, d_rank);
+    }
+    MSM_REQUIRE(ctx, n >= 0 && F >= 1 && ld >= F && lag >= 1, "msm_tica_solve_from_lagged: bad shape / lag");
+    MSM_REQUIRE(ctx, dtype == MSM_F32 || dtype == MSM_F64, "msm_tica_solve_from_lagged: bad dtype");
+    MSM_REQUIRE(ctx, n_seg >= 0 && n_seg <= MSM_SEG_INLINE && (n_seg == 0 || (h_seg_start && h_seg_stop)),
+                "msm_tica_solve_from_lagged: at most %d segments per call", MSM_SEG_INLINE);
+    MSM_REQUIRE(ctx, n_rows >= 1.0 && epsilon >= 0.0, "msm_tica_solve_from_lagged: need n_rows >= 1, epsilon >= 0");
+    MSM_REQUIRE(ctx, d_shift && d_moments && d_sums && d_mean && d_scale && d_inv_scale && d_eigvals && d_coeffs &&
+                         d_mean2 && d_rank && (d_x || n == 0), "msm_tica_solve_from_lagged: NULL pointer");
+    const int ldm = kTriLd;
+    const size_t mat = (size_t)F * ldm;
+    const size_t need = (4 * mat + 3 * F) * sizeof(double) + (size_t)F * sizeof(int) + 64;
+    msm_status rs = msm_reserve_scratch(ctx, need);
+    if (rs != MSM_OK) return rs;
+    double* base = (double*)ctx->scratch;
+    TicaWork wk;
+    wk.A = base; wk.V = base + mat; wk.B1 = base + 2 * mat; wk.B2 = base + 3 * mat;
+    wk.ev = base + 4 * mat; wk.mean = wk.ev + F; wk.isc = wk.mean + F; wk.order = (int*)(wk.isc + F);
+    const size_t lds = 4 * mat * sizeof(double);
+    const EdgeSegs sg = make_edge_segs(n, h_seg_start, h_seg_stop, n_seg, lag);
+#define MSM_TICA_PRE(TX)                                                                                              \
+    do {                                                                                                              \
+        auto kern = tica_solve_kernel<4, TX>;                                                                         \
+        if (lds > 48 * 1024)                                                                                          \
+            MSM_HIP(ctx, hipFuncSetAttribute((const void*)kern, hipFuncAttributeMaxDynamicSharedMemorySize, (int)lds)); \
+        TicaPre<TX> pre{(const TX*)d_x, ld, sg, d_shift, n_rows, with_std, d_sums, d_mean, d_scale, d_inv_scale,      \
+                        (unsigned long long*)d_clear_word};                                                          \
+        hipLaunchKernelGGL(kern, dim3(1), dim3(kEigThreads), lds, ctx->stream, d_moments, (const double*)nullptr, F, ldm, \
+                           epsilon, kinetic_map, wk, d_eigvals, d_coeffs, d_mean2, d_rank, pre);                      \
+    } while (0)
+    if (dtype == MSM_F32) MSM_TICA_PRE(float); else MSM_TICA_PRE(double);
+#undef MSM_TICA_PRE
     MSM_CHECK_LAUNCH(ctx);
     return MSM_OK;
 }
diff --git a/pmarlo_amd/csrc/kmeans.hip b/pmarlo_amd/csrc/kmeans.hip
--- a/pmarlo_amd/csrc/kmeans.hip
+++ b/pmarlo_amd/csrc/kmeans.hip
@@ -103,9 +103,10 @@
                                     const double* __restrict__ mean, const double* __restrict__ stdv, int k,
                                     unsigned long long seed, double* __restrict__ centers,
                                     const unsigned long long* __restrict__ absmax_bits, double n_total, double tol2,
-                                    FitState* __restrict__ st) {
+                                    FitState* __restrict__ st, unsigned long long* __restrict__ clear, int64_t n_clear) {
     const int i = blockIdx.x * blockDim.x + threadIdx.x;
     if (i == 0 && st) fit_scale_body(absmax_bits, n_total, tol2, st);
+    if (i < n_clear) clear[i] = 0ull;
     if (i >= k * d) return;
     const int j = i / d, f = i - j * d;
     unsigned long long h = seed + 0x9E3779B97F4A7C15ull * (unsigned long long)(j + 1);
@@ -844,7 +845,8 @@
 template <typename T, int DP, bool ACCUM>
 msm_status launch_filter_dp(msm_ctx* ctx, const T* x, int64_t n, int d, int64_t ld, const double* centers, int k,
                             const double* mean, const double* stdv, const uint4* image, int32_t* labels, double* mindist,
-                            const FitState* st, unsigned long long* sums, unsigned long long* counts, double* upd_centers) {
+                            const FitState* st, unsigned long long* sums, unsigned long long* counts, double* upd_centers,
+                            bool fresh) {
     constexpr int NF = 4;
     const size_t lds = filter_lds_bytes(k, d, ACCUM);
     msm_status rs;
@@ -859,7 +861,7 @@
         MSM_HIP(ctx, hipFuncSetAttribute((const void*)kern, hipFuncAttributeMaxDynamicSharedMemorySize, (int)lds));
     hipLaunchKernelGGL(kern, dim3(grid), dim3(64 * kWaves), lds, ctx->stream, x, n, d, ld, k, mean, stdv, image, centers,
                        labels, mindist, st, sums, counts, stats, stats ? upd_centers : nullptr,
-                       stats ? (unsigned int*)(stats + 1) : nullptr);
+                       stats ? (unsigned int*)(stats + 1) : nullptr, (int)fresh);
     MSM_CHECK_LAUNCH(ctx);
     return MSM_OK;
 }
@@ -867,12 +869,13 @@
 template <typename T, bool ACCUM>
 msm_status launch_filter(msm_ctx* ctx, const T* x, int64_t n, int d, int64_t ld, const double* centers, int k,
                          const double* mean, const double* stdv, const uint4* image, int32_t* labels, double* mindist,
-                         const FitState* st, unsigned long long* sums, unsigned long long* counts, double* upd_centers) {
+                         const FitState* st, unsigned long long* sums, unsigned long long* counts, double* upd_centers,
+                         bool fresh) {
     if (filter_dp(d) == 4)
         return launch_filter_dp<T, 4, ACCUM>(ctx, x, n, d, ld, centers, k, mean, stdv, image, labels, mindist, st, sums,
-                                             counts, upd_centers);
+                                             counts, upd_centers, fresh);
     return launch_filter_dp<T, 10, ACCUM>(ctx, x, n, d, ld, centers, k, mean, stdv, image, labels, mindist, st, sums, counts,
-                                          upd_centers);
+                                          upd_centers, fresh);
 }
 
 bool filter_fits(int k, int d, bool accum) { return filter_enabled() && d <= kFilterMaxD && filter_lds_bytes(k, d, accum) != 0; }
@@ -881,7 +884,7 @@
 msm_status dispatch_mfma(msm_ctx* ctx, const T* x, int64_t n, int d, int64_t ld, const double* centers, int k,
                          const double* mean, const double* stdv, int32_t* labels, double* mindist, const FitState* st,
                          unsigned long long* sums, unsigned long long* counts, const void* image = nullptr,
-                         double* upd_centers = nullptr, bool* folded = nullptr) {
+                         double* upd_centers = nullptr, bool* folded = nullptr, bool fresh = false) {
     if (folded) *folded = false;
     if (filter_fits(k, d, ACCUM)) {
         if (getenv("MSM_KMEANS_DEBUG"))
@@ -897,8 +900,9 @@
         if (upd_centers && !(ACCUM && (int64_t)k * d <= kUpdateWide && (ctx->km_stats || !ctx->capturing))) upd_centers = nullptr;
         if (folded) *folded = upd_centers != nullptr;
         return launch_filter<T, ACCUM>(ctx, x, n, d, ld, centers, k, mean, stdv, (const uint4*)image, labels, mindist, st,
-                                       sums, counts, upd_centers);
-    }
+                                       sums, counts, upd_centers, fresh);
+    }
+    if (ACCUM && fresh && labels) MSM_HIP(ctx, hipMemsetAsync(labels, 0xFF, (size_t)n * sizeof(int32_t), ctx->stream));
 #define MSM_MFMA_CASE(KSV) \
     if (d <= 4 * KSV)      \
         return launch_mfma<T, KSV, ACCUM>(ctx, x, n, d, ld, centers, k, mean, stdv, labels, mindist, st, sums, counts)
@@ -1023,10 +1027,13 @@
     return mfma_probe(ctx, true, h_a, h_b, h_c, h_d, n_tiles);
 }
 
-msm_status msm_kmeans_fit_begin(msm_ctx* ctx, const void* d_x, msm_dtype dtype, int64_t n, int d, int64_t ld,
-                                const double* d_mean, const double* d_std, int k, uint64_t seed, int init_centers,
-                                double n_total, double tol2, double* d_centers, double* d_state, int absmax_ready) {
+static msm_status kmeans_fit_begin_impl(msm_ctx* ctx, const void* d_x, msm_dtype dtype, int64_t n, int d, int64_t ld,
+                                        const double* d_mean, const double* d_std, int k, uint64_t seed, int init_centers,
+                                        double n_total, double tol2, double* d_centers, double* d_state, int absmax_ready,
+                                        int64_t* d_clear, int64_t n_clear) {
     if (!ctx) return MSM_ERR_INVALID;
+    MSM_REQUIRE(ctx, n_clear >= 0 && n_clear < (int64_t(1) << 31) && (d_clear || n_clear == 0),
+                "msm_kmeans_fit_begin: bad clear range");
     MSM_REQUIRE(ctx, n >= 1 && d >= 1 && d <= 256 && k >= 1 && ld >= d, "msm_kmeans_fit_begin: bad shape");
     MSM_REQUIRE(ctx, !absmax_ready || !d_mean, "msm_kmeans_fit_begin: a precomputed max |x| excludes whitening");
     MSM_REQUIRE(ctx, !init_centers || n >= k, "msm_kmeans_fit_begin: fewer frames (%lld) than centres (%d)",
@@ -1048,29 +1055,46 @@
         MSM_CHECK_LAUNCH(ctx);
     }
     if (!init_centers) {
+        if (n_clear) MSM_HIP(ctx, hipMemsetAsync(d_clear, 0, (size_t)n_clear * sizeof(int64_t), ctx->stream));
         hipLaunchKernelGGL(fit_scale_kernel, dim3(1), dim3(64), 0, ctx->stream, bits, n_total, tol2, (FitState*)d_state);
         MSM_CHECK_LAUNCH(ctx);
     }
     if (init_centers) {
-        const int g2 = msm_ceil_div((int64_t)k * d, 256);
+        unsigned long long* clr = (unsigned long long*)d_clear;
+        const int g2 = msm_ceil_div(std::max<int64_t>((int64_t)k * d, n_clear), 256);
         if (dtype == MSM_F32)
             hipLaunchKernelGGL(init_centers_kernel<float>, dim3(g2), dim3(256), 0, ctx->stream, (const float*)d_x, n, d,
                                ld, d_mean, d_std, k, (unsigned long long)seed, d_centers, bits, n_total, tol2,
-                               (FitState*)d_state);
+                               (FitState*)d_state, clr, n_clear);
         else
             hipLaunchKernelGGL(init_centers_kernel<double>, dim3(g2), dim3(256), 0, ctx->stream, (const double*)d_x, n,
                                d, ld, d_mean, d_std, k, (unsigned long long)seed, d_centers, bits, n_total, tol2,
-                               (FitState*)d_state);
+                               (FitState*)d_state, clr, n_clear);
         MSM_CHECK_LAUNCH(ctx);
     }
     return MSM_OK;
+}
+
+msm_status msm_kmeans_fit_begin(msm_ctx* ctx, const void* d_x, msm_dtype dtype, int64_t n, int d, int64_t ld,
+                                const double* d_mean, const double* d_std, int k, uint64_t seed, int init_centers,
+                                double n_total, double tol2, double* d_centers, double* d_state, int absmax_ready) {
+    return kmeans_fit_begin_impl(ctx, d_x, dtype, n, d, ld, d_mean, d_std, k, seed, init_centers, n_total, tol2, d_centers,
+                                 d_state, absmax_ready, nullptr, 0);
+}
+
+msm_status msm_kmeans_fit_begin_clear(msm_ctx* ctx, const void* d_x, msm_dtype dtype, int64_t n, int d, int64_t ld,
+                                      const double* d_mean, const double* d_std, int k, uint64_t seed, int init_centers,
+                                      double n_total, double tol2, double* d_centers, double* d_state, int absmax_ready,
+                                      int64_t* d_clear, int64_t n_clear) {
+    return kmeans_fit_begin_impl(ctx, d_x, dtype, n, d, ld, d_mean, d_std, k, seed, init_centers, n_total, tol2, d_centers,
+                                 d_state, absmax_ready, d_clear, n_clear);
 }
 
 static msm_status kmeans_accumulate_impl(msm_ctx* ctx, const void* d_x, msm_dtype dtype, int64_t n, int d, int64_t ld,
                                          const double* d_centers, int k, const double* d_mean, const double* d_std,
                                          const void* d_image, const double* d_state, int64_t* d_sums, int64_t* d_counts,
                                          int32_t* d_prev_labels = nullptr, double* d_update_centers = nullptr,
-                                         bool* folded = nullptr) {
+                                         bool* folded = nullptr, bool fresh = false) {
     if (folded) *folded = false;
     if (!ctx) return MSM_ERR_INVALID;
     MSM_REQUIRE(ctx, n >= 0 && d >= 1 && k >= 1 && ld >= d, "msm_kmeans_accumulate: bad shape");
@@ -1081,20 +1105,38 @@
     if (dtype == MSM_F32)
         return dispatch_mfma<float, true>(ctx, (const float*)d_x, n, d, ld, d_centers, k, d_mean, d_std, d_prev_labels,
                                           nullptr, (const FitState*)d_state, (unsigned long long*)d_sums,
-                                          (unsigned long long*)d_counts, d_image, d_update_centers, folded);
+                                          (unsigned long long*)d_counts, d_image, d_update_centers, folded, fresh);
     return dispatch_mfma<double, true>(ctx, (const double*)d_x, n, d, ld, d_centers, k, d_mean, d_std, d_prev_labels,
                                        nullptr, (const FitState*)d_state, (unsigned long long*)d_sums,
-                                       (unsigned long long*)d_counts, d_image, d_update_centers, folded);
+                                       (unsigned long long*)d_counts, d_image, d_update_centers, folded, fresh);
+}
+
+static msm_status kmeans_lloyd_pass_impl(msm_ctx* ctx, const void* d_x, msm_dtype dtype, int64_t n, int d, int64_t ld,
+                                         double* d_centers, int k, const double* d_mean, const double* d_std,
+                                         const void* d_image, double* d_state, int32_t* d_prev_labels, int64_t* d_sums,
+                                         int64_t* d_counts, bool fresh) {
+    bool folded = false;
+    msm_status rs = kmeans_accumulate_impl(ctx, d_x, dtype, n, d, ld, d_centers, k, d_mean, d_std, d_image, d_state, d_sums,
+                                           d_counts, d_prev_labels, d_centers, &folded, fresh);
+    if (rs != MSM_OK || folded) return rs;
+    return msm_kmeans_update(ctx, d_sums, d_counts, k, d, d_centers, d_state, 0);
 }
 
 msm_status msm_kmeans_lloyd_pass(msm_ctx* ctx, const void* d_x, msm_dtype dtype, int64_t n, int d, int64_t ld,
                                  double* d_centers, int k, const double* d_mean, const double* d_std, const void* d_image,
                                  double* d_state, int32_t* d_prev_labels, int64_t* d_sums, int64_t* d_counts) {
-    bool folded = false;
-    msm_status rs = kmeans_accumulate_impl(ctx, d_x, dtype, n, d, ld, d_centers, k, d_mean, d_std, d_image, d_state, d_sums,
-                                           d_counts, d_prev_labels, d_centers, &folded);
-    if (rs != MSM_OK || folded) return rs;
-    return msm_kmeans_update(ctx, d_sums, d_counts, k, d, d_centers, d_state, 0);
+    return kmeans_lloyd_pass_impl(ctx, d_x, dtype, n, d, ld, d_centers, k, d_mean, d_std, d_image, d_state, d_prev_labels,
+                                  d_sums, d_counts, false);
+}
+
+msm_status msm_kmeans_lloyd_first_pass(msm_ctx* ctx, const void* d_x, msm_dtype dtype, int64_t n, int d, int64_t ld,
+                                       double* d_centers, int k, const double* d_mean, const double* d_std,
+                                       const void* d_image, double* d_state, int32_t* d_prev_labels, int64_t* d_sums,
+                                       int64_t* d_counts) {
+    if (!ctx) return MSM_ERR_INVALID;
+    MSM_REQUIRE(ctx, d_prev_labels || n == 0, "msm_kmeans_lloyd_first_pass: NULL label buffer");
+    return kmeans_lloyd_pass_impl(ctx, d_x, dtype, n, d, ld, d_centers, k, d_mean, d_std, d_image, d_state, d_prev_labels,
+                                  d_sums, d_counts, true);
 }
 
 msm_status msm_kmeans_accumulate_delta(msm_ctx* ctx, const void* d_x, msm_dtype dtype, int64_t n, int d, int64_t ld,
diff --git a/pmarlo_amd/csrc/kmeans_filter.h b/pmarlo_amd/csrc/kmeans_filter.h
--- a/pmarlo_amd/csrc/kmeans_filter.h
+++ b/pmarlo_amd/csrc/kmeans_filter.h
@@ -347,7 +347,7 @@
     int32_t* __restrict__ labels,
     double* __restrict__ mindist, const FitState* __restrict__ st, unsigned long long* __restrict__ sums,
     unsigned long long* __restrict__ counts, unsigned long long* __restrict__ n_scanned, double* upd_centers,
-    unsigned int* __restrict__ ticket) {
+    unsigned int* __restrict__ ticket, int fresh) {
     using S = FilterShape<DP>;
     constexpr int kFilterWaves = filter_waves(DP, ACCUM);
     constexpr int kMT = 64 * kFilterWaves, RF = S::RF, RQ = kFilterRowQ;
@@ -426,6 +426,7 @@
     const bool vec_rows = sizeof(T) == 8 && d == DP && ((ld * sizeof(T)) & 15) == 0 && (((uintptr_t)x) & 15) == 0;
     const int iters = n_tiles / 2;
     constexpr int kNone = 0x7fffffff;
+    const bool booked = ACCUM && labels != nullptr && fresh == 0;
 
     auto load_frame = [&](int64_t t, double (&z)[DP]) { filter_load_frame<T, DP, WHITEN>(x, ld, d, vec_rows, mean, stdv, t, z); };
     auto score64 = [&](const double* crow, int c, const double (&z)[DP]) {
@@ -484,7 +485,7 @@
         if (sbi >= k) { sbi = 0; sbest = -__builtin_inf(); }
         int old_s = -1;
         if constexpr (ACCUM) {
-            if (labels) old_s = labels[t];
+            if (booked) old_s = labels[t];
         }
         commit_scan(t, sbi, sbest, zz, old_s);
 #ifdef MSM_KMF_DIAG_COUNT
@@ -541,7 +542,7 @@
         const int64_t fr = fok ? f0 : n - 1;
         int old = -1;
         if constexpr (ACCUM) {
-            if (labels) old = labels[fr];
+            if (booked) old = labels[fr];
         }
         double z[DP];
         load_frame(fr, z);
diff --git a/pmarlo_amd/csrc/moments.hip b/pmarlo_amd/csrc/moments.hip
--- a/pmarlo_amd/csrc/moments.hip
+++ b/pmarlo_amd/csrc/moments.hip
@@ -1,4 +1,5 @@
 #include "common.h"
+#include "standardise.h"
 #include "wave.h"
 
 namespace {
@@ -108,16 +109,8 @@
                                           double* __restrict__ scale, double* __restrict__ inv_scale) {
     const int f = blockIdx.x * blockDim.x + threadIdx.x;
     if (f >= F) return;
-    const double cnt = sums[f], s1 = sums[F + f], s2 = sums[2 * F + f];
-    double m = 0.0, sd = 1.0;
-    if (cnt > 0.0) {
-        m = shift[f] + s1 / cnt;
-        if (with_std) {
-            const double var = (s2 - s1 * s1 / cnt) / n_rows;
-            sd = var > 0.0 ? sqrt(var) : 0.0;
-            if (sd < 10.0 * 2.220446049250313e-16) sd = 1.0;
-        }
-    }
+    double m, sd;
+    standardise_feature(sums[f], sums[F + f], sums[2 * F + f], shift[f], n_rows, with_std, &m, &sd);
     mean[f] = m;
     scale[f] = sd;
     inv_scale[f] = 1.0 / sd;
@@ -509,11 +502,12 @@
 
 static msm_status project_impl(msm_ctx* ctx, const void* d_x, msm_dtype dtype, int64_t n, int F, int64_t ld,
                                const double* d_mu, const double* d_inv_sigma, const double* d_mean2, const double* d_w, int d,
-                               int64_t ldw, double* d_y, int64_t ldy, double* d_absmax, bool finite) {
+                               int64_t ldw, double* d_y, int64_t ldy, double* d_absmax, bool finite,
+                               bool absmax_cleared = false) {
     if (!ctx) return MSM_ERR_INVALID;
     MSM_REQUIRE(ctx, n >= 0 && F >= 1 && d >= 1 && d <= 64, "msm_project: need n >= 0, F >= 1, 1 <= d <= 64");
     unsigned long long* bits = reinterpret_cast<unsigned long long*>(d_absmax);
-    if (bits) MSM_HIP(ctx, hipMemsetAsync(bits, 0, sizeof(unsigned long long), ctx->stream));
+    if (bits && !absmax_cleared) MSM_HIP(ctx, hipMemsetAsync(bits, 0, sizeof(unsigned long long), ctx->stream));
     MSM_REQUIRE(ctx, ld >= F && ldw >= d && ldy >= d, "msm_project: bad leading dimension");
     MSM_REQUIRE(ctx, dtype == MSM_F32 || dtype == MSM_F64, "msm_project: bad dtype");
     if (n == 0) return MSM_OK;
@@ -569,4 +563,11 @@
     return project_impl(ctx, d_x, dtype, n, F, ld, d_mu, d_inv_sigma, d_mean2, d_w, d, ldw, d_y, ldy, d_absmax, true);
 }
 
-}
+msm_status msm_project_cleared(msm_ctx* ctx, const void* d_x, msm_dtype dtype, int64_t n, int F, int64_t ld,
+                               const double* d_mu, const double* d_inv_sigma, const double* d_mean2, const double* d_w,
+                               int d, int64_t ldw, double* d_y, int64_t ldy, double* d_absmax, int assume_finite) {
+    return project_impl(ctx, d_x, dtype, n, F, ld, d_mu, d_inv_sigma, d_mean2, d_w, d, ldw, d_y, ldy, d_absmax,
+                        assume_finite != 0, true);
+}
+
+}
diff --git a/pmarlo_amd/csrc/standardise.h b/pmarlo_amd/csrc/standardise.h
--- /dev/null
+++ b/pmarlo_amd/csrc/standardise.h
@@ -0,0 +1,71 @@
+#pragma once
+
+#include <algorithm>
+
+#include "common.h"
+
+struct EdgeSegs {
+    int n;
+    int lag;
+    int64_t start[MSM_SEG_INLINE];
+    int64_t stop[MSM_SEG_INLINE];
+};
+
+static inline EdgeSegs make_edge_segs(int64_t n, const int64_t* h_seg_start, const int64_t* h_seg_stop, int n_seg, int lag) {
+    EdgeSegs sg;
+    sg.n = 0;
+    sg.lag = lag;
+    if (n_seg == 0) {
+        if (n > 0) { sg.start[0] = 0; sg.stop[0] = n; sg.n = 1; }
+    } else {
+        for (int q = 0; q < n_seg; ++q) {
+            const int64_t a = std::max<int64_t>(0, h_seg_start[q]), b = std::min<int64_t>(n, h_seg_stop[q]);
+            if (b > a) { sg.start[sg.n] = a; sg.stop[sg.n] = b; ++sg.n; }
+        }
+    }
+    return sg;
+}
+
+__device__ __forceinline__ double edge_frames(const EdgeSegs& sg) {
+    double frames = 0.0;
+    for (int q = 0; q < sg.n; ++q) frames += (double)(sg.stop[q] - sg.start[q]);
+    return frames;
+}
+
+template <typename T>
+__device__ __forceinline__ void edge_moment_sums(const T* __restrict__ x, int F, int64_t ld, const EdgeSegs& sg,
+                                                 const double* __restrict__ shift, const double* __restrict__ mom, int f,
+                                                 double* s1, double* s2) {
+    const double sh = shift[f];
+    double e1 = 0.0, e2 = 0.0;
+    for (int q = 0; q < sg.n; ++q) {
+        const int64_t s = sg.start[q], e = sg.stop[q];
+        const int64_t head = min<int64_t>(s + sg.lag, e), tail = max<int64_t>(e - sg.lag, s);
+        const int n_head = (int)(head - s), n_edge = n_head + (int)(e - tail);
+#pragma unroll 8
+        for (int q2 = 0; q2 < n_edge; ++q2) {
+            const int64_t t = q2 < n_head ? s + q2 : tail + (q2 - n_head);
+            const double z = (double)x[t * ld + f] - sh;
+            e1 += z;
+            e2 = fma(z, z, e2);
+        }
+    }
+    const double sx = mom[(size_t)2 * F * F + f], sy = mom[(size_t)2 * F * F + F + f];
+    *s1 = 0.5 * (sx + sy + e1);
+    *s2 = 0.5 * (mom[(size_t)f * F + f] + e2);
+}
+
+__device__ __forceinline__ void standardise_feature(double cnt, double s1, double s2, double shift, double n_rows,
+                                                    int with_std, double* mean, double* sigma) {
+    double m = 0.0, sd = 1.0;
+    if (cnt > 0.0) {
+        m = shift + s1 / cnt;
+        if (with_std) {
+            const double var = (s2 - s1 * s1 / cnt) / n_rows;
+            sd = var > 0.0 ? sqrt(var) : 0.0;
+            if (sd < 10.0 * 2.220446049250313e-16) sd = 1.0;
+        }
+    }
+    *mean = m;
+    *sigma = sd;
+}
diff --git a/pmarlo_amd/device.py b/pmarlo_amd/device.py
--- a/pmarlo_amd/device.py
+++ b/pmarlo_amd/device.py
@@ -538,16 +538,43 @@
               self.handle)
         return eig, W, mean, rank
 
+    def tica_solve_from_lagged(self, x: DeviceArray, lag: int, shift: DeviceArray, moments: DeviceArray, n_rows: float, *,
+                               with_std: bool = True, epsilon: float = 1e-6, kinetic_map: bool = True, starts=None,
+                               stops=None, sums: DeviceArray | None = None, params=None, out=None,
+                               clear_word: DeviceArray | None = None, ld: int | None = None):
+        n, F = x.shape
+        if starts is None:
+            starts, stops = segments_to_bounds(None, n)
+        starts, stops = self._seg_ptrs(starts, stops)
+        sums = sums if sums is not None else self.empty((3 * F,), np.float64)
+        mean, scale, inv = params if params is not None else tuple(self.empty((F,), np.float64) for _ in range(3))
+        if out is not None:
+            eig, W, mean2, rank = out
+        else:
+            eig, W, mean2 = self.empty((F,), np.float64), self.empty((F, F), np.float64), self.empty((F,), np.float64)
+            rank = self.empty((1,), np.int32)
+        check(lib.msm_tica_solve_from_lagged(self.handle, x.ptr, _dtype_code(x.dtype), n, F, int(F if ld is None else ld),
+                                             starts.ctypes.data, stops.ctypes.data, len(starts), int(lag), shift.ptr,
+                                             moments.ptr, float(n_rows), int(bool(with_std)), float(epsilon),
+                                             int(bool(kinetic_map)), sums.ptr, mean.ptr, scale.ptr, inv.ptr, eig.ptr, W.ptr,
+                                             mean2.ptr, rank.ptr, clear_word.ptr if clear_word is not None else None),
+              self.handle)
+        return sums, (mean, scale, inv), (eig, W, mean2, rank)
+
     def project(self, x: DeviceArray, mu: DeviceArray, inv_sigma: DeviceArray, W: DeviceArray, d: int, *,
                 mean2: DeviceArray | None = None, out: DeviceArray | None = None,
-                absmax: DeviceArray | None = None, assume_finite: bool = False, ld: int | None = None) -> DeviceArray:
+                absmax: DeviceArray | None = None, assume_finite: bool = False, ld: int | None = None,
+                absmax_cleared: bool = False) -> DeviceArray:
         n, F = x.shape
         ldw = W.shape[1]
         out = out if out is not None else self.empty((n, d), np.float64)
-        fn = lib.msm_project_finite if assume_finite else lib.msm_project
-        check(fn(self.handle, x.ptr, _dtype_code(x.dtype), n, F, int(F if ld is None else ld), mu.ptr, inv_sigma.ptr,
-                 mean2.ptr if mean2 is not None else None, W.ptr, int(d), ldw, out.ptr,
-                 out.shape[1], absmax.ptr if absmax is not None else None), self.handle)
+        args = (self.handle, x.ptr, _dtype_code(x.dtype), n, F, int(F if ld is None else ld), mu.ptr, inv_sigma.ptr,
+                mean2.ptr if mean2 is not None else None, W.ptr, int(d), ldw, out.ptr,
+                out.shape[1], absmax.ptr if absmax is not None else None)
+        if absmax_cleared:
+            check(lib.msm_project_cleared(*args, int(bool(assume_finite))), self.handle)
+        else:
+            check((lib.msm_project_finite if assume_finite else lib.msm_project)(*args), self.handle)
         return out
 
     def eigh(self, a: DeviceArray, want_vectors: bool = True):
@@ -636,15 +663,20 @@
     def kmeans_fit_begin(self, x: DeviceArray, k: int, *, seed: int, n_total: int, tol2: float,
                          mean: DeviceArray | None = None, std: DeviceArray | None = None,
                          centers: DeviceArray | None = None, init_centers: bool = True,
-                         state: DeviceArray | None = None, absmax_ready: bool = False):
+                         state: DeviceArray | None = None, absmax_ready: bool = False,
+                         clear: DeviceArray | None = None):
         n, d = x.shape
         centers = centers if centers is not None else self.empty((k, d), np.float64)
         state = state if state is not None else self.zeros((8,), np.float64)
-        check(lib.msm_kmeans_fit_begin(self.handle, x.ptr, _dtype_code(x.dtype), n, d, d,
-                                       mean.ptr if mean is not None else None,
-                                       std.ptr if std is not None else None, int(k), int(seed) & (2**64 - 1),
-                                       int(bool(init_centers)), float(n_total), float(tol2), centers.ptr, state.ptr,
-                                       int(bool(absmax_ready))), self.handle)
+        args = (self.handle, x.ptr, _dtype_code(x.dtype), n, d, d, mean.ptr if mean is not None else None,
+                std.ptr if std is not None else None, int(k), int(seed) & (2**64 - 1), int(bool(init_centers)),
+                float(n_total), float(tol2), centers.ptr, state.ptr, int(bool(absmax_ready)))
+        if clear is not None:
+            if clear.dtype != np.dtype(np.int64):
+                raise TypeError("kmeans_fit_begin: `clear` must be an int64 array")
+            check(lib.msm_kmeans_fit_begin_clear(*args, clear.ptr, int(clear.size)), self.handle)
+        else:
+            check(lib.msm_kmeans_fit_begin(*args), self.handle)
         return centers, state
 
     def kmeans_accumulate(self, x: DeviceArray, centers: DeviceArray, state: DeviceArray, sums: DeviceArray,
@@ -708,14 +740,14 @@
 
     def kmeans_lloyd_pass(self, x: DeviceArray, centers: DeviceArray, state: DeviceArray, sums: DeviceArray,
                           counts: DeviceArray, *, mean: DeviceArray | None = None, std: DeviceArray | None = None,
-                          image: DeviceArray | None = None, prev_labels: DeviceArray | None = None):
+                          image: DeviceArray | None = None, prev_labels: DeviceArray | None = None, first: bool = False):
         n, d = x.shape
         k = centers.shape[0]
-        check(lib.msm_kmeans_lloyd_pass(self.handle, x.ptr, _dtype_code(x.dtype), n, d, d, centers.ptr, k,
-                                        mean.ptr if mean is not None else None, std.ptr if std is not None else None,
-                                        image.ptr if image is not None else None, state.ptr,
-                                        prev_labels.ptr if prev_labels is not None else None, sums.ptr, counts.ptr),
-              self.handle)
+        fn = lib.msm_kmeans_lloyd_first_pass if first else lib.msm_kmeans_lloyd_pass
+        check(fn(self.handle, x.ptr, _dtype_code(x.dtype), n, d, d, centers.ptr, k,
+                 mean.ptr if mean is not None else None, std.ptr if std is not None else None,
+                 image.ptr if image is not None else None, state.ptr,
+                 prev_labels.ptr if prev_labels is not None else None, sums.ptr, counts.ptr), self.handle)
 
     def kmeans_update(self, sums: DeviceArray, counts: DeviceArray, centers: DeviceArray, state: DeviceArray,
                       clear: bool = True):
diff --git a/pmarlo_amd/dist.py b/pmarlo_amd/dist.py
--- a/pmarlo_amd/dist.py
+++ b/pmarlo_amd/dist.py
@@ -352,20 +352,35 @@
             self._stamp("featurize")
         if cfg.tica_dim > 0:
             eng.lagged_moments(self.x, cfg.lag, b["shift"], assume_finite=True, out=b["lagged"], symmetric=True)
-            eng.moments_from_lagged(self.x, cfg.lag, b["shift"], b["lagged"], out=b["mom_sums"])
+            absmax = b["fit_state"].view((1,), offset_elems=2)
             if multi:
+                eng.moments_from_lagged(self.x, cfg.lag, b["shift"], b["lagged"], out=b["mom_sums"])
                 comm.allreduce_sum("moments")
-            eng.standardise_params(b["mom_sums"], b["shift"], F, float(self.n_total), True,
-                                   out=(self.mean, self.scale, self.inv_scale))
-            self._stamp("moments")
-            eng.tica_solve(b["lagged"], F, scale=self.scale, epsilon=1e-6, kinetic_map=True,
-                           out=(self.eig, self.W, self.m2, self.rank_d))
+                eng.standardise_params(b["mom_sums"], b["shift"], F, float(self.n_total), True,
+                                       out=(self.mean, self.scale, self.inv_scale))
+                self._stamp("moments")
+                eng.tica_solve(b["lagged"], F, scale=self.scale, epsilon=1e-6, kinetic_map=True,
+                               out=(self.eig, self.W, self.m2, self.rank_d))
+            else:
+                self._stamp("moments")
+                eng.tica_solve_from_lagged(self.x, cfg.lag, b["shift"], b["lagged"], float(self.n_total),
+                                           sums=b["mom_sums"], params=(self.mean, self.scale, self.inv_scale),
+                                           out=(self.eig, self.W, self.m2, self.rank_d), clear_word=absmax)
             self._stamp("tica_solve")
-            eng.project(self.x, b["shift"], self.inv_scale, self.W, d, mean2=self.m2, out=self.Y,
-                        absmax=b["fit_state"].view((1,), offset_elems=2), assume_finite=True)
+            if multi:
+                eng.project(self.x, b["shift"], self.inv_scale, self.W, d, mean2=self.m2, out=self.Y, absmax=absmax,
+                            assume_finite=True)
+            else:
+                eng.project(self.x, b["shift"], self.inv_scale, self.W, d, mean2=self.m2, out=self.Y, absmax=absmax,
+                            assume_finite=True, absmax_cleared=True)
             self._stamp("project")
-        eng.kmeans_fit_begin(self.Y, k, seed=cfg.seed, n_total=self.n_total, tol2=0.0, centers=b["centers"],
-                             state=b["fit_state"], absmax_ready=cfg.tica_dim > 0)
+        acc = self.km_local if self.km_local is not None else b["km_acc"]
+        if multi:
+            eng.kmeans_fit_begin(self.Y, k, seed=cfg.seed, n_total=self.n_total, tol2=0.0, centers=b["centers"],
+                                 state=b["fit_state"], absmax_ready=cfg.tica_dim > 0)
+        else:
+            eng.kmeans_fit_begin(self.Y, k, seed=cfg.seed, n_total=self.n_total, tol2=0.0, centers=b["centers"],
+                                 state=b["fit_state"], absmax_ready=cfg.tica_dim > 0, clear=acc)
         if multi:
             if comm.rank != 0:
                 b["centers"].fill_bytes_(0x7F)
@@ -373,19 +388,18 @@
             comm.allreduce_min("start")
             b["fit_scale"].copy_from(b["start_scale"])
             comm.reciprocal("fit_inv_scale", "fit_scale")
-        acc = self.km_local if self.km_local is not None else b["km_acc"]
-        acc.zero_()
+            acc.zero_()
+            self.labels.fill_bytes_(0xFF)
         acc_sums, acc_counts = acc.view((k * d,), np.int64), acc.view((k,), np.int64, offset_elems=k * d)
-        self.labels.fill_bytes_(0xFF)
         if self.km_image is not None:
             eng.kmeans_pack(self.Y, image=self.km_image, absmax=b["fit_state"].view((1,), offset_elems=2))
-        for _ in range(cfg.kmeans_iters):
+        for it in range(cfg.kmeans_iters):
             if self.time_accum:
                 e0, e1 = eng.event(), eng.event()
                 e0.record()
             if not multi:
                 eng.kmeans_lloyd_pass(self.Y, b["centers"], b["fit_state"], acc_sums, acc_counts,
-                                      image=self.km_image, prev_labels=self.labels)
+                                      image=self.km_image, prev_labels=self.labels, first=it == 0)
             else:
                 eng.kmeans_accumulate(self.Y, b["centers"], b["fit_state"], acc_sums, acc_counts,
                                       image=self.km_image, prev_labels=self.labels)
```

Measured after the change: 707.0 million frames/s, median of 6. Within noise of the previous version (+0.8%).
